# bminixhofer/zett

Hardware: AMD Instinct MI355X
Metric: predicted token-embeddings/sec (full target vocab) (higher is better)
Workload: dtype f16

## Files before the change

zett_amd/csrc/gemm.hip.h:

```cpp
#pragma once

#include <hip/hip_runtime.h>
#include <stdint.h>

#include <type_traits>

#ifndef ZETT_GROUP_M
#define ZETT_GROUP_M 4
#endif

namespace zett {

typedef __attribute__((ext_vector_type(16))) float f32x16;
typedef __attribute__((ext_vector_type(4))) float f32x4;
typedef __attribute__((ext_vector_type(8))) __bf16 bf16x8;
typedef __attribute__((ext_vector_type(4))) uint32_t u32x4;

typedef uint16_t bf16_t;
typedef _Float16 f16_t;
typedef __attribute__((ext_vector_type(8))) _Float16 f16x8;

__device__ __forceinline__ float bf16_to_f32(bf16_t v) { return __uint_as_float(((uint32_t)v) << 16); }
__device__ __forceinline__ bf16_t f32_to_bf16(float f) {
    return __builtin_bit_cast(bf16_t, (__bf16)f);
// ... 76 lines not shown
}

typedef __attribute__((ext_vector_type(2))) float f32x2;
#define ZETT_PIN_STAGE(arr, n) do { _Pragma("unroll") for (int e_ = 0; e_ < (n); ++e_) asm volatile("" : "+v"((arr)[e_])); } while (0)

template <int ACT, bool HAS_RES, bool HAS_SCALE, int NV>
__device__ __forceinline__ void epi_values(float (&vs)[NV], const float (&bias)[NV], const float (&res)[NV], const float (&sc)[NV], const float (&sh)[NV]) {
#pragma clang fp contract(off)
    static_assert(NV % 2 == 0, "pairs");
    constexpr int NP = NV / 2;
    f32x2 v[NP];
#pragma unroll
    for (int e = 0; e < NP; ++e) v[e] = f32x2{vs[2 * e], vs[2 * e + 1]} + f32x2{bias[2 * e], bias[2 * e + 1]};
    if (ACT == ACT_GELU_TANH) {
        f32x2 u2[NP], t[NP];
        ZETT_PIN_STAGE(v, NP);
#pragma unroll
        for (int e = 0; e < NP; ++e) u2[e] = (v[e] * v[e]) * v[e];
        ZETT_PIN_STAGE(u2, NP);
#pragma unroll
        for (int e = 0; e < NP; ++e) u2[e] = 1.5957691216057308f * __builtin_elementwise_fma(f32x2{0.044715f, 0.044715f}, u2[e], v[e]);
        ZETT_PIN_STAGE(u2, NP);
#pragma unroll
        for (int e = 0; e < NP; ++e) u2[e] = u2[e] * 1.4426950408889634f;
        ZETT_PIN_STAGE(u2, NP);
#pragma unroll
        for (int e = 0; e < NP; ++e) t[e] = f32x2{__builtin_amdgcn_exp2f(u2[e].x), __builtin_amdgcn_exp2f(u2[e].y)};
        ZETT_PIN_STAGE(t, NP);
#pragma unroll
        for (int e = 0; e < NP; ++e) t[e] = 1.0f + t[e];
        ZETT_PIN_STAGE(t, NP);
#pragma unroll
        for (int e = 0; e < NP; ++e) t[e] = f32x2{__builtin_amdgcn_rcpf(t[e].x), __builtin_amdgcn_rcpf(t[e].y)};
        ZETT_PIN_STAGE(t, NP);
#pragma unroll
        for (int e = 0; e < NP; ++e) t[e] = 1.0f - 2.0f * t[e];
        ZETT_PIN_STAGE(t, NP);
#pragma unroll
        for (int e = 0; e < NP; ++e) v[e] = (0.5f * v[e]) * (1.0f + t[e]);
        ZETT_PIN_STAGE(v, NP);
    } else if (ACT == ACT_GELU_ERF) {
        f32x2 z[NP], ax[NP], t[NP], p[NP], ex[NP];
        ZETT_PIN_STAGE(v, NP);
#pragma unroll
        for (int e = 0; e < NP; ++e) z[e] = v[e] * 0.70710678118654752440f;
        ZETT_PIN_STAGE(z, NP);
#pragma unroll
        for (int e = 0; e < NP; ++e) ax[e] = __builtin_elementwise_abs(z[e]);
#pragma unroll
        for (int e = 0; e < NP; ++e) t[e] = __builtin_elementwise_fma(f32x2{0.3275911f, 0.3275911f}, ax[e], f32x2{1.0f, 1.0f});
        ZETT_PIN_STAGE(t, NP);
#pragma unroll
        for (int e = 0; e < NP; ++e) t[e] = f32x2{__builtin_amdgcn_rcpf(t[e].x), __builtin_amdgcn_rcpf(t[e].y)};
        ZETT_PIN_STAGE(t, NP);
#pragma unroll
        for (int e = 0; e < NP; ++e) ex[e] = (ax[e] * ax[e]) * -1.4426950408889634f;
        ZETT_PIN_STAGE(ex, NP);
#pragma unroll
        for (int e = 0; e < NP; ++e) ex[e] = f32x2{__builtin_amdgcn_exp2f(ex[e].x), __builtin_amdgcn_exp2f(ex[e].y)};
        ZETT_PIN_STAGE(ex, NP);
#pragma unroll
        for (int e = 0; e < NP; ++e) p[e] = __builtin_elementwise_fma(f32x2{1.061405429f, 1.061405429f}, t[e], f32x2{-1.453152027f, -1.453152027f});
        ZETT_PIN_STAGE(p, NP);
#pragma unroll
        for (int e = 0; e < NP; ++e) p[e] = __builtin_elementwise_fma(p[e], t[e], f32x2{1.421413741f, 1.421413741f});
        ZETT_PIN_STAGE(p, NP);
#pragma unroll
        for (int e = 0; e < NP; ++e) p[e] = __builtin_elementwise_fma(p[e], t[e], f32x2{-0.284496736f, -0.284496736f});
        ZETT_PIN_STAGE(p, NP);
#pragma unroll
        for (int e = 0; e < NP; ++e) p[e] = __builtin_elementwise_fma(p[e], t[e], f32x2{0.254829592f, 0.254829592f});
        ZETT_PIN_STAGE(p, NP);
#pragma unroll
        for (int e = 0; e < NP; ++e) p[e] = -(p[e] * t[e]);
        ZETT_PIN_STAGE(p, NP);
#pragma unroll
        for (int e = 0; e < NP; ++e) p[e] = __builtin_elementwise_fma(p[e], ex[e], f32x2{1.0f, 1.0f});
        ZETT_PIN_STAGE(p, NP);
#pragma unroll
        for (int e = 0; e < NP; ++e) p[e] = 1.0f + __builtin_elementwise_copysign(p[e], z[e]);
        ZETT_PIN_STAGE(p, NP);
#pragma unroll
        for (int e = 0; e < NP; ++e) v[e] = (v[e] * 0.5f) * p[e];
        ZETT_PIN_STAGE(v, NP);
    }
    if (HAS_RES) {
#pragma unroll
        for (int e = 0; e < NP; ++e) v[e] = v[e] + f32x2{res[2 * e], res[2 * e + 1]};
    }
    if (HAS_SCALE) {
#pragma unroll
        for (int e = 0; e < NP; ++e) v[e] = __builtin_elementwise_fma(f32x2{sc[2 * e], sc[2 * e + 1]}, v[e], f32x2{sh[2 * e], sh[2 * e + 1]});
    }
#pragma unroll
    for (int e = 0; e < NP; ++e) { vs[2 * e] = v[e].x; vs[2 * e + 1] = v[e].y; }
}

template <typename T>
struct GemmEpilogue {
    const float* bias;
    int act;
    const float* residual;
    int ld_res;
    const float* res_stats;
    const float* res_gamma;
    const float* res_beta;
    const int32_t* res_index;
    float2* stats_part;
    int ld_part;
    const float* fold_stats;
    const float* fold_c;
    const float* scale;
    const float* shift;
    float* out_f32;
    int ld_f32;
    T* out_lo;
    int ld_lo;
    int split_col;
    float* out_f32_b;
    int32_t* range_flag;
    int range_final;
    const T* residual_lo;
    int ld_res_lo;
    void* dst;
    const int64_t* dst_rows;
    int64_t ld_dst;
    int dst_dtype;
};

template <typename T> struct LoRange { static constexpr bool checked = false; static constexpr float limit = 0.f; };
template <> struct LoRange<f16_t> { static constexpr bool checked = true; static constexpr float limit = 65504.0f; };
__device__ __forceinline__ bool out_of_range(float v, float limit) { return !(__builtin_fabsf(v) <= limit); }
constexpr float ZETT_F32_MAX = 3.402823466e38f;
constexpr int ZETT_RANGE_BIT_SOURCE = 1, ZETT_RANGE_BIT_ACTIVATION = 2, ZETT_RANGE_BIT_OUTPUT = 4, ZETT_RANGE_BIT_WEIGHT = 8, ZETT_RANGE_BIT_DEST = 16;
template <typename OT> __device__ __forceinline__ bool dest_overflow(float v) {
    if constexpr (std::is_same<OT, f16_t>::value) { const float a = __builtin_fabsf(v); return a >= 65520.0f && a <= 3.402823466e38f; }
    else return false;
}
__device__ __forceinline__ void range_report(int32_t* flag, bool bad, int bit) {
    if (bad && flag) atomicOr(flag, bit);
}

template <typename T>
struct GemmArgs {
    const T* A;
    int lda;
    const T* W;
    int ldw;
    int M, N, K;
    GemmEpilogue<T> epi;
    int tile_order = 0;
    int group = 0;
    int row0 = 0;
};

constexpr int GEMM_BM = 128;
constexpr int GEMM_BN = 128;
constexpr int GEMM_WAIT_VMCNT0 = 0x0F70;
constexpr int GEMM_ROW_BYTES = 128;
constexpr int GEMM_TILE_BYTES = GEMM_BM * GEMM_ROW_BYTES;

__device__ __forceinline__ int lds_chunk_off(int row, int chunk) {
    return row * GEMM_ROW_BYTES + ((chunk ^ ((row >> 1) & 7)) << 4);
}

template <typename T>
__device__ __forceinline__ void mfma_chunk(const u32x4& a, const u32x4& b, f32x16& acc);

template <>
__device__ __forceinline__ void mfma_chunk<bf16_t>(const u32x4& a, const u32x4& b, f32x16& acc) {
    acc = __builtin_amdgcn_mfma_f32_32x32x16_bf16(__builtin_bit_cast(bf16x8, a), __builtin_bit_cast(bf16x8, b),
                                                  acc, 0, 0, 0);
}
template <>
__device__ __forceinline__ void mfma_chunk<f16_t>(const u32x4& a, const u32x4& b, f32x16& acc) {
    acc = __builtin_amdgcn_mfma_f32_32x32x16_f16(__builtin_bit_cast(f16x8, a), __builtin_bit_cast(f16x8, b), acc, 0, 0, 0);
}
template <>
__device__ __forceinline__ void mfma_chunk<float>(const u32x4& a, const u32x4& b, f32x16& acc) {
#pragma unroll
    for (int j = 0; j < 4; ++j)
        acc = __builtin_amdgcn_mfma_f32_32x32x2f32(__uint_as_float(a[j]), __uint_as_float(b[j]), acc, 0, 0, 0);
}

template <typename T>
__global__ __launch_bounds__(256) void gemm_tn_kernel(GemmArgs<T> g) {
    extern __shared__ __attribute__((aligned(16))) unsigned char smem[];
    constexpr int EPC = 16 / (int)sizeof(T);
    constexpr int BK = GEMM_ROW_BYTES / (int)sizeof(T);

    const int tiles_m = (g.M + GEMM_BM - 1) / GEMM_BM;
    const int tiles_n = (g.N + GEMM_BN - 1) / GEMM_BN;
    const int nwg = tiles_m * tiles_n;
    int wg = blockIdx.x;
    {
        const int q = nwg >> 3, r = nwg & 7, xcd = wg & 7;
        wg = (xcd < r ? xcd * (q + 1) : r * (q + 1) + (xcd - r) * q) + (wg >> 3);
    }
    constexpr int GROUP_M = 8;
    const int group_size = GROUP_M * tiles_n;
    const int first_m = (wg / group_size) * GROUP_M;
    const int gm = (tiles_m - first_m) < GROUP_M ? (tiles_m - first_m) : GROUP_M;
    const int tm = first_m + (wg % group_size) % gm;
    const int tn = (wg % group_size) / gm;
    const int m0 = tm * GEMM_BM, n0 = tn * GEMM_BN;

    const int tid = threadIdx.x;
    const int lane = tid & 63, wave = tid >> 6;
    const int wm = wave >> 1, wn = wave & 1;
    const int l31 = lane & 31, hi = lane >> 5;

    const unsigned char* a_src[4];
    const unsigned char* w_src[4];
    int lds_dst[4];
#pragma unroll
    for (int i = 0; i < 4; ++i) {
        const int c = tid + 256 * i;
        const int row = c >> 3, ch = c & 7;
        int ar = m0 + row; ar = ar < g.M ? ar : g.M - 1;
        int wr = n0 + row; wr = wr < g.N ? wr : g.N - 1;
        a_src[i] = (const unsigned char*)(g.A + (size_t)ar * g.lda) + ch * 16;
        w_src[i] = (const unsigned char*)(g.W + (size_t)wr * g.ldw) + ch * 16;
        lds_dst[i] = lds_chunk_off(row, ch);
    }

    f32x16 acc[2][2];
#pragma unroll
    for (int i = 0; i < 2; ++i)
#pragma unroll
        for (int j = 0; j < 2; ++j)
#pragma unroll
            for (int r = 0; r < 16; ++r) acc[i][j][r] = 0.f;

    const int nk = g.K / BK;
    u32x4 ra[4], rw[4];
#pragma unroll
    for (int i = 0; i < 4; ++i) {
        ra[i] = *(const u32x4*)(a_src[i]);
        rw[i] = *(const u32x4*)(w_src[i]);
    }
#pragma unroll
    for (int i = 0; i < 4; ++i) {
        *(u32x4*)(smem + lds_dst[i]) = ra[i];
        *(u32x4*)(smem + GEMM_TILE_BYTES + lds_dst[i]) = rw[i];
    }
    __syncthreads();

    for (int kt = 0; kt < nk; ++kt) {
        const int cur = kt & 1;
        const unsigned char* As = smem + cur * 2 * GEMM_TILE_BYTES;
        const unsigned char* Ws = As + GEMM_TILE_BYTES;
        const bool more = kt + 1 < nk;
        if (more) {
            const size_t koff = (size_t)(kt + 1) * GEMM_ROW_BYTES;
#pragma unroll
            for (int i = 0; i < 4; ++i) {
                ra[i] = *(const u32x4*)(a_src[i] + koff);
                rw[i] = *(const u32x4*)(w_src[i] + koff);
            }
        }
#pragma unroll
        for (int kk = 0; kk < 4; ++kk) {
            const int ch = kk * 2 + hi;
            u32x4 fa[2], fw[2];
#pragma unroll
            for (int i = 0; i < 2; ++i) {
                fa[i] = *(const u32x4*)(As + lds_chunk_off(wm * 64 + i * 32 + l31, ch));
                fw[i] = *(const u32x4*)(Ws + lds_chunk_off(wn * 64 + i * 32 + l31, ch));
            }
#pragma unroll
            for (int i = 0; i < 2; ++i)
#pragma unroll
                for (int j = 0; j < 2; ++j) mfma_chunk<T>(fa[i], fw[j], acc[i][j]);
        }
        if (more) {
            unsigned char* Ad = smem + (cur ^ 1) * 2 * GEMM_TILE_BYTES;
#pragma unroll
            for (int i = 0; i < 4; ++i) {
                *(u32x4*)(Ad + lds_dst[i]) = ra[i];
                *(u32x4*)(Ad + GEMM_TILE_BYTES + lds_dst[i]) = rw[i];
            }
        }
        __syncthreads();
    }
    (void)EPC;

    const GemmEpilogue<T>& e = g.epi;
    bool bad_lo = false, bad_out = false;
#pragma unroll
    for (int j = 0; j < 2; ++j) {
        const int col = n0 + wn * 64 + j * 32 + l31;
        if (col >= g.N) continue;
        const float bias = e.bias ? e.bias[col] : 0.f;
        const float sc = e.scale ? e.scale[col] : 1.f;
        const float sh = e.shift ? e.shift[col] : 0.f;
#pragma unroll
        for (int i = 0; i < 2; ++i) {
#pragma unroll
            for (int r = 0; r < 16; ++r) {
                const int row = m0 + wm * 64 + i * 32 + (r & 3) + 8 * (r >> 2) + 4 * hi;
                if (row >= g.M) continue;
                const size_t rrow = e.res_index ? (size_t)e.res_index[row] : (size_t)row;
                float res = e.residual ? e.residual[rrow * e.ld_res + col] : 0.f;
                if (e.residual && e.res_stats) res = ln_affine(res, e.res_stats[2 * rrow], e.res_stats[2 * rrow + 1], e.res_gamma[col], e.res_beta[col]);
                const bool hr = e.residual != nullptr, hs = e.scale != nullptr;
                const float v = e.act == ACT_GELU_TANH ? epi_value<ACT_GELU_TANH>(acc[i][j][r], bias, hr, res, hs, sc, sh)
// ... 32 lines not shown
```

zett_amd/csrc/gemm4d.hip.h:

```cpp
#pragma once

#include <hip/hip_runtime.h>
#include <stdint.h>

#include <algorithm>
#include <type_traits>

#include "gemm_tile.hip.h"

namespace zett {

#ifndef G4D_ABLATE
#define G4D_ABLATE 5
#endif
constexpr int G4D_ABL = G4D_ABLATE;
#ifdef G4D_MFMA32
constexpr bool G4D_M32 = true;
static_assert(G4D_ABLATE < 5, "the 32x32x16 K loop exists for the ablation levels without an epilogue");
#else
constexpr bool G4D_M32 = false;
#endif
typedef float f32x16 __attribute__((ext_vector_type(16)));

constexpr int g4d_wait_vm(int n) { return ((n >> 4) << 14) | 0x0F70 | (n & 15); }

template <typename T> __device__ __forceinline__ void mfma16_agpr(f32x4& c, const u32x4& a, const u32x4& b);
template <> __device__ __forceinline__ void mfma16_agpr<bf16_t>(f32x4& c, const u32x4& a, const u32x4& b) {
    asm volatile("v_mfma_f32_16x16x32_bf16 %0, %1, %2, %0" : "+a"(c) : "v"(a), "v"(b));
}
template <> __device__ __forceinline__ void mfma16_agpr<f16_t>(f32x4& c, const u32x4& a, const u32x4& b) {
    asm volatile("v_mfma_f32_16x16x32_f16 %0, %1, %2, %0" : "+a"(c) : "v"(a), "v"(b));
}

template <typename T> __device__ __forceinline__ void mfma32_agpr(f32x16& c, const u32x4& a, const u32x4& b);
template <> __device__ __forceinline__ void mfma32_agpr<bf16_t>(f32x16& c, const u32x4& a, const u32x4& b) {
    asm volatile("v_mfma_f32_32x32x16_bf16 %0, %1, %2, %0" : "+a"(c) : "v"(a), "v"(b));
}
template <> __device__ __forceinline__ void mfma32_agpr<f16_t>(f32x16& c, const u32x4& a, const u32x4& b) {
    asm volatile("v_mfma_f32_32x32x16_f16 %0, %1, %2, %0" : "+a"(c) : "v"(a), "v"(b));
}

template <int K> __device__ __forceinline__ float g4d_xor_lane(float v) {
    return __builtin_bit_cast(float, __builtin_amdgcn_ds_swizzle(__builtin_bit_cast(int, v), (K << 10) | 0x1f));
}


enum { G4D_EPI_GENERIC = 0, G4D_EPI_LO = 1, G4D_EPI_F32 = 2, G4D_EPI_F32_SCALE = 3, G4D_EPI_BOTH = 4, G4D_EPI_F32_LN = 5, G4D_EPI_LO_FOLD = 6,
       G4D_EPI_LO_LN = 7, G4D_EPI_F32_SCALE_FOLD = 8, G4D_EPI_LN16 = 9 };
constexpr int G4D_EPI_STRIDE = 132;
constexpr int G4D_EPI_REGION = 64 * G4D_EPI_STRIDE * 4;
constexpr int G4D_LDS_BYTES = 4 * G4D_EPI_REGION;
static_assert(G4D_LDS_BYTES >= G256_LDS_BYTES && G4D_LDS_BYTES <= 160 * 1024, "LDS budget");

template <bool HALF> struct G4dGeom {
    static constexpr int BM = HALF ? 128 : G256_BM;
    static constexpr int WROWS = BM / 2;
    static constexpr int MI = WROWS / 16;
    static constexpr int AREQ = BM / 32;
    static constexpr int NREQ = AREQ + 8;
    static constexpr int NPASS = WROWS / 64;
    static constexpr int STAGES = HALF ? 3 : 2;
    static constexpr int A_BYTES = BM * GEMM_ROW_BYTES;
    static constexpr int STAGE_BYTES = A_BYTES + G256_OPERAND_BYTES;
    static constexpr int LDS_BYTES = STAGES * STAGE_BYTES;
};

template <typename T, int ACT = ACT_NONE, bool RES = false, int EPI = G4D_EPI_GENERIC, bool HALF = false, typename OT = void>
__global__ __launch_bounds__(256) __attribute__((amdgpu_waves_per_eu(1, 1))) void gemm4d_tn_kernel(GemmArgs<T> g) {
    extern __shared__ __attribute__((aligned(16))) unsigned char smem[];
    constexpr int BK = GEMM_ROW_BYTES / (int)sizeof(T);
    typedef G4dGeom<HALF> GEO;
    static_assert(!HALF || EPI != G4D_EPI_GENERIC, "the half tile carries the streamlined epilogues only");
    constexpr bool DST = !std::is_void<OT>::value;
    static_assert(!DST || EPI == G4D_EPI_F32_SCALE || EPI == G4D_EPI_F32_SCALE_FOLD, "destination stores: the output heads' epilogues only");

    const int tiles_m = (g.M - g.row0 + GEO::BM - 1) / GEO::BM;
    const int tiles_n = (g.N + G256_BN - 1) / G256_BN;
    const int nwg = tiles_m * tiles_n;
    int wg = blockIdx.x;
    {
        const int q = nwg >> 3, r = nwg & 7, xcd = wg & 7;
        wg = (xcd < r ? xcd * (q + 1) : r * (q + 1) + (xcd - r) * q) + (wg >> 3);
    }
    const int GROUP_N = g.group > 0 ? g.group : 4;
    int tm, tn;
    if (g.tile_order == 0) {
        const int group_size = GROUP_N * tiles_m;
        const int first_n = (wg / group_size) * GROUP_N;
        const int gn = (tiles_n - first_n) < GROUP_N ? (tiles_n - first_n) : GROUP_N;
        tn = first_n + (wg % group_size) % gn;
        tm = (wg % group_size) / gn;
    } else {
        const int GROUP_M = g.group > 0 ? g.group : ZETT_GROUP_M;
        const int group_size = GROUP_M * tiles_n;
        const int first_m = (wg / group_size) * GROUP_M;
        const int gm = (tiles_m - first_m) < GROUP_M ? (tiles_m - first_m) : GROUP_M;
        tm = first_m + (wg % group_size) % gm;
        tn = (wg % group_size) / gm;
    }
    const int m0 = g.row0 + tm * GEO::BM, n0 = tn * G256_BN;

    const int tid = threadIdx.x;
    const int lane = tid & 63;
    const int wave = __builtin_amdgcn_readfirstlane(tid >> 6);
    const int wm = wave >> 1, wn = wave & 1;

    const unsigned char* a_base = (const unsigned char*)(g.A + (size_t)m0 * g.lda);
    const unsigned char* w_base = (const unsigned char*)(g.W + (size_t)n0 * g.ldw);
    uint32_t a_voff[8], w_voff[8];
#pragma unroll
    for (int r = 0; r < 8; ++r) {
        const int row = wave * 64 + r * 8 + (lane >> 3);
        const int chunk = ((lane & 7) ^ ((row >> 1) & 7)) << 4;
        int wr = row; wr = n0 + wr < g.N ? wr : g.N - 1 - n0;
        w_voff[r] = (uint32_t)wr * (uint32_t)g.ldw * (uint32_t)sizeof(T) + chunk;
    }
#pragma unroll
    for (int r = 0; r < GEO::AREQ; ++r) {
        const int row = wave * (GEO::AREQ * 8) + r * 8 + (lane >> 3);
        const int chunk = ((lane & 7) ^ ((row >> 1) & 7)) << 4;
        int ar = row; ar = m0 + ar < g.M ? ar : g.M - 1 - m0;
        a_voff[r] = (uint32_t)ar * (uint32_t)g.lda * (uint32_t)sizeof(T) + chunk;
    }
    const __amdgpu_buffer_rsrc_t a_rsrc = __builtin_amdgcn_make_buffer_rsrc((void*)a_base, (short)0, 0x7fffffff, G4R_RSRC_WORD3);
    const __amdgpu_buffer_rsrc_t w_rsrc = __builtin_amdgcn_make_buffer_rsrc((void*)w_base, (short)0, 0x7fffffff, G4R_RSRC_WORD3);
    unsigned char* const my_rows = smem + wave * 64 * GEMM_ROW_BYTES;
    unsigned char* const my_a_rows = smem + wave * (GEO::AREQ * 8) * GEMM_ROW_BYTES;
    auto dma_a = [&](int stage, int kt, int r) {
        __builtin_amdgcn_raw_ptr_buffer_load_lds(a_rsrc, (lds_ptr_t)(my_a_rows + stage * GEO::STAGE_BYTES + r * 8 * GEMM_ROW_BYTES), 16,
                                                 a_voff[r], kt * GEMM_ROW_BYTES, 0, 0);
    };
    auto dma_w = [&](int stage, int kt, int r) {
        __builtin_amdgcn_raw_ptr_buffer_load_lds(w_rsrc, (lds_ptr_t)(my_rows + stage * GEO::STAGE_BYTES + GEO::A_BYTES + r * 8 * GEMM_ROW_BYTES), 16,
                                                 w_voff[r], kt * GEMM_ROW_BYTES, 0, 0);
    };

    constexpr bool M32 = G4D_M32 && !HALF;
    f32x4 acc[8][8];
    f32x16 acc32[4][4];
    if constexpr (M32) {
#pragma unroll
        for (int i = 0; i < 4; ++i)
#pragma unroll
            for (int j = 0; j < 4; ++j)
#pragma unroll
                for (int r = 0; r < 16; ++r) acc32[i][j][r] = 0.f;
    } else {
#pragma unroll
    for (int i = 0; i < GEO::MI; ++i)
#pragma unroll
        for (int j = 0; j < 8; ++j)
#pragma unroll
            for (int r = 0; r < 4; ++r) acc[i][j][r] = 0.f;
    }

    int a_off[2], w_off[2];
    {
        const int l15 = lane & 15, kq = lane >> 4;
        const int swz = (l15 >> 1) & 7;
#pragma unroll
        for (int kb = 0; kb < 2; ++kb) {
            const int c = ((kb * 4 + kq) ^ swz) << 4;
            a_off[kb] = (wm * GEO::WROWS + l15) * GEMM_ROW_BYTES + c;
            w_off[kb] = GEO::A_BYTES + (wn * 128 + l15) * GEMM_ROW_BYTES + c;
        }
    }
    int a_off32[4], w_off32[4];
    if constexpr (M32) {
        const int l31 = lane & 31, kh = lane >> 5;
        const int swz = (l31 >> 1) & 7;
#pragma unroll
        for (int k16 = 0; k16 < 4; ++k16) {
            const int c = ((k16 * 2 + kh) ^ swz) << 4;
            a_off32[k16] = (wm * GEO::WROWS + l31) * GEMM_ROW_BYTES + c;
            w_off32[k16] = GEO::A_BYTES + (wn * 128 + l31) * GEMM_ROW_BYTES + c;
        }
    }
    u32x4 fa[2][8], fw[2][8];
    auto read_a = [&](int stage, int kb, int i) {
        if constexpr (M32) fa[kb][i] = *(const u32x4*)(smem + stage * GEO::STAGE_BYTES + a_off32[kb * 2 + (i >> 2)] + (i & 3) * 32 * GEMM_ROW_BYTES);
        else fa[kb][i] = *(const u32x4*)(smem + stage * GEO::STAGE_BYTES + a_off[kb] + i * 16 * GEMM_ROW_BYTES);
    };
    auto read_w = [&](int stage, int kb, int j) {
        if constexpr (M32) fw[kb][j] = *(const u32x4*)(smem + stage * GEO::STAGE_BYTES + w_off32[kb * 2 + (j >> 2)] + (j & 3) * 32 * GEMM_ROW_BYTES);
        else fw[kb][j] = *(const u32x4*)(smem + stage * GEO::STAGE_BYTES + w_off[kb] + j * 16 * GEMM_ROW_BYTES);
    };

    const int nk = g.K / BK;
    constexpr bool LN16K = EPI == G4D_EPI_LN16;
    uint4 res16[LN16K ? 16 : 1];
    const bool res16_early = LN16K && g.epi.res_index == nullptr;
    auto res16_request = [&](int p, int t) __attribute__((always_inline)) {
        if constexpr (LN16K) {
            int grow = m0 + wm * GEO::WROWS + p * 64 + t * 4 + (lane >> 4);
            grow = grow < g.M ? grow : g.M - 1;
            int gc = n0 + wn * 128 + (lane & 15) * 8;
            gc = gc < g.N ? gc : 0;
            res16[t] = *(const uint4*)(g.epi.residual_lo + (size_t)grow * g.epi.ld_res_lo + gc);
        }
    };
#pragma unroll
    for (int st = 0; st < GEO::STAGES; ++st) {
        if (st < nk) {
#pragma unroll
            for (int r = 0; r < 8; ++r) dma_w(st, st, r);
#pragma unroll
            for (int r = 0; r < GEO::AREQ; ++r) dma_a(st, st, r);
        }
    }
    {
        const int ahead = (nk < GEO::STAGES ? nk : GEO::STAGES) - 1;
        if (ahead >= 2) __builtin_amdgcn_s_waitcnt(g4d_wait_vm(2 * GEO::NREQ));
        else if (ahead == 1) __builtin_amdgcn_s_waitcnt(g4d_wait_vm(GEO::NREQ));
        else __builtin_amdgcn_s_waitcnt(g4d_wait_vm(0));
    }
    __builtin_amdgcn_s_barrier();
    __builtin_amdgcn_sched_barrier(0);
#pragma unroll
    for (int j = 0; j < 8; ++j) read_w(0, 0, j);
#pragma unroll
    for (int i = 0; i < GEO::MI; ++i) read_a(0, 0, i);
    if constexpr (G4D_ABL < 2) {
#pragma unroll
        for (int j = 0; j < 8; ++j) read_w(0, 1, j);
#pragma unroll
        for (int i = 0; i < GEO::MI; ++i) read_a(0, 1, i);
        __builtin_amdgcn_s_waitcnt(G4R_WAIT_LGKM0);
    }

    auto step = [&](int kt, int cur, auto more_c, auto more2_c, auto moreA_c, auto wave_c) {
        constexpr bool more = decltype(more_c)::value, more2 = decltype(more2_c)::value, moreA = decltype(moreA_c)::value;
        constexpr int WV = decltype(wave_c)::value;
        const int nxt = cur + 1 == GEO::STAGES ? 0 : cur + 1;
        constexpr int P_BAR1 = HALF ? 26 : 36, P_BAR2 = HALF ? 52 : 102;
        constexpr int INFLIGHT = HALF ? ((more2 ? 1 : 0) + (moreA ? 1 : 0)) * GEO::NREQ : (moreA ? GEO::NREQ : 0);
#pragma unroll
        for (int kb = 0; kb < 2; ++kb)
#pragma unroll
        for (int i = 0; i < GEO::MI; ++i)
#pragma unroll
        for (int j = 0; j < 8; ++j) {
            const int p = kb * (GEO::MI * 8) + i * 8 + j;
            if (G4D_ABL >= 4 && p == P_BAR1 && (moreA || (!more && EPI != G4D_EPI_GENERIC))) {
                __builtin_amdgcn_s_waitcnt(G4R_WAIT_LGKM0);
                __builtin_amdgcn_s_barrier();
                __builtin_amdgcn_sched_barrier(0);
            }
            if (G4D_ABL >= 4 && p == P_BAR2 && more) {
                __builtin_amdgcn_s_waitcnt(g4d_wait_vm(INFLIGHT));
                __builtin_amdgcn_s_barrier();
                __builtin_amdgcn_sched_barrier(0);
            }
            if constexpr (M32) {
                if ((p & 1) == 0) {
                    const int q = (p >> 1) & 31, h = q >> 4, i32 = (q >> 2) & 3, j32 = q & 3;
                    mfma32_agpr<T>(acc32[i32][j32], fa[kb][h * 4 + i32], fw[kb][h * 4 + j32]);
                }
            } else
            mfma16_agpr<T>(acc[i][j], fa[kb][i], fw[kb][j]);
            constexpr bool RD = G4D_ABL >= 2, DMA = G4D_ABL >= 3;
            if (RD && p < 16 && (p & 1) == 0) read_w(cur, 1, p >> 1);
            if constexpr (!HALF) {
                if (RD && p >= 16 && p <= 30 && (p & 1) == 0) read_a(cur, 1, (p - 16) >> 1);
                if (DMA && moreA && p >= 38 && p < 70 && WV == ((p - 38) & 3)) dma_w(cur, kt + 2, (p - 38) >> 2);
                if (DMA && moreA && p >= 70 && p < 102 && WV == ((p - 70) & 3)) dma_a(cur, kt + 2, (p - 70) >> 2);
                if (RD && more && p >= 103 && p <= 110) read_w(nxt, 0, p - 103);
                if (RD && more && p >= 111 && p <= 125 && (p & 1) == 1) read_a(nxt, 0, (p - 111) >> 1);
                if constexpr (LN16K) { if (!more && p >= 40 && p < 104 && (p & 3) == 0 && res16_early) res16_request(0, (p - 40) >> 2); }
            } else {
                if (p >= 16 && p <= 22 && (p & 1) == 0) read_a(cur, 1, (p - 16) >> 1);
                if (moreA && p >= 27 && p < 43 && (WV & 1) == ((p - 27) & 1)) dma_w(cur, kt + 3, (p - 27) >> 1);
                if (moreA && p >= 43 && p < 51 && (WV & 1) == ((p - 43) & 1)) dma_a(cur, kt + 3, (p - 43) >> 1);
                if (more && p >= 53 && p <= 60) read_w(nxt, 0, p - 53);
                if (more && p >= 60 && p <= 63) read_a(nxt, 0, p - 60);
// ... 5 lines not shown
    typedef std::integral_constant<bool, true> yes_t;
    typedef std::integral_constant<bool, false> no_t;
    auto k_loop = [&](auto wave_c) {
        int kt = 0, cur = 0;
        auto next = [&]() { ++kt; cur = cur + 1 == GEO::STAGES ? 0 : cur + 1; };
        for (; kt + GEO::STAGES < nk; next()) step(kt, cur, yes_t{}, yes_t{}, yes_t{}, wave_c);
        if constexpr (HALF) {
            if (kt + 2 < nk) { step(kt, cur, yes_t{}, yes_t{}, no_t{}, wave_c); next(); }
        }
        if (kt + 1 < nk) { step(kt, cur, yes_t{}, no_t{}, no_t{}, wave_c); next(); }
        step(kt, cur, no_t{}, no_t{}, no_t{}, wave_c);
    };
    if (wave == 0) k_loop(std::integral_constant<int, 0>{});
    else if (wave == 1) k_loop(std::integral_constant<int, 1>{});
    else if (wave == 2) k_loop(std::integral_constant<int, 2>{});
    else k_loop(std::integral_constant<int, 3>{});

    asm volatile("s_nop 15\n\ts_nop 15");
    if constexpr (G4D_ABL < 5) {
        float keep = 0.f;
        if constexpr (M32) {
#pragma unroll
            for (int i = 0; i < 4; ++i)
#pragma unroll
                for (int j = 0; j < 4; ++j)
#pragma unroll
                    for (int r = 0; r < 16; ++r) keep += acc32[i][j][r];
        } else {
#pragma unroll
        for (int i = 0; i < GEO::MI; ++i)
#pragma unroll
            for (int j = 0; j < 8; ++j) keep += acc[i][j][0] + acc[i][j][1] + acc[i][j][2] + acc[i][j][3];
        }
        if (keep == 123.456f) g.epi.out_lo[threadIdx.x] = (T)0;
        return;
    }
    int tid_e = tid;
    asm volatile("" : "+v"(tid_e));
    const int lane_e = tid_e & 63;
    const int l15 = lane_e & 15, kq = lane_e >> 4;
    if constexpr (EPI == G4D_EPI_GENERIC) {
        __syncthreads();
        float* region = (float*)(smem + wave * 32768);
        typedef EpiDrain<T, ACT, RES, 64, 128, !RES, false> Drain;
        const int gcol = n0 + wn * 128 + (lane_e % Drain::LPR) * 8;
        const bool col_ok = gcol < g.N;
        float4 bias8[2], sc8[2], sh8[2];
        Drain::load_cols(g.epi, gcol, col_ok, bias8, sc8, sh8);
        float4 lng[2], lnb[2];
        Drain::load_ln_cols(g.epi, gcol, col_ok, lng, lnb);
#pragma unroll
        for (int p = 0; p < 2; ++p) {
            float4 oa[Drain::NIT], ob[Drain::NIT];
            const int row0 = m0 + wm * 128 + p * 64;
            Drain::load_res(g, row0, gcol, col_ok, lane_e, oa, ob);
            float2 lnst;
            Drain::load_res_stats(g, row0, lane_e, lnst);
#pragma unroll
            for (int i4 = 0; i4 < 4; ++i4)
#pragma unroll
                for (int j = 0; j < 8; ++j)
#pragma unroll
                    for (int r = 0; r < 4; ++r)
                        region[(i4 * 16 + kq * 4 + r) * 128 + j * 16 + l15] = acc[4 * p + i4][j][r];
            if (RES || p == 0) __builtin_amdgcn_s_waitcnt(GEMM_WAIT_VMCNT0);
            Drain::ln_res(g, lane_e, lng, lnb, lnst, oa, ob);
            Drain::drain(g, region, row0, gcol, col_ok, lane_e, bias8, sc8, sh8, oa, ob);
        }
    } else {
        constexpr bool LO = EPI == G4D_EPI_LO || EPI == G4D_EPI_LO_FOLD, SCALE = EPI == G4D_EPI_F32_SCALE || EPI == G4D_EPI_F32_SCALE_FOLD;
        constexpr bool LN16 = EPI == G4D_EPI_LN16;
        constexpr bool LNP = EPI == G4D_EPI_F32_LN || EPI == G4D_EPI_LO_LN || LN16, FOLD = EPI == G4D_EPI_LO_FOLD || EPI == G4D_EPI_F32_SCALE_FOLD;
        constexpr bool WF32 = EPI != G4D_EPI_LO_LN && !LN16;
        static_assert(!LNP || RES, "a LayerNorm producer is a residual epilogue");
        static_assert((EPI != G4D_EPI_F32_LN && !LN16) || ACT == ACT_NONE, "the encoder's producer has no activation");
        static_assert(!LN16 || sizeof(T) == 2, "16-bit residual stream");
        constexpr int CPL = (LO || LN16) ? 8 : 4;
        constexpr int LPR = 128 / CPL;
        constexpr int RPI = 64 / LPR;
        constexpr int NIT = 64 / RPI;
        static_assert(!(LO && RES), "the 16-bit-only epilogue has no residual");
        float* region = (float*)(smem + wave * G4D_EPI_REGION);
        const GemmEpilogue<T>& e = g.epi;
        constexpr bool W16 = LO || EPI == G4D_EPI_BOTH || LNP;
        constexpr bool CHK16 = W16 && LoRange<T>::checked;
        const bool chk_final = !W16 && e.range_final != 0;
        bool bad = false;
        const int idx = lane_e % LPR, rsub = lane_e / LPR;
        const int gcol = n0 + wn * 128 + idx * CPL;
        const bool col_ok = gcol < g.N;
        const int grow0 = m0 + wm * GEO::WROWS + rsub;
        float bias[CPL], sc[CPL], sh[CPL];
#pragma unroll
        for (int c = 0; c < CPL; ++c) { bias[c] = 0.f; sc[c] = 1.f; sh[c] = 0.f; }
        if (col_ok) {
#pragma unroll
            for (int c4 = 0; c4 < CPL; c4 += 4) {
                if (e.bias) { const float4 b = *(const float4*)(e.bias + gcol + c4); bias[c4] = b.x; bias[c4 + 1] = b.y; bias[c4 + 2] = b.z; bias[c4 + 3] = b.w; }
                if (SCALE) {
                    const float4 a = *(const float4*)(e.scale + gcol + c4), b = *(const float4*)(e.shift + gcol + c4);
                    sc[c4] = a.x; sc[c4 + 1] = a.y; sc[c4 + 2] = a.z; sc[c4 + 3] = a.w;
                    sh[c4] = b.x; sh[c4 + 1] = b.y; sh[c4 + 2] = b.z; sh[c4 + 3] = b.w;
                }
            }
        }
        const bool res_ln = RES && ACT == ACT_NONE && e.res_stats != nullptr;
        float lg[CPL], lb[CPL];
#pragma unroll
        for (int c = 0; c < CPL; ++c) { lg[c] = 1.f; lb[c] = 0.f; }
        float2 pst[2] = {make_float2(0.f, 1.f), make_float2(0.f, 1.f)};
        if constexpr (RES && ACT == ACT_NONE) {
            if (res_ln) {
                if (col_ok) {
#pragma unroll
                    for (int c4 = 0; c4 < CPL; c4 += 4) {
                        const float4 a = *(const float4*)(e.res_gamma + gcol + c4), b = *(const float4*)(e.res_beta + gcol + c4);
                        lg[c4] = a.x; lg[c4 + 1] = a.y; lg[c4 + 2] = a.z; lg[c4 + 3] = a.w; lb[c4] = b.x; lb[c4 + 1] = b.y; lb[c4 + 2] = b.z; lb[c4 + 3] = b.w;
                    }
                }
#pragma unroll
                for (int p = 0; p < GEO::NPASS; ++p) {
                    int srow = m0 + wm * GEO::WROWS + p * 64 + lane_e; srow = srow < g.M ? srow : g.M - 1;
                    if (e.res_index) srow = e.res_index[srow];
                    pst[p] = *(const float2*)(e.res_stats + 2 * (size_t)srow);
                }
            }
        }
        int rix[2] = {0, 0};
        const bool res_ix = RES && e.res_index != nullptr;
        if constexpr (RES) {
            if (res_ix) {
#pragma unroll
                for (int p = 0; p < GEO::NPASS; ++p) {
                    int srow = m0 + wm * GEO::WROWS + p * 64 + lane_e; srow = srow < g.M ? srow : g.M - 1;
                    rix[p] = e.res_index[srow];
                }
            }
        }
        float fc[FOLD ? CPL : 1];
        float2 fst[2] = {make_float2(0.f, 1.f), make_float2(0.f, 1.f)};
        if constexpr (FOLD) {
#pragma unroll
            for (int c = 0; c < CPL; ++c) fc[c] = 0.f;
            if (col_ok) {
#pragma unroll
                for (int c4 = 0; c4 < CPL; c4 += 4) {
                    const float4 a = *(const float4*)(e.fold_c + gcol + c4);
                    fc[c4] = a.x; fc[c4 + 1] = a.y; fc[c4 + 2] = a.z; fc[c4 + 3] = a.w;
                }
            }
#pragma unroll
            for (int p = 0; p < GEO::NPASS; ++p) {
                int srow = m0 + wm * GEO::WROWS + p * 64 + lane_e; srow = srow < g.M ? srow : g.M - 1;
                fst[p] = *(const float2*)(e.fold_stats + 2 * (size_t)srow);
            }
        }
        int64_t drow[2] = {0, 0};
        if constexpr (DST) {
#pragma unroll
            for (int p = 0; p < GEO::NPASS; ++p) {
                int srow = m0 + wm * GEO::WROWS + p * 64 + lane_e; srow = srow < g.M ? srow : g.M - 1;
                drow[p] = e.dst_rows ? e.dst_rows[srow] : (int64_t)srow;
            }
        }
        bool bad_dst = false;
        constexpr int RB = LNP ? 1 : 2;
        float4 res[LN16 ? 1 : RB][(RES && !LN16) ? NIT : 1];
        auto load_res16 = [&](int p, int ta, int tb) {
            if constexpr (LN16) {
#pragma unroll
                for (int t = ta; t < tb; ++t) {
                    if (res_ix) {
                        const int grow = grow0 + p * 64 + t * RPI;
                        const size_t rrow = (size_t)__shfl(rix[p], t * RPI + rsub, 64);
                        res16[t] = (grow < g.M && col_ok) ? *(const uint4*)(e.residual_lo + rrow * e.ld_res_lo + gcol) : make_uint4(0u, 0u, 0u, 0u);
                    } else {
                        res16_request(p, t);
                    }
                }
            }
        };
        auto load_res = [&](int p) {
            if constexpr (LN16) {
                load_res16(p, 0, NIT);
            } else if constexpr (RES) {
#pragma unroll
                for (int t = 0; t < NIT; ++t) {
                    const int grow = grow0 + p * 64 + t * RPI;
                    size_t rrow = (size_t)grow;
                    if (res_ix) {
                        const int i0 = __builtin_amdgcn_readlane(rix[p], t * RPI), i1 = __builtin_amdgcn_readlane(rix[p], t * RPI + 1);
                        rrow = (size_t)(rsub ? i1 : i0);
                    }
                    res[p % RB][t] = (grow < g.M && col_ok) ? *(const float4*)(e.residual + rrow * e.ld_res + gcol) : make_float4(0.f, 0.f, 0.f, 0.f);
                }
            }
        };
        auto stage = [&](int p) {
#pragma unroll
            for (int i4 = 0; i4 < 4; ++i4)
#pragma unroll
                for (int j = 0; j < 8; ++j)
#pragma unroll
                    for (int r = 0; r < 4; ++r)
                        region[(i4 * 16 + kq * 4 + r) * G4D_EPI_STRIDE + j * 16 + l15] = acc[4 * p + i4][j][r];
            if constexpr (FOLD)
                *(float2*)(region + lane_e * G4D_EPI_STRIDE + 128) = fst[p];
            if constexpr (LN16)
                *(float2*)(region + lane_e * G4D_EPI_STRIDE + 128) = pst[p];
        };
        auto drain = [&](int p, auto full_c) {
            constexpr bool FULL = decltype(full_c)::value;
            constexpr int GROUP = (LO || RES) ? 4 : 8;
            constexpr int NV = GROUP * CPL;
            float acc_s = 0.f, acc_q = 0.f;
#pragma unroll
            for (int t0 = 0; t0 < NIT; t0 += GROUP) {
                float v[NV], bb[NV], rr[NV], ss[NV], hh[NV];
#pragma unroll
                for (int u = 0; u < GROUP; ++u) {
                    const float* src = region + ((t0 + u) * RPI + rsub) * G4D_EPI_STRIDE + idx * CPL;
#pragma unroll
                    for (int c4 = 0; c4 < CPL; c4 += 4) {
                        const float4 x = *(const float4*)(src + c4);
                        v[u * CPL + c4] = x.x; v[u * CPL + c4 + 1] = x.y; v[u * CPL + c4 + 2] = x.z; v[u * CPL + c4 + 3] = x.w;
                    }
#pragma unroll
                    for (int c = 0; c < CPL; ++c) { bb[u * CPL + c] = bias[c]; ss[u * CPL + c] = sc[c]; hh[u * CPL + c] = sh[c]; rr[u * CPL + c] = 0.f; }
                    if constexpr (LN16) {
                        const uint4 x = res16[t0 + u];
                        unpack2_lo<T>(x.x, rr[u * 8], rr[u * 8 + 1]); unpack2_lo<T>(x.y, rr[u * 8 + 2], rr[u * 8 + 3]);
                        unpack2_lo<T>(x.z, rr[u * 8 + 4], rr[u * 8 + 5]); unpack2_lo<T>(x.w, rr[u * 8 + 6], rr[u * 8 + 7]);
                        if (res_ln) {
                            const float2 st = *(const float2*)(region + ((t0 + u) * RPI + rsub) * G4D_EPI_STRIDE + 128);
#pragma unroll
                            for (int c = 0; c < 8; ++c) rr[u * 8 + c] = ln_affine(rr[u * 8 + c], st.x, st.y, lg[c], lb[c]);
                        }
                    } else if constexpr (RES) {
                        const float4 x = res[p % RB][t0 + u];
                        rr[u * CPL] = x.x; rr[u * CPL + 1] = x.y; rr[u * CPL + 2] = x.z; rr[u * CPL + 3] = x.w;
                        if (ACT == ACT_NONE && res_ln) {
                            const int r0 = (t0 + u) * RPI;
                            const float mean0 = __builtin_bit_cast(float, __builtin_amdgcn_readlane(__builtin_bit_cast(int, pst[p].x), r0));
                            const float mean1 = __builtin_bit_cast(float, __builtin_amdgcn_readlane(__builtin_bit_cast(int, pst[p].x), r0 + 1));
                            const float rstd0 = __builtin_bit_cast(float, __builtin_amdgcn_readlane(__builtin_bit_cast(int, pst[p].y), r0));
                            const float rstd1 = __builtin_bit_cast(float, __builtin_amdgcn_readlane(__builtin_bit_cast(int, pst[p].y), r0 + 1));
                            const float mean = rsub ? mean1 : mean0, rstd = rsub ? rstd1 : rstd0;
#pragma unroll
                            for (int c = 0; c < 4; ++c) rr[u * CPL + c] = ln_affine(rr[u * CPL + c], mean, rstd, lg[c], lb[c]);
                        }
                    }
                }
                if constexpr (FOLD) {
#pragma unroll
                    for (int u = 0; u < GROUP; ++u) {
                        const float2 st = *(const float2*)(region + ((t0 + u) * RPI + rsub) * G4D_EPI_STRIDE + 128);
                        const float t = -st.x * st.y;
                        const f32x2 t2 = {t, t}, r2 = {st.y, st.y};
#pragma unroll
                        for (int c = 0; c < CPL; c += 2) {
                            const f32x2 x = __builtin_elementwise_fma(t2, f32x2{fc[c], fc[c + 1]}, f32x2{bias[c], bias[c + 1]});
                            const f32x2 y = __builtin_elementwise_fma(f32x2{v[u * CPL + c], v[u * CPL + c + 1]}, r2, x);
                            v[u * CPL + c] = y.x; v[u * CPL + c + 1] = y.y;
                            bb[u * CPL + c] = 0.f; bb[u * CPL + c + 1] = 0.f;
                        }
                    }
                }
                epi_values<ACT, RES, SCALE, NV>(v, bb, rr, ss, hh);
                if constexpr (CHK16) {
#pragma unroll
                    for (int x = 0; x < NV; ++x) bad |= out_of_range(v[x], LoRange<T>::limit);
                } else if (chk_final) {
#pragma unroll
                    for (int x = 0; x < NV; ++x) bad |= out_of_range(v[x], ZETT_F32_MAX);
                }
                if constexpr (LN16) {
                    static_assert(!LN16 || (GROUP == 4 && CPL == 8 && RPI == 4), "reduce-scatter layout");
                    float S[4], Q[4];
#pragma unroll
                    for (int u = 0; u < 4; ++u) {
                        const float* x = v + 8 * u;
                        S[u] = ((x[0] + x[1]) + (x[2] + x[3])) + ((x[4] + x[5]) + (x[6] + x[7]));
                        Q[u] = __builtin_fmaf(x[0], x[0], __builtin_fmaf(x[1], x[1], __builtin_fmaf(x[2], x[2], __builtin_fmaf(x[3], x[3],
                               __builtin_fmaf(x[4], x[4], __builtin_fmaf(x[5], x[5], __builtin_fmaf(x[6], x[6], x[7] * x[7])))))));
                    }
                    const bool b3 = (idx & 8) != 0, b2 = (idx & 4) != 0;
                    float ks0 = b3 ? S[2] : S[0], ks1 = b3 ? S[3] : S[1], kq0 = b3 ? Q[2] : Q[0], kq1 = b3 ? Q[3] : Q[1];
                    ks0 += g4d_xor_lane<8>(b3 ? S[0] : S[2]); ks1 += g4d_xor_lane<8>(b3 ? S[1] : S[3]);
                    kq0 += g4d_xor_lane<8>(b3 ? Q[0] : Q[2]); kq1 += g4d_xor_lane<8>(b3 ? Q[1] : Q[3]);
                    float ks = b2 ? ks1 : ks0, kq = b2 ? kq1 : kq0;
                    ks += g4d_xor_lane<4>(b2 ? ks0 : ks1); kq += g4d_xor_lane<4>(b2 ? kq0 : kq1);
                    ks += g4d_xor_lane<2>(ks); kq += g4d_xor_lane<2>(kq);
                    ks += g4d_xor_lane<1>(ks); kq += g4d_xor_lane<1>(kq);
                    const bool mine = (idx & 3) == (t0 >> 2);
                    acc_s = mine ? ks : acc_s; acc_q = mine ? kq : acc_q;
                } else if constexpr (LNP) {
                    static_assert(GROUP == 4 && CPL == 4 && RPI == 2, "reduce-scatter layout");
                    float S[4], Q[4];
#pragma unroll
                    for (int u = 0; u < 4; ++u) {
                        const float a = v[4 * u], b = v[4 * u + 1], c = v[4 * u + 2], d = v[4 * u + 3];
                        S[u] = (a + b) + (c + d);
                        Q[u] = __builtin_fmaf(a, a, __builtin_fmaf(b, b, __builtin_fmaf(c, c, d * d)));
                    }
                    const bool b4 = (idx & 16) != 0, b3 = (idx & 8) != 0;
                    float ks0 = b4 ? S[2] : S[0], ks1 = b4 ? S[3] : S[1], kq0 = b4 ? Q[2] : Q[0], kq1 = b4 ? Q[3] : Q[1];
// ... 80 lines not shown
        return -1;
    }
    if (e.stats_part) {
        const bool common = e.out_lo && e.residual && !e.scale && !e.shift && !e.out_f32_b && e.split_col >= g.N && g.N % 128 == 0 &&
                            e.ld_lo % 4 == 0 && e.ld_res % 4 == 0;
        if (common && e.out_f32 && e.act == ACT_NONE && e.ld_f32 % 4 == 0) return G4D_EPI_F32_LN;
        if (common && !e.out_f32 && e.act == ACT_GELU_TANH && !e.res_stats && !e.res_index) return G4D_EPI_LO_LN;
        return -1;
    }
    if (e.fold_stats) {
        if (e.fold_c && e.out_lo && !e.out_f32 && !e.residual && !e.scale && !e.shift && !e.out_f32_b && e.split_col >= g.N &&
            g.N % 8 == 0 && e.ld_lo % 8 == 0) return G4D_EPI_LO_FOLD;
        if (e.fold_c && e.out_f32 && !e.out_lo && !e.residual && e.scale && e.shift && e.act == ACT_NONE && !e.out_f32_b && e.split_col >= g.N &&
            g.N % 4 == 0 && e.ld_f32 % 4 == 0) return G4D_EPI_F32_SCALE_FOLD;
        return -1;
    }
    if (e.out_f32_b || e.split_col < g.N) return G4D_EPI_GENERIC;
    if (e.res_stats && (e.act != ACT_NONE || !e.residual)) return G4D_EPI_GENERIC;
    if (e.out_lo && !e.out_f32 && !e.residual && !e.scale && !e.shift && g.N % 8 == 0 && e.ld_lo % 8 == 0) return G4D_EPI_LO;
    if (e.out_f32 && e.out_lo && !e.residual && !e.scale && !e.shift && e.act == ACT_NONE && g.N % 4 == 0 && e.ld_f32 % 4 == 0 && e.ld_lo % 4 == 0)
        return G4D_EPI_BOTH;
    if (e.out_f32 && !e.out_lo && g.N % 4 == 0 && e.ld_f32 % 4 == 0 && (!e.residual || e.ld_res % 4 == 0)) {
        if (e.scale && e.shift && !e.residual && e.act == ACT_NONE) return G4D_EPI_F32_SCALE;
        if (!e.scale && !e.shift && (e.act == ACT_NONE || (e.act == ACT_GELU_TANH && e.residual))) return G4D_EPI_F32;
    }
    return G4D_EPI_GENERIC;
}

template <typename T, int ACT, bool RES, int EPI, bool HALF = false>
inline hipError_t launch_gemm4d_inst(const GemmArgs<T>& g, hipStream_t stream) {
    constexpr int lds = EPI == G4D_EPI_GENERIC ? G256_LDS_BYTES : (G4dGeom<HALF>::LDS_BYTES > G4D_LDS_BYTES ? G4dGeom<HALF>::LDS_BYTES : G4D_LDS_BYTES);
    static_assert(lds <= 160 * 1024, "LDS budget");
    static DeviceFlags attr;
    bool* done = attr.current();
    if (!done || !*done) {
        hipError_t e = hipFuncSetAttribute((const void*)gemm4d_tn_kernel<T, ACT, RES, EPI, HALF>, hipFuncAttributeMaxDynamicSharedMemorySize, lds);
        if (e != hipSuccess) return e;
        if (done) *done = true;
    }
    constexpr int BM = HALF ? 128 : G256_BM;
    const int tiles_m = (g.M - g.row0 + BM - 1) / BM;
    const int tiles_n = (g.N + G256_BN - 1) / G256_BN;
    if (tiles_m <= 0 || tiles_n <= 0) return hipSuccess;
    hipLaunchKernelGGL((gemm4d_tn_kernel<T, ACT, RES, EPI, HALF>), dim3(tiles_m * tiles_n), dim3(256), lds, stream, g);
    return hipGetLastError();
}

template <typename T, int ACT, bool HALF>
inline hipError_t launch_gemm4d_act(const GemmArgs<T>& g, hipStream_t stream, int mode) {
    const bool res = g.epi.residual != nullptr;
    switch (mode) {
        case G4D_EPI_LO: return launch_gemm4d_inst<T, ACT, false, G4D_EPI_LO, HALF>(g, stream);
        case G4D_EPI_LO_FOLD: return launch_gemm4d_inst<T, ACT, false, G4D_EPI_LO_FOLD, HALF>(g, stream);
        case G4D_EPI_F32:
            if constexpr (ACT == ACT_NONE) return res ? launch_gemm4d_inst<T, ACT, true, G4D_EPI_F32, HALF>(g, stream) : launch_gemm4d_inst<T, ACT, false, G4D_EPI_F32, HALF>(g, stream);
            else if constexpr (ACT == ACT_GELU_TANH) { if (res) return launch_gemm4d_inst<T, ACT, true, G4D_EPI_F32, HALF>(g, stream); }
            [[fallthrough]];
        default:
            if constexpr (HALF) return hipErrorInvalidValue;
            else return res ? launch_gemm4d_inst<T, ACT, true, G4D_EPI_GENERIC>(g, stream) : launch_gemm4d_inst<T, ACT, false, G4D_EPI_GENERIC>(g, stream);
    }
}

template <typename T, bool HALF>
inline hipError_t launch_gemm4d_mode(const GemmArgs<T>& g, hipStream_t stream, int mode) {
    if (mode == G4D_EPI_F32_LN) return launch_gemm4d_inst<T, ACT_NONE, true, G4D_EPI_F32_LN, HALF>(g, stream);
    if (mode == G4D_EPI_LN16) return launch_gemm4d_inst<T, ACT_NONE, true, G4D_EPI_LN16, HALF>(g, stream);
    if (mode == G4D_EPI_LO_LN) return launch_gemm4d_inst<T, ACT_GELU_TANH, true, G4D_EPI_LO_LN, HALF>(g, stream);
    if (mode == G4D_EPI_F32_SCALE_FOLD) return launch_gemm4d_inst<T, ACT_NONE, false, G4D_EPI_F32_SCALE_FOLD, HALF>(g, stream);
    if (mode == G4D_EPI_F32_SCALE) return launch_gemm4d_inst<T, ACT_NONE, false, G4D_EPI_F32_SCALE, HALF>(g, stream);
    if (mode == G4D_EPI_BOTH) return launch_gemm4d_inst<T, ACT_NONE, false, G4D_EPI_BOTH, HALF>(g, stream);
    switch (g.epi.act) {
        case ACT_GELU_TANH: return launch_gemm4d_act<T, ACT_GELU_TANH, HALF>(g, stream, mode);
        case ACT_GELU_ERF: return launch_gemm4d_act<T, ACT_GELU_ERF, HALF>(g, stream, mode);
        default: return launch_gemm4d_act<T, ACT_NONE, HALF>(g, stream, mode);
    }
}

template <typename T>
inline bool gemm4d_half_ok(const GemmArgs<T>& g, int mode) {
    if (mode <= G4D_EPI_GENERIC) return false;
    if (mode == G4D_EPI_F32) return g.epi.act == ACT_NONE || (g.epi.act == ACT_GELU_TANH && g.epi.residual);
    return true;
}

inline int gemm4d_row_split(int M, int N, int cus = 256, double half_cost = 0.62) {
    const long tn = (N + G256_BN - 1) / G256_BN, tm = (M + G256_BM - 1) / G256_BM;
    const long T = tm * tn;
    if (T % cus == 0) return M;
    const long rounds = (T + cus - 1) / cus;
    const long tm_full = std::min<long>(tm, ((rounds - 1) * cus) / tn);
    const long row0 = tm_full * G256_BM;
    if (row0 >= M) return M;
    const long th = ((M - row0 + 127) / 128) * tn;
    const double cost = (double)((tm_full * tn + cus - 1) / cus) + half_cost * (double)((th + cus - 1) / cus);
    return cost < (double)rounds - 0.05 ? (int)row0 : M;
}

template <typename T, int EPI, typename OT, bool HALF>
inline hipError_t launch_gemm4d_dst_inst(const GemmArgs<T>& g, hipStream_t stream) {
    constexpr int lds = G4dGeom<HALF>::LDS_BYTES > G4D_LDS_BYTES ? G4dGeom<HALF>::LDS_BYTES : G4D_LDS_BYTES;
    static DeviceFlags attr;
    bool* done = attr.current();
    if (!done || !*done) {
        hipError_t e = hipFuncSetAttribute((const void*)gemm4d_tn_kernel<T, ACT_NONE, false, EPI, HALF, OT>, hipFuncAttributeMaxDynamicSharedMemorySize, lds);
        if (e != hipSuccess) return e;
        if (done) *done = true;
    }
    constexpr int BM = HALF ? 128 : G256_BM;
    const int tiles_m = (g.M - g.row0 + BM - 1) / BM;
    const int tiles_n = (g.N + G256_BN - 1) / G256_BN;
    if (tiles_m <= 0 || tiles_n <= 0) return hipSuccess;
    hipLaunchKernelGGL((gemm4d_tn_kernel<T, ACT_NONE, false, EPI, HALF, OT>), dim3(tiles_m * tiles_n), dim3(256), lds, stream, g);
    return hipGetLastError();
}

template <typename T, bool HALF>
inline hipError_t launch_gemm4d_dst_mode(const GemmArgs<T>& g, hipStream_t stream, int mode) {
    const int dt = g.epi.dst_dtype;
    if (mode == G4D_EPI_F32_SCALE_FOLD) {
        if (dt == 1) return launch_gemm4d_dst_inst<T, G4D_EPI_F32_SCALE_FOLD, f16_t, HALF>(g, stream);
        if (dt == 2) return launch_gemm4d_dst_inst<T, G4D_EPI_F32_SCALE_FOLD, bf16_t, HALF>(g, stream);
        return launch_gemm4d_dst_inst<T, G4D_EPI_F32_SCALE_FOLD, float, HALF>(g, stream);
    }
    if (dt == 1) return launch_gemm4d_dst_inst<T, G4D_EPI_F32_SCALE, f16_t, HALF>(g, stream);
    if (dt == 2) return launch_gemm4d_dst_inst<T, G4D_EPI_F32_SCALE, bf16_t, HALF>(g, stream);
    return launch_gemm4d_dst_inst<T, G4D_EPI_F32_SCALE, float, HALF>(g, stream);
}

template <typename T>
inline int gemm4d_dst_mode(const GemmArgs<T>& g) {
    const GemmEpilogue<T>& e = g.epi;
    if (!e.dst || e.dst_dtype < 0 || e.dst_dtype > 2 || e.ld_dst % 4 != 0) return -1;
    const size_t align = e.dst_dtype == 0 ? 16 : 8;
    if ((uintptr_t)e.dst % align) return -1;
    GemmArgs<T> f = g;
    f.epi.out_f32 = (float*)e.dst;
    f.epi.ld_f32 = 4;
    const int mode = gemm4d_epi_mode(f);
    return (mode == G4D_EPI_F32_SCALE || mode == G4D_EPI_F32_SCALE_FOLD) ? mode : -1;
}

hipError_t launch_gemm_4d_half(const GemmArgs<f16_t>& g, hipStream_t stream, int mode);
hipError_t launch_gemm_4d_half(const GemmArgs<bf16_t>& g, hipStream_t stream, int mode);

hipError_t launch_gemm_4d_half_dst(const GemmArgs<f16_t>& g, hipStream_t stream, int mode);
hipError_t launch_gemm_4d_half_dst(const GemmArgs<bf16_t>& g, hipStream_t stream, int mode);

template <typename T>
inline hipError_t launch_gemm4d(const GemmArgs<T>& g, hipStream_t stream, bool force_generic = false) {
    const bool dst = g.epi.dst != nullptr;
    const int mode = dst ? gemm4d_dst_mode(g) : (force_generic && !g.epi.stats_part && !g.epi.fold_stats) ? G4D_EPI_GENERIC : gemm4d_epi_mode(g);
    if (mode < 0) return hipErrorInvalidValue;
    int split = g.row0 == -1 ? gemm4d_row_split(g.M, g.N) : (g.row0 == -2 ? 0 : (g.row0 > 0 ? std::min(g.row0, g.M) : g.M));
    if (split < g.M && (!gemm4d_half_ok(g, mode) || split % G256_BM != 0)) split = g.M;
    GemmArgs<T> full = g;
    full.row0 = 0;
    if (split < g.M) {
        full.M = split;
        if (split > 0)
            if (hipError_t e = dst ? launch_gemm4d_dst_mode<T, false>(full, stream, mode) : launch_gemm4d_mode<T, false>(full, stream, mode); e != hipSuccess) return e;
        GemmArgs<T> rest = g;
        rest.row0 = split;
        return dst ? launch_gemm_4d_half_dst(rest, stream, mode) : launch_gemm_4d_half(rest, stream, mode);
    }
    return dst ? launch_gemm4d_dst_mode<T, false>(full, stream, mode) : launch_gemm4d_mode<T, false>(full, stream, mode);
}

}
```

zett_amd/csrc/gemm_launch.hip:

```cpp
#include "gemm_launch.hip.h"

namespace zett {

hipError_t launch_gemm_variant(int variant, const GemmArgs<f16_t>& g, hipStream_t stream) {
    if (variant == 7 || variant == 8) return launch_gemm_4d(g, stream, variant == 8);
    return launch_gemm_x(variant, g, stream);
}
hipError_t launch_gemm_variant(int variant, const GemmArgs<bf16_t>& g, hipStream_t stream) {
    if (variant == 7 || variant == 8) return launch_gemm_4d(g, stream, variant == 8);
    return launch_gemm_x(variant, g, stream);
}
hipError_t launch_gemm_variant(int variant, const GemmArgs<float>& g, hipStream_t stream) {
    if (variant == 7 || variant == 8) return hipErrorInvalidValue;
    return launch_gemm_x(variant, g, stream);
}

}
```

zett_amd/csrc/rowops.hip.h:

```cpp
#pragma once

#include <hip/hip_runtime.h>
#include <stdint.h>

#include <type_traits>

#include "gemm.hip.h"

namespace zett {


struct PlanArrays {
    int32_t* row_count;
    int32_t* row_offset;
    uint8_t* row_uniform;
    int32_t* id_flag;
    int32_t* id_slot;
    int32_t* id_list;
    int32_t* tok_slot;
    int32_t* tok_pos;
    int32_t* tok_row;
    int32_t* tok_pkey;
    int32_t* pair_flag;
    int32_t* pair_slot;
    int32_t* tok_pair;
    int32_t* pair_tslot;
    int32_t* pair_pos;
    uint8_t* tok_key;
    int32_t* err;
    int32_t* counters;
    int32_t n_pair_keys;
};

__global__ void plan_rows_kernel(const int32_t* __restrict__ sfm, int64_t n_rows, int seq, int pad, int lam,
                                 int n_ids, PlanArrays p) {
    const int64_t n = (int64_t)blockIdx.x * blockDim.x + threadIdx.x;
    if (n >= n_rows) return;
    const int32_t* row = sfm + n * seq;
    int visible = 0;
    for (int j = 0; j < seq; ++j) {
        const int id = row[j];
        if (id < 0 || id >= n_ids) {
            atomicMax(p.err, (int)(n < 0x7ffffffe ? n + 1 : 0x7fffffff));
            p.row_count[n] = 0;
            p.row_uniform[n] = 2;
            return;
        }
        visible += (id != pad);
    }
    const bool uniform = (visible + lam) == 0;
    int count;
    if (uniform) {
        count = seq;
        for (int j = 0; j < seq; ++j) p.id_flag[row[j]] = 1;
    } else {
        count = visible + lam + (row[0] == pad ? 1 : 0);
        for (int j = 0; j < seq; ++j)
            if (j == 0 || row[j] != pad) p.id_flag[row[j]] = 1;
    }
    p.row_count[n] = count;
    p.row_uniform[n] = uniform ? 1 : 0;
}

__global__ __launch_bounds__(1024) void exclusive_scan_kernel(const int32_t* __restrict__ in,
                                                              int32_t* __restrict__ out, int64_t n) {
    __shared__ int32_t part[1024];
    const int t = threadIdx.x;
    const int64_t per = (n + 1023) / 1024;
    const int64_t b = (int64_t)t * per, e = (b + per < n) ? b + per : n;
    int32_t s = 0;
    for (int64_t i = b; i < e; ++i) s += in[i];
    part[t] = s;
    __syncthreads();
    for (int off = 1; off < 1024; off <<= 1) {
        int32_t v = (t >= off) ? part[t - off] : 0;
        __syncthreads();
        part[t] += v;
        __syncthreads();
    }
    int32_t run = (t == 0) ? 0 : part[t - 1];
    for (int64_t i = b; i < e; ++i) { const int32_t v = in[i]; out[i] = run; run += v; }
    if (t == 1023) out[n] = part[1023];
}

constexpr int SCAN_CHUNK = 4096;

__device__ __forceinline__ int32_t block_exclusive_scan_256(int32_t v, int32_t* sh , int32_t* total) {
    const int t = threadIdx.x;
    sh[t] = v;
    __syncthreads();
    for (int off = 1; off < 256; off <<= 1) {
        const int32_t add = (t >= off) ? sh[t - off] : 0;
        __syncthreads();
        sh[t] += add;
        __syncthreads();
    }
    if (total) *total = sh[255];
    return sh[t] - v;
}

__global__ __launch_bounds__(256) void scan_chunk_sums_kernel(const int32_t* __restrict__ in, int64_t n, int32_t* __restrict__ sums) {
    __shared__ int32_t sh[256];
    const int64_t base = (int64_t)blockIdx.x * SCAN_CHUNK + threadIdx.x * 16;
    int32_t s = 0;
#pragma unroll
    for (int k = 0; k < 16; ++k) { const int64_t i = base + k; if (i < n) s += in[i]; }
    int32_t total;
    block_exclusive_scan_256(s, sh, &total);
    if (threadIdx.x == 0) sums[blockIdx.x] = total;
}

__global__ __launch_bounds__(256) void scan_apply_kernel(const int32_t* __restrict__ in, int64_t n, const int32_t* __restrict__ offs,
                                                         int32_t* __restrict__ out) {
    __shared__ int32_t sh[256];
    const int64_t base = (int64_t)blockIdx.x * SCAN_CHUNK + threadIdx.x * 16;
    int32_t v[16];
    int32_t s = 0;
#pragma unroll
    for (int k = 0; k < 16; ++k) { const int64_t i = base + k; v[k] = i < n ? in[i] : 0; s += v[k]; }
    int32_t run = offs[blockIdx.x] + block_exclusive_scan_256(s, sh, nullptr);
#pragma unroll
    for (int k = 0; k < 16; ++k) { const int64_t i = base + k; if (i < n) out[i] = run; run += v[k]; }
    if (blockIdx.x == gridDim.x - 1 && threadIdx.x == 0) out[n] = offs[gridDim.x];
}

inline void launch_exclusive_scan(const int32_t* in, int32_t* out, int64_t n, int32_t* scratch, hipStream_t st) {
    if (n <= SCAN_CHUNK * 4) {
        hipLaunchKernelGGL(exclusive_scan_kernel, dim3(1), dim3(1024), 0, st, in, out, n);
        return;
    }
    const int chunks = (int)((n + SCAN_CHUNK - 1) / SCAN_CHUNK);
    int32_t* sums = scratch;
    int32_t* offs = scratch + chunks;
    hipLaunchKernelGGL(scan_chunk_sums_kernel, dim3(chunks), dim3(256), 0, st, in, n, sums);
    hipLaunchKernelGGL(exclusive_scan_kernel, dim3(1), dim3(1024), 0, st, (const int32_t*)sums, offs, (int64_t)chunks);
    hipLaunchKernelGGL(scan_apply_kernel, dim3(chunks), dim3(256), 0, st, in, n, (const int32_t*)offs, out);
}

__global__ void plan_tokens_kernel(const int32_t* __restrict__ sfm, int64_t n_rows, int seq, int pad, int lam,
                                   int n_ids, PlanArrays p) {
    const int64_t n = (int64_t)blockIdx.x * blockDim.x + threadIdx.x;
    if (n >= n_rows) return;
    const int32_t* row = sfm + n * seq;
    int t = p.row_offset[n];
    if (p.row_uniform[n] == 2) return;
    const bool uniform = p.row_uniform[n] == 1;
    const int lp = seq + lam;
    for (int j = 0; j < seq; ++j) {
        const int id = row[j];
        const bool vis = id != pad;
        if (uniform || vis || j == 0) {
            p.tok_slot[t] = p.id_slot[id];
            p.tok_pos[t] = j;
            p.tok_row[t] = (int32_t)n;
            p.tok_key[t] = vis ? 1 : 0;
            if (p.pair_flag) { const int key = id * lp + j; p.tok_pkey[t] = key; p.pair_flag[key] = 1; }
            ++t;
        }
    }
    if (lam) {
        p.tok_slot[t] = -1;
        p.tok_pos[t] = seq;
        p.tok_row[t] = (int32_t)n;
        p.tok_key[t] = 1;
        if (p.pair_flag) { const int key = n_ids * lp + seq; p.tok_pkey[t] = key; p.pair_flag[key] = 1; }
    }
}

__global__ void plan_pairs_kernel(int64_t n_rows, PlanArrays p) {
    const int64_t t = (int64_t)blockIdx.x * blockDim.x + threadIdx.x;
    if (t >= p.row_offset[n_rows]) return;
    const int ps = p.pair_slot[p.tok_pkey[t]];
    p.tok_pair[t] = ps;
    p.pair_tslot[ps] = p.tok_slot[t];
    p.pair_pos[ps] = p.tok_pos[t];
}

__device__ __forceinline__ int chunk_row(int t_rel, int row_rel, bool first, int rows);
__global__ void pair_rows_kernel(int m, int tok0, int64_t row0, int rows, PlanArrays p, int32_t* __restrict__ brow_pair) {
    const int t = blockIdx.x * blockDim.x + threadIdx.x;
    if (t >= m) return;
    const int n = p.tok_row[tok0 + t];
    brow_pair[chunk_row(t, (int)(n - row0), p.row_offset[n] == tok0 + t, rows)] = p.tok_pair[tok0 + t];
}

__global__ void plan_idlist_kernel(int n_ids, PlanArrays p) {
    const int id = blockIdx.x * blockDim.x + threadIdx.x;
    if (id < n_ids && p.id_flag[id]) p.id_list[p.id_slot[id]] = id;
    if (id == 0) {
        p.counters[0] = p.id_slot[n_ids];
        p.counters[1] = p.err[0];
        p.counters[2] = p.n_pair_keys ? p.pair_slot[p.n_pair_keys] : 0;
    }
}

__device__ __forceinline__ float wave_sum(float v) {
#pragma unroll
    for (int off = 32; off > 0; off >>= 1) v += __shfl_xor(v, off, 64);
    return v;
}

__device__ __forceinline__ float block_sum_256(float v, float* red ) {
    v = wave_sum(v);
    __syncthreads();
    if ((threadIdx.x & 63) == 0) red[threadIdx.x >> 6] = v;
    __syncthreads();
    return red[0] + red[1] + red[2] + red[3];
}

template <typename T> __device__ __forceinline__ void store_lo4(T* dst, float4 v);
template <> __device__ __forceinline__ void store_lo4<float>(float* dst, float4 v) { *(float4*)dst = v; }
template <> __device__ __forceinline__ void store_lo4<bf16_t>(bf16_t* dst, float4 v) {
    *(uint2*)dst = make_uint2(pack2_lo<bf16_t>(v.x, v.y), pack2_lo<bf16_t>(v.z, v.w));
}
template <> __device__ __forceinline__ void store_lo4<f16_t>(f16_t* dst, float4 v) {
    *(uint2*)dst = make_uint2(pack2_lo<f16_t>(v.x, v.y), pack2_lo<f16_t>(v.z, v.w));
}

template <int SRC_DTYPE> __device__ __forceinline__ float4 load_src4(const void* base, size_t elem);
template <> __device__ __forceinline__ float4 load_src4<0>(const void* base, size_t e) {
    return *(const float4*)((const float*)base + e);
}
template <> __device__ __forceinline__ float4 load_src4<1>(const void* base, size_t e) {
    const uint2 u = *(const uint2*)((const uint16_t*)base + e);
    typedef __attribute__((ext_vector_type(4))) _Float16 f16x4;
    const f16x4 hv = __builtin_bit_cast(f16x4, u);
    return make_float4((float)hv[0], (float)hv[1], (float)hv[2], (float)hv[3]);
}
template <> __device__ __forceinline__ float4 load_src4<2>(const void* base, size_t e) {
    const uint2 u = *(const uint2*)((const uint16_t*)base + e);
    return make_float4(__uint_as_float(u.x << 16), __uint_as_float(u.x & 0xffff0000u),
                       __uint_as_float(u.y << 16), __uint_as_float(u.y & 0xffff0000u));
}

template <typename T, int SRC_DTYPE>
__global__ __launch_bounds__(256) void gather_src_kernel(const int32_t* __restrict__ id_list, int slot0, int n_slots,
                                                         const void* __restrict__ src, int e_in, int v0,
                                                         const float* __restrict__ fallback,
                                                         const float* __restrict__ sc_w, const float* __restrict__ sc_b,
                                                         T* __restrict__ out, int32_t* __restrict__ range_flag) {
    const int s = blockIdx.x;
    if (s >= n_slots) return;
    const int id = id_list[slot0 + s];
    T* dst = out + (size_t)s * e_in;
    bool bad = false;
    auto chk = [&](float4 v) {
        if (LoRange<T>::checked)
            bad |= out_of_range(v.x, LoRange<T>::limit) | out_of_range(v.y, LoRange<T>::limit) | out_of_range(v.z, LoRange<T>::limit) |
                   out_of_range(v.w, LoRange<T>::limit);
    };
    if (id >= v0) {
        const float* f = fallback + (size_t)(id - v0) * e_in;
        for (int c = threadIdx.x * 4; c < e_in; c += 1024) { const float4 v = *(const float4*)(f + c); chk(v); store_lo4<T>(dst + c, v); }
    } else {
        const size_t base = (size_t)id * e_in;
        for (int c = threadIdx.x * 4; c < e_in; c += 1024) {
            float4 v = load_src4<SRC_DTYPE>(src, base + c);
            if (sc_w) {
                const float4 w = *(const float4*)(sc_w + c), b = *(const float4*)(sc_b + c);
                v.x = w.x * v.x + b.x; v.y = w.y * v.y + b.y; v.z = w.z * v.z + b.z; v.w = w.w * v.w + b.w;
            }
            chk(v);
            store_lo4<T>(dst + c, v);
        }
    }
    range_report(range_flag, bad, ZETT_RANGE_BIT_SOURCE);
}

struct LnEmbed {
    const float* table;
    const int32_t* tok_slot;
    const int32_t* tok_pos;
    const float* type0;
    const float* pos_emb;
    const float* lang;
    int lang_pos;
    const int32_t* tok_row;
    const int32_t* row_offset;
    int64_t row0;
    int rows;
    const void* table_lo;
    const float* table_stats;
    const float* table_gamma;
    const float* table_beta;
};

__device__ __forceinline__ int chunk_row(int t_rel, int row_rel, bool first, int rows) {
    return first ? row_rel : rows + t_rel - row_rel - 1;
}

struct LnReadout {
    const float* bias_w;
    const float* bias_b;
    float* out_bias;
    const void* in_lo;
    const int64_t* bias_rows;
    int32_t* range_flag;
};

template <typename BT> __device__ __forceinline__ void ln_readout_store(const LnReadout& ro, int r, float v) {
    if constexpr (std::is_void<BT>::value) {
        ro.out_bias[r] = v;
    } else {
        const int64_t d = ro.bias_rows ? ro.bias_rows[r] : (int64_t)r;
        if (d < 0) return;
        ((BT*)ro.out_bias)[d] = to_lo<BT>(v);
        range_report(ro.range_flag, dest_overflow<BT>(v), ZETT_RANGE_BIT_DEST);
    }
}

constexpr int LN_MAX_VEC = 8;

template <typename T, bool EMBED, int TPR = 256, bool READOUT = false, typename BT = void>
__global__ __launch_bounds__(256) void layernorm_rows_kernel(const float* __restrict__ in, int ld_in, int rows, int H,
                                                             const float* __restrict__ gamma,
                                                             const float* __restrict__ beta, float eps,
                                                             float* __restrict__ out_f32, T* __restrict__ out_lo,
                                                             float* __restrict__ stats_out, float* __restrict__ sum_out,
                                                             LnEmbed emb, int tok0, LnReadout readout) {
    __shared__ float red[4];
    const int r = blockIdx.x * (256 / TPR) + (int)threadIdx.x / TPR;
    if (r >= rows) return;
    const int nvec = H >> 2;
    const int tid = threadIdx.x % TPR;
    auto row_sum = [&](float x_) { return TPR == 256 ? block_sum_256(x_, red) : wave_sum(x_); };
    const float* x = nullptr;
    const float* posr = nullptr;
    bool is_lang = false;
    int ro = r;
    const T* tbl_lo = nullptr;
    float2 tbl_st = make_float2(0.f, 1.f);
    if constexpr (EMBED) {
        const int slot = emb.tok_slot[tok0 + r];
        is_lang = slot < 0;
        if (emb.table_lo && !is_lang) {
            tbl_lo = (const T*)emb.table_lo + (size_t)slot * H;
            tbl_st = *(const float2*)(emb.table_stats + 2 * (size_t)slot);
            x = emb.lang;
        } else
        x = is_lang ? emb.lang : emb.table + (size_t)slot * H;
        posr = emb.pos_emb + (size_t)emb.tok_pos[tok0 + r] * H;
        if (emb.tok_row) {
            const int n = emb.tok_row[tok0 + r];
            ro = chunk_row(r, (int)(n - emb.row0), emb.row_offset[n] == tok0 + r, emb.rows);
        }
// ... 146 lines not shown
    float2 tbl_st = make_float2(0.f, 1.f);
    if constexpr (EMBED) {
        const int slot = emb.tok_slot[tok0 + r];
        is_lang = slot < 0;
        if (emb.table_lo && !is_lang) {
            tbl_lo = (const T*)emb.table_lo + (size_t)slot * H;
            tbl_st = *(const float2*)(emb.table_stats + 2 * (size_t)slot);
            x = emb.lang;
        } else
        x = is_lang ? emb.lang : emb.table + (size_t)slot * H;
        posr = emb.pos_emb + (size_t)emb.tok_pos[tok0 + r] * H;
        if (emb.tok_row) {
            const int n = emb.tok_row[tok0 + r];
            ro = chunk_row(r, (int)(n - emb.row0), emb.row_offset[n] == tok0 + r, emb.rows);
        }
    } else {
        x = in + (size_t)r * ld_in;
    }
    auto load = [&](int c, float (&a)[8]) {
        bool have = false;
        if constexpr (READOUT) {
            if (readout.in_lo) { load8<T>((const T*)readout.in_lo + (size_t)r * ld_in + c, a); have = true; }
        }
        if constexpr (EMBED) {
            if (tbl_lo) {
                load8<T>(tbl_lo + c, a);
                float g[8], b[8];
                load8<float>(emb.table_gamma + c, g);
                load8<float>(emb.table_beta + c, b);
#pragma unroll
                for (int k = 0; k < 8; ++k) a[k] = ln_affine(a[k], tbl_st.x, tbl_st.y, g[k], b[k]);
                have = true;
            }
        }
        if (!have) load8<float>(x + c, a);
        if constexpr (EMBED) {
            float t0[8], p[8];
            load8<float>(emb.type0 + c, t0);
            load8<float>(posr + c, p);
            if (is_lang) {
                float pl[8];
                load8<float>(emb.pos_emb + (size_t)emb.lang_pos * H + c, pl);
#pragma unroll
                for (int k = 0; k < 8; ++k) a[k] -= (t0[k] + pl[k]);
            }
#pragma unroll
            for (int k = 0; k < 8; ++k) a[k] = (a[k] + t0[k]) + p[k];
        }
    };
    float v[NVMAX][8];
    float s = 0.f;
#pragma unroll
    for (int j = 0; j < NVMAX; ++j) {
        if (j < nv) {
            load((tid + TPR * j) * 8, v[j]);
            s += ((v[j][0] + v[j][1]) + (v[j][2] + v[j][3])) + ((v[j][4] + v[j][5]) + (v[j][6] + v[j][7]));
        }
    }
    const float mean = group_sum<TPR>(s) / (float)H;
    float q = 0.f;
#pragma unroll
    for (int j = 0; j < NVMAX; ++j) {
        if (j < nv) {
            float d[8];
#pragma unroll
            for (int k = 0; k < 8; ++k) { d[k] = v[j][k] - mean; d[k] *= d[k]; }
            q += ((d[0] + d[1]) + (d[2] + d[3])) + ((d[4] + d[5]) + (d[6] + d[7]));
        }
    }
    const float var = group_sum<TPR>(q) / (float)H;
    const float rstd = 1.0f / sqrtf(var + eps);
    if (stats_out && tid == 0) *(float2*)(stats_out + 2 * (size_t)ro) = make_float2(mean, rstd);
    float dot = 0.f;
#pragma unroll
    for (int j = 0; j < NVMAX; ++j) {
        if (j < nv) {
            const int c = (tid + TPR * j) * 8;
            float g[8], b[8], o[8];
            load8<float>(gamma + c, g);
            load8<float>(beta + c, b);
#pragma unroll
            for (int k = 0; k < 8; ++k) o[k] = ln_affine(v[j][k], mean, rstd, g[k], b[k]);
            if (EMBED && sum_out) store8<float>(sum_out + (size_t)ro * H + c, v[j]);
            if (out_f32) store8<float>(out_f32 + (size_t)ro * H + c, o);
            if (out_lo) store8<T>(out_lo + (size_t)ro * H + c, o);
            if (READOUT && readout.bias_w) {
                float w[8];
                load8<float>(readout.bias_w + c, w);
                dot += ((o[0] * w[0] + o[1] * w[1]) + (o[2] * w[2] + o[3] * w[3])) + ((o[4] * w[4] + o[5] * w[5]) + (o[6] * w[6] + o[7] * w[7]));
            }
        }
    }
    if constexpr (READOUT) {
        if (readout.out_bias) {
            const float tot = group_sum<TPR>(dot);
            if (tid == 0) ln_readout_store<BT>(readout, r, readout.bias_w ? tot + readout.bias_b[0] : 0.f);
        }
    }
}

constexpr int ATT_FAST_KEYS = 8;

template <typename T> __device__ __forceinline__ float dot8_lo(const uint4& a, const uint4& b);
template <> __device__ __forceinline__ float dot8_lo<f16_t>(const uint4& a, const uint4& b) {
    typedef __attribute__((ext_vector_type(2))) _Float16 h2;
    float s = __builtin_amdgcn_fdot2(__builtin_bit_cast(h2, a.x), __builtin_bit_cast(h2, b.x), 0.f, false);
    s = __builtin_amdgcn_fdot2(__builtin_bit_cast(h2, a.y), __builtin_bit_cast(h2, b.y), s, false);
    s = __builtin_amdgcn_fdot2(__builtin_bit_cast(h2, a.z), __builtin_bit_cast(h2, b.z), s, false);
    return __builtin_amdgcn_fdot2(__builtin_bit_cast(h2, a.w), __builtin_bit_cast(h2, b.w), s, false);
}
template <> __device__ __forceinline__ float dot8_lo<bf16_t>(const uint4& a, const uint4& b) {
    float x[8], y[8];
    unpack2_lo<bf16_t>(a.x, x[0], x[1]); unpack2_lo<bf16_t>(a.y, x[2], x[3]); unpack2_lo<bf16_t>(a.z, x[4], x[5]); unpack2_lo<bf16_t>(a.w, x[6], x[7]);
    unpack2_lo<bf16_t>(b.x, y[0], y[1]); unpack2_lo<bf16_t>(b.y, y[2], y[3]); unpack2_lo<bf16_t>(b.z, y[4], y[5]); unpack2_lo<bf16_t>(b.w, y[6], y[7]);
    float s = 0.f;
#pragma unroll
    for (int c = 0; c < 8; ++c) s = fmaf(x[c], y[c], s);
    return s;
}
template <> __device__ __forceinline__ float dot8_lo<float>(const uint4&, const uint4&) { return 0.f; }

__device__ __forceinline__ float head_sum(float s, int lph) {
    auto dpp = [](float v, auto ctrl) {
        return __builtin_bit_cast(float, __builtin_amdgcn_update_dpp(0, __builtin_bit_cast(int, v), decltype(ctrl)::value, 0xf, 0xf, true));
    };
    if (lph >= 2) s += dpp(s, std::integral_constant<int, 0xB1>{});
    if (lph >= 4) s += dpp(s, std::integral_constant<int, 0x4E>{});
    if (lph >= 8) s += dpp(s, std::integral_constant<int, 0x141>{});
    if (lph >= 16) s += dpp(s, std::integral_constant<int, 0x140>{});
    if (lph >= 32) s += __builtin_bit_cast(float, __builtin_amdgcn_ds_swizzle(__builtin_bit_cast(int, s), (16 << 10) | 0x1f));
    if (lph >= 64) s += __shfl_xor(s, 32, 64);
    return s;
}

struct AttentionWaves { int64_t total, full; int full_groups, lanes_per_row; };
__host__ __device__ inline AttentionWaves attention_waves(int rows, int H, bool pack) {
    const int rem = H & 511, gfull = H >> 9;
    AttentionWaves a;
    if (pack && (rem == 256 || rem == 128 || rem == 64)) {
        a.full_groups = gfull; a.lanes_per_row = rem >> 3;
        a.full = (int64_t)rows * gfull;
        const int per = 64 / a.lanes_per_row;
        a.total = a.full + (rows + per - 1) / per;
    } else {
        a.full_groups = (H + 511) >> 9; a.lanes_per_row = 64;
        a.full = (int64_t)rows * a.full_groups;
        a.total = a.full;
    }
    return a;
}

template <typename T>
__global__ __launch_bounds__(256) void attention_rows_kernel(const T* __restrict__ qbase, size_t ldq,
                                                             const T* __restrict__ kbase, const T* __restrict__ vbase,
                                                             size_t ldkv, int H, int head_dim,
                                                             const int32_t* __restrict__ row_offset,
                                                             const uint8_t* __restrict__ row_uniform,
                                                             const uint8_t* __restrict__ tok_key, int64_t row0,
                                                             int rows, int tok0, float scaling, int flags ,
                                                             const int32_t* __restrict__ tok_pair, T* __restrict__ ctx) {
    const int cls_only = flags & 1;
    const int lane = threadIdx.x & 63;
    const int64_t w = (int64_t)blockIdx.x * 4 + (threadIdx.x >> 6);
    const AttentionWaves aw = attention_waves(rows, H, (flags & 4) != 0);
    if (w >= aw.total) return;
    int rl, grp, li = lane, base = 0, lpr = 64;
    bool valid = true;
    if (w < aw.full) { rl = (int)(w / aw.full_groups); grp = (int)(w % aw.full_groups); }
    else {
        lpr = aw.lanes_per_row;
        const int sub = lane / lpr;
        li = lane - sub * lpr;
        base = sub * lpr;
        rl = (int)(w - aw.full) * (64 / lpr) + sub;
        grp = aw.full_groups;
        valid = rl < rows;
        if (!valid) rl = rows - 1;
    }
    const int col = grp * 512 + li * 8;
    const bool active = valid && col < H;
    const int lph = head_dim >> 3;
    const int64_t n = row0 + rl;
    const int t0 = row_offset[n] - tok0, t1 = row_offset[n + 1] - tok0;
    const bool uniform = row_uniform[n];
    const int nq = cls_only ? 1 : (t1 - t0);
    const int ccol = active ? col : 0;
    auto brow = [&](int t) -> size_t { return (size_t)chunk_row(t, rl, t == t0, rows); };
    int pslot = 0;
    if (tok_pair) { const int t = t0 + li; pslot = t < t1 ? tok_pair[tok0 + t] : 0; }
    auto qrow = [&](int t) -> size_t {
        if (!tok_pair) return brow(t);
        return t - t0 < lpr ? (size_t)__shfl(pslot, base + (t - t0), 64) : (size_t)tok_pair[tok0 + t];
    };
    const int nk = t1 - t0;
    if constexpr (sizeof(T) == 2) {
        if (nk <= ATT_FAST_KEYS && (flags & 2)) {
            const bool mine = li < nk && (uniform || tok_key[tok0 + t0 + li] != 0);
            const unsigned on = (unsigned)(__ballot(mine) >> base) & (lpr >= 32 ? 0xffffffffu : ((1u << lpr) - 1u));
            uint4 kk[ATT_FAST_KEYS], vv[ATT_FAST_KEYS], qq[ATT_FAST_KEYS];
#pragma unroll
            for (int j = 0; j < ATT_FAST_KEYS; ++j) {
                if (j < nk) {
                    const size_t kr = qrow(t0 + j);
                    kk[j] = *(const uint4*)(kbase + kr * ldkv + ccol);
                    vv[j] = *(const uint4*)(vbase + kr * ldkv + ccol);
                    if (!cls_only) qq[j] = *(const uint4*)(qbase + kr * ldq + ccol);
                }
            }
            if (cls_only) qq[0] = *(const uint4*)(qbase + (size_t)rl * ldq + ccol);
            const float sc2 = scaling * 1.4426950408889634f;
#pragma unroll
            for (int qi = 0; qi < ATT_FAST_KEYS; ++qi) {
                if (qi < nq) {
                    float sj[ATT_FAST_KEYS];
                    float mx = -INFINITY;
#pragma unroll
                    for (int j = 0; j < ATT_FAST_KEYS; ++j) {
                        sj[j] = -INFINITY;
                        if (j < nk && ((on >> j) & 1u)) {
                            const float d = head_sum(dot8_lo<T>(qq[qi], kk[j]), lph);
                            sj[j] = uniform ? 0.f : d * sc2;
                            mx = fmaxf(mx, sj[j]);
                        }
                    }
                    float l = 0.f, acc[8];
#pragma unroll
                    for (int c = 0; c < 8; ++c) acc[c] = 0.f;
#pragma unroll
                    for (int j = 0; j < ATT_FAST_KEYS; ++j) {
                        if (j < nk && ((on >> j) & 1u)) {
                            const float pj = __builtin_amdgcn_exp2f(sj[j] - mx);
                            l += pj;
                            float v[8];
                            unpack2_lo<T>(vv[j].x, v[0], v[1]); unpack2_lo<T>(vv[j].y, v[2], v[3]);
                            unpack2_lo<T>(vv[j].z, v[4], v[5]); unpack2_lo<T>(vv[j].w, v[6], v[7]);
#pragma unroll
                            for (int c = 0; c < 8; ++c) acc[c] = fmaf(pj, v[c], acc[c]);
                        }
                    }
                    const float inv = 1.0f / l;
#pragma unroll
                    for (int c = 0; c < 8; ++c) acc[c] *= inv;
                    if (active) {
                        const size_t orow = cls_only ? (size_t)rl : brow(t0 + qi);
                        store8<T>(ctx + orow * H + col, acc);
                    }
                }
            }
            return;
        }
    }
    for (int qi = 0; qi < nq; ++qi) {
        float q[8];
        load8<T>(qbase + (cls_only ? (size_t)rl : qrow(t0 + qi)) * ldq + ccol, q);
        float mx = -INFINITY, l = 0.f, acc[8];
#pragma unroll
        for (int c = 0; c < 8; ++c) acc[c] = 0.f;
        for (int kj = t0; kj < t1; ++kj) {
            if (!uniform && !tok_key[tok0 + kj]) continue;
            float k[8], v[8];
            const size_t kr = qrow(kj);
            load8<T>(kbase + kr * ldkv + ccol, k);
            load8<T>(vbase + kr * ldkv + ccol, v);
            float s = 0.f;
#pragma unroll
            for (int c = 0; c < 8; ++c) s = fmaf(q[c], k[c], s);
            for (int off = 1; off < lph; off <<= 1) s += __shfl_xor(s, off, 64);
            s = uniform ? 0.f : s * scaling;
            const float nm = fmaxf(mx, s);
            const float corr = expf(mx - nm);
            const float p = expf(s - nm);
            l = fmaf(l, corr, p);
#pragma unroll
            for (int c = 0; c < 8; ++c) acc[c] = fmaf(acc[c], corr, p * v[c]);
            mx = nm;
        }
        const float inv = 1.0f / l;
#pragma unroll
        for (int c = 0; c < 8; ++c) acc[c] *= inv;
        if (active) {
            const size_t orow = cls_only ? (size_t)rl : brow(t0 + qi);
            store8<T>(ctx + orow * H + col, acc);
        }
    }
}

__global__ __launch_bounds__(64) void ln_stats_kernel(const float2* __restrict__ part, int parts, int ld_part, int rows, int H, float eps,
                                                      float* __restrict__ stats) {
    const int r = blockIdx.x * blockDim.x + threadIdx.x;
    if (r >= rows) return;
    float s = 0.f, q = 0.f;
    const float2* col = part + r;
    int p = 0;
    for (; p + 8 <= parts; p += 8) {
        float2 v[8];
#pragma unroll
        for (int j = 0; j < 8; ++j) v[j] = col[(size_t)(p + j) * ld_part];
#pragma unroll
        for (int j = 0; j < 8; ++j) { s += v[j].x; q += v[j].y; }
    }
    {
        float2 v[8];
#pragma unroll
        for (int j = 0; j < 8; ++j) v[j] = p + j < parts ? col[(size_t)(p + j) * ld_part] : make_float2(0.f, 0.f);
#pragma unroll
        for (int j = 0; j < 8; ++j)
            if (p + j < parts) { s += v[j].x; q += v[j].y; }
    }
    const float mean = s / (float)H;
    const float var = fmaxf(q / (float)H - mean * mean, 0.f);
    *(float2*)(stats + 2 * (size_t)r) = make_float2(mean, 1.0f / sqrtf(var + eps));
}

template <typename T>
__global__ __launch_bounds__(256) void fold_weight_kernel(const float* __restrict__ w, int K, const float* __restrict__ gamma,
                                                          const float* __restrict__ beta, const float* __restrict__ bias,
                                                          T* __restrict__ w_fold, float* __restrict__ c_out, float* __restrict__ b_out,
                                                          int32_t* __restrict__ range_flag) {
    __shared__ float red[4];
    const int n = blockIdx.x;
    const float* row = w + (size_t)n * K;
    float cs = 0.f, bs = 0.f;
    for (int k = threadIdx.x; k < K; k += 256) {
        const float x = row[k];
        if (LoRange<T>::checked) range_report(range_flag, out_of_range(x * gamma[k], LoRange<T>::limit), ZETT_RANGE_BIT_WEIGHT);
        const T lo = to_lo<T>(x * gamma[k]);
        w_fold[(size_t)n * K + k] = lo;
        cs += lo_to_f32<T>(lo);
        bs = fmaf(x, beta[k], bs);
    }
    const float ct = block_sum_256(cs, red);
    const float bt = block_sum_256(bs, red);
    if (threadIdx.x == 0) { c_out[n] = ct; b_out[n] = bias[n] + bt; }
}

template <typename T>
__global__ void convert_f32_to_lo_kernel(const float* __restrict__ in, T* __restrict__ out, size_t n, int32_t* __restrict__ range_flag) {
    size_t i = ((size_t)blockIdx.x * blockDim.x + threadIdx.x) * 4;
    const size_t stride = (size_t)gridDim.x * blockDim.x * 4;
    bool bad = false;
    for (; i + 3 < n; i += stride) {
        const float4 v = *(const float4*)(in + i);
        if (LoRange<T>::checked)
            bad |= out_of_range(v.x, LoRange<T>::limit) | out_of_range(v.y, LoRange<T>::limit) | out_of_range(v.z, LoRange<T>::limit) |
                   out_of_range(v.w, LoRange<T>::limit);
        store_lo4<T>(out + i, v);
    }
    if (blockIdx.x == 0 && threadIdx.x == 0) {
        for (size_t j = n & ~(size_t)3; j < n; ++j) { out[j] = to_lo<T>(in[j]); if (LoRange<T>::checked) bad |= out_of_range(in[j], LoRange<T>::limit); }
    }
    range_report(range_flag, bad, ZETT_RANGE_BIT_WEIGHT);
}
template <int SRC_DTYPE>
__global__ void convert_to_f32_kernel(const void* __restrict__ in, float* __restrict__ out, size_t n) {
    size_t i = (size_t)blockIdx.x * blockDim.x + threadIdx.x;
    const size_t stride = (size_t)gridDim.x * blockDim.x;
    for (; i < n; i += stride) {
        if constexpr (SRC_DTYPE == 1) out[i] = (float)((const _Float16*)in)[i];
        else out[i] = __uint_as_float(((uint32_t)((const uint16_t*)in)[i]) << 16);
    }
}

template <typename OT> __device__ __forceinline__ void store4_dst(OT* d, float4 v) {
    if constexpr (std::is_same<OT, float>::value) *(float4*)d = v;
    else *(uint2*)d = make_uint2(pack2_lo<OT>(v.x, v.y), pack2_lo<OT>(v.z, v.w));
}

template <typename OT, bool VEC>
__global__ __launch_bounds__(256) void dest_store_rows_kernel(const float* __restrict__ src, int64_t ld_src, OT* __restrict__ dst, int64_t ld_dst,
                                                              const int64_t* __restrict__ rows, int64_t n_rows, int cols, int32_t* range_flag) {
    bool bad = false;
    for (int64_t i = blockIdx.x; i < n_rows; i += gridDim.x) {
        const int64_t d = rows ? rows[i] : i;
        if (d < 0) continue;
        const float* s = src + i * ld_src;
        OT* o = dst + d * ld_dst;
        if constexpr (VEC) {
            for (int c = (int)threadIdx.x * 4; c < cols; c += 256 * 4) {
                const float4 v = *(const float4*)(s + c);
                store4_dst<OT>(o + c, v);
                bad |= dest_overflow<OT>(v.x) | dest_overflow<OT>(v.y) | dest_overflow<OT>(v.z) | dest_overflow<OT>(v.w);
            }
        } else {
            for (int c = (int)threadIdx.x; c < cols; c += 256) {
                const float v = s[c];
                o[c] = to_lo<OT>(v);
                bad |= dest_overflow<OT>(v);
            }
        }
    }
    range_report(range_flag, bad, ZETT_RANGE_BIT_DEST);
}

__global__ void dest_rows_check_kernel(const int64_t* __restrict__ rows, int64_t n, int64_t n_dest, int32_t* err) {
    const int64_t i = (int64_t)blockIdx.x * blockDim.x + threadIdx.x;
    if (i < n && rows[i] >= n_dest) atomicMax(err, (int)(i < 0x7ffffffe ? i + 1 : 0x7fffffff));
}

}
```

zett_amd/csrc/zett_hip.hip:

```cpp
#include <hip/hip_runtime.h>

#include <algorithm>
#include <array>
#include <cstdlib>
#include <cmath>
#include <cstdarg>
#include <cstdio>
#include <cstring>
#include <map>
#include <string>
#include <type_traits>
#include <vector>

#include "../../include/zett_hip.h"
#include "common.hip.h"
#include "gemm.hip.h"
#include "gemm_launch.hip.h"
#include "rowops.hip.h"
#include "retok.hip.h"
#include "lexical.hip.h"
#include "partition.hip.h"

using namespace zett;

namespace {

struct Tensor {
    float* f32 = nullptr;
    void* lo = nullptr;
    std::vector<int64_t> shape;
    size_t numel = 0;
};

inline size_t round_up(size_t v, size_t m) { return (v + m - 1) / m * m; }

}

struct zett_hypernet {
    zett_config cfg{};
    int device = 0;
    int precision = ZETT_PREC_BF16;
    bool finalized = false;
    std::map<std::string, Tensor> w;
    std::vector<void*> qkv_w;
    std::vector<float*> qkv_b;
    struct Folded { void* w = nullptr; float* c = nullptr; float* b = nullptr; };
    std::vector<Folded> fold_qkv, fold_up;
    Folded fold_head_in, fold_head_out;
    float* head_one = nullptr;
    float* head_zero = nullptr;
    int ln_fold = 1;
    float* head_scale = nullptr;
    float* head_shift = nullptr;
    std::vector<void*> owned;
    int64_t max_chunk_tokens = 0;
    int time_gemm = 0;
    int cls_only_last = 1;
    int pair_dedupe = 1;
    int residual_lo = 1;
    int concurrent_lanes = 0;
    hipStream_t lane_stream = nullptr;
    hipEvent_t lane_ev[4] = {nullptr, nullptr, nullptr, nullptr};
    int attention_fast = 1;
    int attention_pack = 1;
    int gemm_tail_split = 1;
    int gemm_tile_order = 0;
    int ln_rows8 = 1;
    int table_lo = 1;
    int gemm_group = 0;
    int gemm4d_min_k = 512;
    int gemm_variant = 0;
    struct PlanSlot {
        DevBuf i32, u8;
        int32_t* host = nullptr;
        size_t host_ints = 0;
        hipEvent_t done = nullptr;
        hipEvent_t released = nullptr;
        const int32_t* sfm = nullptr;
        int64_t n_rows = 0;
        int seq = 0;
        bool pair_plan = false;
        const int32_t* ext_id_slot = nullptr;
        bool pending = false;
    } plan[2];
    PlanSlot table_plan;
    struct ExtTable { const void* table = nullptr; const float* stats = nullptr; const int32_t* id_slot = nullptr; } ext;
    int plan_cur = 0;
    hipStream_t plan_stream = nullptr;
    hipEvent_t plan_fork = nullptr;
    DevBuf table, x0, yf, yt, big, pre, ctx, cf, ct, lnstats, lnparts;
    hipEvent_t out_ready[2] = {nullptr, nullptr};
    bool out_recorded = false;
    int range_accumulate = 0;
    int32_t* range_word = nullptr;
    int32_t* range_host = nullptr;
    DevBuf dest_word, dest_stage[2], dest_sink;
    int32_t* dest_host = nullptr;
    hipEvent_t dest_checked = nullptr;
    std::vector<hipEvent_t> ev;
    size_t ev_used = 0;
    std::vector<double> ev_flops;
    std::vector<std::array<int, 4>> ev_shape;
    std::vector<zett_gemm_record> gemm_log;
    zett_stats stats{};
};

namespace {

size_t elt_size(int precision) { return precision == ZETT_PREC_F32 ? 4 : 2; }

bool is_gemm_weight(const std::string& n) {
    static const char* suffixes[] = {"input_projection.0.weight", "dense1.weight", "dense2.weight",
                                     "query.weight", "key.weight", "value.weight", "dense.weight",
                                     "output_projection.1.weight", "output_projection_out.1.weight"};
    for (const char* s : suffixes) {
        const size_t ls = strlen(s);
        if (n.size() >= ls && n.compare(n.size() - ls, ls, s) == 0) return true;
    }
    return false;
}

void expected_shapes(const zett_config& c, std::map<std::string, std::vector<int64_t>>& s) {
    const int64_t H = c.hidden, I = c.intermediate;
    auto proj = [&](const std::string& p) {
        s[p + "dense1.weight"] = {I, H}; s[p + "dense1.bias"] = {I};
        s[p + "dense2.weight"] = {H, I}; s[p + "dense2.bias"] = {H};
        s[p + "ln.weight"] = {H}; s[p + "ln.bias"] = {H};
    };
    if (c.embed_lang) s["lang_embeddings.weight"] = {c.n_langs, H};
    s["model.embeddings.token_type_embeddings.weight"] = {1, H};
    s["model.embeddings.LayerNorm.weight"] = {H};
    s["model.embeddings.LayerNorm.bias"] = {H};
    s["model.embeddings.position_embeddings.weight"] = {c.max_positions, H};
    for (int l = 0; l < c.layers; ++l) {
        const std::string p = "model.encoder.layer." + std::to_string(l) + ".";
        for (const char* q : {"query", "key", "value"}) {
            s[p + "attention.self." + q + ".weight"] = {H, H};
            s[p + "attention.self." + q + ".bias"] = {H};
        }
        s[p + "attention.output.dense.weight"] = {H, H}; s[p + "attention.output.dense.bias"] = {H};
        s[p + "attention.output.LayerNorm.weight"] = {H}; s[p + "attention.output.LayerNorm.bias"] = {H};
        s[p + "intermediate.dense.weight"] = {I, H}; s[p + "intermediate.dense.bias"] = {I};
        s[p + "output.dense.weight"] = {H, I}; s[p + "output.dense.bias"] = {H};
        s[p + "output.LayerNorm.weight"] = {H}; s[p + "output.LayerNorm.bias"] = {H};
    }
    s["fallback_embeddings.weight"] = {c.n_extra, c.n_in_embd};
    s["input_projection.0.weight"] = {H, c.n_in_embd}; s["input_projection.0.bias"] = {H};
    proj("input_projection.1.");
    proj("output_projection.0.");
    const int64_t w0 = c.single_head ? c.n_in_embd : c.n_embd;
    s["output_projection.1.weight"] = {w0, H}; s["output_projection.1.bias"] = {w0};
    if (c.separate_out && !c.single_head) {
        proj("output_projection_out.0.");
        s["output_projection_out.1.weight"] = {c.n_embd, H}; s["output_projection_out.1.bias"] = {c.n_embd};
    }
    if (c.rescale) {
        s["in_scaler.w"] = {1, c.n_in_embd}; s["in_scaler.b"] = {1, c.n_in_embd};
        s["scaler.w"] = {1, c.n_embd}; s["scaler.b"] = {1, c.n_embd};
        if (c.separate_out) { s["out_scaler.w"] = {1, c.n_embd}; s["out_scaler.b"] = {1, c.n_embd}; }
    }
    if (c.predict_bias) { s["bias_projection.weight"] = {1, H}; s["bias_projection.bias"] = {1}; }
}

int validate_config(const zett_config& c, int precision) {
    if (c.n_embd <= 0 || c.hidden <= 0 || c.intermediate <= 0 || c.heads <= 0 || c.layers <= 0)
        return fail(ZETT_E_INVALID, "non-positive dimension in zett_config");
    if (c.n_in_embd != (c.separate_out ? 2 * c.n_embd : c.n_embd))
        return fail(ZETT_E_INVALID, "n_in_embd must be 2*n_embd iff separate_out");
    if (c.hidden % c.heads) return fail(ZETT_E_INVALID, "hidden %d not divisible by heads %d", c.hidden, c.heads);
    const int d = c.hidden / c.heads;
    if (d < 8 || d > 512 || (d & (d - 1))) return fail(ZETT_E_INVALID, "head_dim %d unsupported (need a power of two in [8,512])", d);
    const int kq = precision == ZETT_PREC_F32 ? 32 : 64;
    for (int k : {c.n_in_embd, c.hidden, c.intermediate})
        if (k % kq) return fail(ZETT_E_INVALID, "contraction width %d is not a multiple of %d", k, kq);
    if (c.n_embd % 4) return fail(ZETT_E_INVALID, "n_embd must be a multiple of 4");
    if (c.n_extra < 1) return fail(ZETT_E_INVALID, "n_extra must be >= 1 (reference allocates max(hn_n_extra_tokens,1))");
    if (c.pad_token_id < 0) return fail(ZETT_E_INVALID, "pad_token_id is required");
    if (c.embed_lang && c.n_langs <= 0) return fail(ZETT_E_INVALID, "hn_embed_lang_id needs n_langs");
    return 0;
}

struct WorkspaceSizes {
    int64_t chunk_tokens;
    size_t table, x0, f32_rows, lo_rows, big, stats;
    size_t total() const { return table + x0 + 3 * f32_rows + 3 * lo_rows + big + stats; }
};

static int64_t pair_keys(const zett_config& c, int seq) {
    return ((int64_t)c.original_vocab_size + c.n_extra + 1) * (int64_t)(seq + (c.embed_lang ? 1 : 0));
}

static size_t plan_i32_bytes(const zett_config& c, int64_t N, int seq) {
    const int64_t V = (int64_t)c.original_vocab_size + c.n_extra;
    const int64_t max_tok = N * (int64_t)(seq + (c.embed_lang ? 1 : 0));
    const int64_t K = pair_keys(c, seq);
    const size_t scan_scratch = 2 * ((size_t)std::max<int64_t>(std::max<int64_t>(N, V), K) / SCAN_CHUNK + 2) + 1;
    return ((size_t)N + (N + 1) + 3 + V + (V + 1) + V + 7 * (size_t)max_tok + 2 * (size_t)K + 2 + scan_scratch) * 4;
}

static int64_t chunk_token_cap(const zett_config& c, size_t es) {
    const size_t wide = (size_t)std::max(c.intermediate, 3 * c.hidden);
    const size_t per_token = (size_t)c.n_in_embd * es + 3 * (size_t)c.hidden * 4 + 3 * (size_t)c.hidden * es + wide * es + 24;
    return std::max<int64_t>(131072, (int64_t)(((size_t)12 << 30) / per_token));
}

static WorkspaceSizes workspace_sizes(const zett_config& c, size_t es, int seq, int64_t Ttot, int64_t D, int64_t cap) {
    const int lam = c.embed_lang ? 1 : 0;
    WorkspaceSizes w{};
    if (cap <= 0) cap = chunk_token_cap(c, es);
    w.chunk_tokens = std::max<int64_t>(std::min<int64_t>(cap, std::max<int64_t>(Ttot, D)), seq + lam);
    const size_t MC = (size_t)w.chunk_tokens, MCS = MC + 768;
    const size_t wide = (size_t)std::max(c.intermediate, 3 * c.hidden);
    w.table = (size_t)D * c.hidden * 4;
    w.x0 = MCS * c.n_in_embd * es;
    w.f32_rows = MCS * c.hidden * 4;
    w.lo_rows = MCS * c.hidden * es;
    w.big = MCS * wide * es;
    w.stats = 2 * MCS * 2 * sizeof(float);
    return w;
}

struct PlanLayout {
    PlanArrays p{};
    int32_t* scan_tmp = nullptr;
    bool pair_plan = false;
    int64_t PK = 0;
    size_t n_clear = 0;
};
static PlanLayout plan_layout(const zett_hypernet* h, const zett_hypernet::PlanSlot& s, int64_t N, int seq) {
    const zett_config& c = h->cfg;
    const int lam = c.embed_lang ? 1 : 0;
    const int V = c.original_vocab_size + c.n_extra;
    const int64_t max_tok = N * (int64_t)(seq + lam);
    PlanLayout L;
    PlanArrays& p = L.p;
    L.PK = pair_keys(c, seq);
    L.pair_plan = h->pair_dedupe && c.layers >= 2 && L.PK <= std::max<int64_t>(4 * max_tok, (int64_t)1 << 23) && L.PK < (int64_t)0x7fffffff;
    int32_t* base = s.i32.as<int32_t>();
    p.id_flag = base; base += V;
    if (L.pair_plan) { p.pair_flag = base; base += L.PK; }
    p.err = base; base += 1;
    L.n_clear = (size_t)(base - s.i32.as<int32_t>());
    p.row_count = base; base += N;
    p.row_offset = base; base += N + 1;
    p.counters = base; base += 3;
    p.id_slot = base; base += V + 1;
    p.id_list = base; base += V;
    p.tok_slot = base; base += max_tok;
    p.tok_pos = base; base += max_tok;
    p.tok_row = base; base += max_tok;
    p.n_pair_keys = L.pair_plan ? (int32_t)L.PK : 0;
    if (L.pair_plan) {
        p.tok_pkey = base; base += max_tok;
        p.tok_pair = base; base += max_tok;
        p.pair_tslot = base; base += max_tok;
        p.pair_pos = base; base += max_tok;
        p.pair_slot = base; base += L.PK + 1;
    }
    L.scan_tmp = base;
    p.row_uniform = s.u8.as<uint8_t>();
    p.tok_key = p.row_uniform + N;
    return L;
}

static int enqueue_plan(zett_hypernet* h, zett_hypernet::PlanSlot& s, const int32_t* sfm, int64_t N, int seq, hipStream_t st) {
    const zett_config& c = h->cfg;
    const int lam = c.embed_lang ? 1 : 0;
    const int V = c.original_vocab_size + c.n_extra;
    const int64_t max_tok = N * (int64_t)(seq + lam);
    if (int rc = s.i32.reserve(plan_i32_bytes(c, N, seq))) return rc;
    if (int rc = s.u8.reserve((size_t)N + (size_t)max_tok)) return rc;
    const size_t need_ints = (size_t)N + 1 + 3;
    if (s.host_ints < need_ints) {
        if (s.host) (void)hipHostFree(s.host);
        s.host = nullptr;
        HIP_TRY(hipHostMalloc((void**)&s.host, need_ints * 4, hipHostMallocDefault));
        s.host_ints = need_ints;
    }
    if (!s.done) HIP_TRY(hipEventCreateWithFlags(&s.done, hipEventDisableTiming));
    if (!s.released) HIP_TRY(hipEventCreateWithFlags(&s.released, hipEventDisableTiming));
    const PlanLayout L = plan_layout(h, s, N, seq);
    const PlanArrays& p = L.p;
    HIP_TRY(hipMemsetAsync(s.i32.p, 0, L.n_clear * 4, st));
    const int rb = (int)((N + 255) / 256);
    hipLaunchKernelGGL(plan_rows_kernel, dim3(rb), dim3(256), 0, st, sfm, N, seq, c.pad_token_id, lam, V, p);
    launch_exclusive_scan(p.row_count, p.row_offset, N, L.scan_tmp, st);
    launch_exclusive_scan(p.id_flag, p.id_slot, (int64_t)V, L.scan_tmp, st);
    {
        PlanArrays pt = p;
        if (h->ext.id_slot) pt.id_slot = const_cast<int32_t*>(h->ext.id_slot);
        hipLaunchKernelGGL(plan_tokens_kernel, dim3(rb), dim3(256), 0, st, sfm, N, seq, c.pad_token_id, lam, V, pt);
    }
    if (L.pair_plan) {
        launch_exclusive_scan(p.pair_flag, p.pair_slot, L.PK, L.scan_tmp, st);
        hipLaunchKernelGGL(plan_pairs_kernel, dim3((unsigned)((max_tok + 255) / 256)), dim3(256), 0, st, N, p);
    }
    hipLaunchKernelGGL(plan_idlist_kernel, dim3((V + 255) / 256), dim3(256), 0, st, V, p);
    HIP_TRY(hipGetLastError());
    HIP_TRY(hipMemcpyAsync(s.host, p.row_offset, ((size_t)N + 1 + 3) * 4, hipMemcpyDeviceToHost, st));
    HIP_TRY(hipEventRecord(s.done, st));
    s.sfm = sfm; s.n_rows = N; s.seq = seq; s.pair_plan = L.pair_plan; s.ext_id_slot = h->ext.id_slot;
    return 0;
}

template <typename T>
int do_forward(zett_hypernet* h, const int32_t* sfm, int64_t N, int seq, const void* src, int src_dtype, const zett_dest* dest,
               int64_t v_src, int lang_index, float* out_in, float* out_out, float* out_bias, hipStream_t st);
template <typename T>
int do_table_rows(zett_hypernet* h, const int32_t* id_list, int first, int count, const void* src, int src_dtype, void* table_out, float* stats_out, hipStream_t st);

}

extern "C" {

const char* zett_last_error(void) { return g_err.c_str(); }
int zett_abi_version(void) { return ZETT_ABI_VERSION; }

int zett_create(const zett_config* cfg, int device, int precision, zett_hypernet** out) {
    if (!cfg || !out) return fail(ZETT_E_INVALID, "null argument");
    if (precision != ZETT_PREC_BF16 && precision != ZETT_PREC_F32 && precision != ZETT_PREC_F16) return fail(ZETT_E_INVALID, "unknown precision %d", precision);
    if (int rc = validate_config(*cfg, precision)) return rc;
    int ndev = 0;
    HIP_TRY(hipGetDeviceCount(&ndev));
    if (device < 0 || device >= ndev) return fail(ZETT_E_INVALID, "device %d out of range (%d visible)", device, ndev);
    ZETT_ON_DEVICE(device);
    auto* h = new zett_hypernet();
    h->cfg = *cfg;
    h->device = device;
    h->precision = precision;
    if (hipMalloc((void**)&h->range_word, 64) != hipSuccess || hipHostMalloc((void**)&h->range_host, 64, hipHostMallocDefault) != hipSuccess ||
        hipMemset(h->range_word, 0, 64) != hipSuccess) {
        if (h->range_word) (void)hipFree(h->range_word);
        if (h->range_host) (void)hipHostFree(h->range_host);
        delete h;
        return fail(ZETT_E_HIP, "allocation of the range word failed");
    }
    *out = h;
    return 0;
}

int zett_destroy(zett_hypernet* h) {
    if (!h) return 0;
    ::zett::DeviceScope _scope(h->device);
    for (auto& kv : h->w) {
        if (kv.second.f32) (void)hipFree(kv.second.f32);
        if (kv.second.lo && kv.second.lo != (void*)kv.second.f32) (void)hipFree(kv.second.lo);
    }
    for (void* p : h->owned) (void)hipFree(p);
    for (DevBuf* b : {&h->table, &h->x0, &h->yf, &h->yt, &h->big, &h->pre, &h->ctx, &h->cf, &h->ct, &h->lnstats, &h->lnparts, &h->dest_word, &h->dest_stage[0], &h->dest_stage[1], &h->dest_sink})
        b->release();
    for (zett_hypernet::PlanSlot* psp : {&h->plan[0], &h->plan[1], &h->table_plan}) {
        zett_hypernet::PlanSlot& ps = *psp;
        ps.i32.release(); ps.u8.release();
        if (ps.host) (void)hipHostFree(ps.host);
        if (ps.done) (void)hipEventDestroy(ps.done);
        if (ps.released) (void)hipEventDestroy(ps.released);
    }
    if (h->plan_stream) (void)hipStreamDestroy(h->plan_stream);
    if (h->plan_fork) (void)hipEventDestroy(h->plan_fork);
    if (h->range_word) (void)hipFree(h->range_word);
    if (h->range_host) (void)hipHostFree(h->range_host);
    if (h->dest_host) (void)hipHostFree(h->dest_host);
    if (h->dest_checked) (void)hipEventDestroy(h->dest_checked);
    for (hipEvent_t e : h->out_ready) if (e) (void)hipEventDestroy(e);
    for (hipEvent_t e : h->lane_ev) if (e) (void)hipEventDestroy(e);
    if (h->lane_stream) (void)hipStreamDestroy(h->lane_stream);
    for (hipEvent_t e : h->ev) (void)hipEventDestroy(e);
    delete h;
    return 0;
}

int zett_load_weight(zett_hypernet* h, const char* name, const void* data, int dtype, const int64_t* shape, int ndim) {
    if (!h || !name || !data || !shape || ndim < 1) return fail(ZETT_E_INVALID, "null argument");
    if (h->finalized) return fail(ZETT_E_STATE, "weights are frozen after zett_finalize");
    std::map<std::string, std::vector<int64_t>> exp;
    expected_shapes(h->cfg, exp);
    const std::string n(name);
    auto it = exp.find(n);
    if (it == exp.end()) return 0;
    std::vector<int64_t> got(shape, shape + ndim);
    if (got != it->second) {
        std::string a, b;
        for (auto v : got) a += std::to_string(v) + ",";
        for (auto v : it->second) b += std::to_string(v) + ",";
        return fail(ZETT_E_INVALID, "%s: shape [%s] does not match the config's [%s]", name, a.c_str(), b.c_str());
    }
    ZETT_ON_DEVICE(h->device);
    size_t numel = 1;
    for (auto v : got) numel *= (size_t)v;
    Tensor& t = h->w[n];
    if (t.f32) { (void)hipFree(t.f32); t.f32 = nullptr; }
    t.shape = got;
    t.numel = numel;
    HIP_TRY(hipMalloc((void**)&t.f32, numel * 4));
    if (dtype == ZETT_F32) {
        HIP_TRY(hipMemcpy(t.f32, data, numel * 4, hipMemcpyDefault));
    } else if (dtype == ZETT_F16 || dtype == ZETT_BF16) {
        void* stage = nullptr;
        HIP_TRY(hipMalloc(&stage, numel * 2));
        hipError_t e = hipMemcpy(stage, data, numel * 2, hipMemcpyDefault);
        if (e == hipSuccess) {
            const int blocks = (int)std::min<size_t>((numel + 255) / 256, 65535);
            if (dtype == ZETT_F16) hipLaunchKernelGGL(convert_to_f32_kernel<1>, dim3(blocks), dim3(256), 0, 0, stage, t.f32, numel);
            else hipLaunchKernelGGL(convert_to_f32_kernel<2>, dim3(blocks), dim3(256), 0, 0, stage, t.f32, numel);
            e = hipDeviceSynchronize();
        }
        (void)hipFree(stage);
        if (e != hipSuccess) return fail(ZETT_E_HIP, "upload of %s failed: %s", name, hipGetErrorString(e));
    } else {
        return fail(ZETT_E_INVALID, "unknown dtype %d", dtype);
    }
    return 0;
}

int zett_finalize(zett_hypernet* h) {
    if (!h) return fail(ZETT_E_INVALID, "null handle");
    if (h->finalized) return 0;
    ZETT_ON_DEVICE(h->device);
    std::map<std::string, std::vector<int64_t>> exp;
    expected_shapes(h->cfg, exp);
    for (auto& kv : exp)
        if (!h->w.count(kv.first)) return fail(ZETT_E_STATE, "missing weight: %s", kv.first.c_str());
    const zett_config& c = h->cfg;
    const size_t es = elt_size(h->precision);
    for (auto& kv : h->w) {
        Tensor& t = kv.second;
        if (!is_gemm_weight(kv.first)) continue;
        if (h->precision == ZETT_PREC_F32) { t.lo = t.f32; continue; }
        HIP_TRY(hipMalloc(&t.lo, t.numel * 2));
        const int blocks = (int)std::min<size_t>((t.numel / 4 + 255) / 256 + 1, 65535);
        if (h->precision == ZETT_PREC_F16)
            hipLaunchKernelGGL(convert_f32_to_lo_kernel<f16_t>, dim3(blocks), dim3(256), 0, 0, t.f32, (f16_t*)t.lo, t.numel, h->range_word);
        else
            hipLaunchKernelGGL(convert_f32_to_lo_kernel<bf16_t>, dim3(blocks), dim3(256), 0, 0, t.f32, (bf16_t*)t.lo, t.numel, h->range_word);
    }
    HIP_TRY(hipDeviceSynchronize());
    const size_t H = c.hidden;
    for (int l = 0; l < c.layers; ++l) {
        const std::string p = "model.encoder.layer." + std::to_string(l) + ".attention.self.";
        void* wq = nullptr; float* bq = nullptr;
        HIP_TRY(hipMalloc(&wq, 3 * H * H * es));
        HIP_TRY(hipMalloc((void**)&bq, 3 * H * 4));
        h->owned.push_back(wq); h->owned.push_back(bq);
        int k = 0;
        for (const char* q : {"query", "key", "value"}) {
            Tensor& tw = h->w[p + q + ".weight"];
            Tensor& tb = h->w[p + q + ".bias"];
            HIP_TRY(hipMemcpy((char*)wq + (size_t)k * H * H * es, tw.lo, H * H * es, hipMemcpyDeviceToDevice));
            HIP_TRY(hipMemcpy(bq + (size_t)k * H, tb.f32, H * 4, hipMemcpyDeviceToDevice));
            ++k;
        }
        h->qkv_w.push_back(wq);
        h->qkv_b.push_back(bq);
    }
    if (h->precision != ZETT_PREC_F32 && c.hidden % 128 == 0) {
        auto fold = [&](const float* w32, size_t N, size_t K, const float* gamma, const float* beta, const float* bias,
                        zett_hypernet::Folded& f) -> int {
            HIP_TRY(hipMalloc(&f.w, N * K * es));
            HIP_TRY(hipMalloc((void**)&f.c, N * 4));
            HIP_TRY(hipMalloc((void**)&f.b, N * 4));
            h->owned.push_back(f.w); h->owned.push_back(f.c); h->owned.push_back(f.b);
            if (h->precision == ZETT_PREC_F16)
                hipLaunchKernelGGL(fold_weight_kernel<f16_t>, dim3((unsigned)N), dim3(256), 0, 0, w32, (int)K, gamma, beta, bias, (f16_t*)f.w, f.c, f.b, h->range_word);
            else
                hipLaunchKernelGGL(fold_weight_kernel<bf16_t>, dim3((unsigned)N), dim3(256), 0, 0, w32, (int)K, gamma, beta, bias, (bf16_t*)f.w, f.c, f.b, h->range_word);
            return 0;
        };
        h->fold_qkv.resize(c.layers); h->fold_up.resize(c.layers);
        float* tmp = nullptr;
        HIP_TRY(hipMalloc((void**)&tmp, 3 * H * H * 4));
        for (int l = 0; l < c.layers; ++l) {
            const std::string lp = "model.encoder.layer." + std::to_string(l) + ".";
            if (int rc = fold(h->w[lp + "intermediate.dense.weight"].f32, c.intermediate, H, h->w[lp + "attention.output.LayerNorm.weight"].f32,
                              h->w[lp + "attention.output.LayerNorm.bias"].f32, h->w[lp + "intermediate.dense.bias"].f32, h->fold_up[l])) return rc;
            if (l == 0) continue;
            const std::string pp = "model.encoder.layer." + std::to_string(l - 1) + ".output.LayerNorm.";
            int k = 0;
            for (const char* q : {"query", "key", "value"}) {
                HIP_TRY(hipMemcpy(tmp + (size_t)k * H * H, h->w[lp + "attention.self." + q + ".weight"].f32, H * H * 4, hipMemcpyDeviceToDevice));
                ++k;
            }
            if (int rc = fold(tmp, 3 * H, H, h->w[pp + "weight"].f32, h->w[pp + "bias"].f32, h->qkv_b[l], h->fold_qkv[l])) return rc;
        }
        if (!(c.single_head && c.separate_out)) {
            const size_t w0 = c.single_head ? c.n_in_embd : c.n_embd;
            if (int rc = fold(h->w["output_projection.1.weight"].f32, w0, H, h->w["output_projection.0.ln.weight"].f32,
                              h->w["output_projection.0.ln.bias"].f32, h->w["output_projection.1.bias"].f32, h->fold_head_in)) return rc;
            if (c.separate_out && !c.single_head)
                if (int rc = fold(h->w["output_projection_out.1.weight"].f32, c.n_embd, H, h->w["output_projection_out.0.ln.weight"].f32,
                                  h->w["output_projection_out.0.ln.bias"].f32, h->w["output_projection_out.1.bias"].f32, h->fold_head_out)) return rc;
            std::vector<float> ones(w0, 1.0f), zeros(w0, 0.0f);
            HIP_TRY(hipMalloc((void**)&h->head_one, w0 * 4));
            HIP_TRY(hipMalloc((void**)&h->head_zero, w0 * 4));
            h->owned.push_back(h->head_one); h->owned.push_back(h->head_zero);
            HIP_TRY(hipMemcpy(h->head_one, ones.data(), w0 * 4, hipMemcpyHostToDevice));
            HIP_TRY(hipMemcpy(h->head_zero, zeros.data(), w0 * 4, hipMemcpyHostToDevice));
        }
        HIP_TRY(hipDeviceSynchronize());
        (void)hipFree(tmp);
    }
    HIP_TRY(hipMemcpy(h->range_host, h->range_word, 4, hipMemcpyDeviceToHost));
    if (h->range_host[0] & ZETT_RANGE_WEIGHT)
        return fail(ZETT_E_RANGE, "a GEMM weight (or a LayerNorm-folded weight W*gamma) exceeds the half range (|w| > 65504 or not finite): "
                                  "this checkpoint needs ZETT_PREC_BF16 or ZETT_PREC_F32");
    if (c.rescale) {
        const size_t w0 = c.single_head ? c.n_in_embd : c.n_embd;
        HIP_TRY(hipMalloc((void**)&h->head_scale, w0 * 4));
        HIP_TRY(hipMalloc((void**)&h->head_shift, w0 * 4));
        h->owned.push_back(h->head_scale); h->owned.push_back(h->head_shift);
        HIP_TRY(hipMemcpy(h->head_scale, h->w["scaler.w"].f32, c.n_embd * 4, hipMemcpyDeviceToDevice));
        HIP_TRY(hipMemcpy(h->head_shift, h->w["scaler.b"].f32, c.n_embd * 4, hipMemcpyDeviceToDevice));
        if (c.single_head && c.separate_out) {
            HIP_TRY(hipMemcpy(h->head_scale + c.n_embd, h->w["out_scaler.w"].f32, c.n_embd * 4, hipMemcpyDeviceToDevice));
            HIP_TRY(hipMemcpy(h->head_shift + c.n_embd, h->w["out_scaler.b"].f32, c.n_embd * 4, hipMemcpyDeviceToDevice));
        }
    }
    if (h->precision != ZETT_PREC_F32) {
        for (auto& kv : h->w) {
            Tensor& t = kv.second;
            if (is_gemm_weight(kv.first) && t.f32) { (void)hipFree(t.f32); t.f32 = nullptr; }
        }
    }
    h->finalized = true;
    return 0;
}

int zett_set_option(zett_hypernet* h, const char* key, int64_t value) {
    if (!h || !key) return fail(ZETT_E_INVALID, "null argument");
    const std::string k(key);
    if (k == "max_chunk_tokens") {
        if (value < 1024) return fail(ZETT_E_INVALID, "max_chunk_tokens must be >= 1024");
        h->max_chunk_tokens = value;
    } else if (k == "time_gemm") {
        h->time_gemm = value != 0;
    } else if (k == "cls_only_last_layer") {
        h->cls_only_last = value != 0;
    } else if (k == "pair_dedupe") {
        h->pair_dedupe = value != 0;
    } else if (k == "residual_lo") {
        if (value < 0 || value > 2) return fail(ZETT_E_INVALID, "residual_lo must be 0 (fp32 residual stream), 1 (16-bit stream in f16 mode) or 2 (in bf16 mode too)");
        h->residual_lo = (int)value;
    } else if (k == "concurrent_lanes") {
        if (value < 0 || value > 2) return fail(ZETT_E_INVALID, "concurrent_lanes must be 0 (never), 1 (auto) or 2 (whenever a call is one chunk of >= 512 rows)");
        h->concurrent_lanes = (int)value;
    } else if (k == "attention_fast") {
        h->attention_fast = value != 0;
    } else if (k == "ln_fold") {
        if (value < 0 || value > 2) return fail(ZETT_E_INVALID, "ln_fold must be 0 (off), 1 (encoder and output heads) or 2 (encoder only: A/B)");
        h->ln_fold = (int)value;
    } else if (k == "gemm_tail_split") {
        if (value < 0 || value > 3) return fail(ZETT_E_INVALID, "gemm_tail_split must be 0 (never), 1 (auto), 2 (cut every gemm4d launch in the middle) or 3 (128x256 tiles only)");
        h->gemm_tail_split = (int)value;
    } else if (k == "attention_pack") {
        h->attention_pack = value != 0;
    } else if (k == "ln_rows8") {
        h->ln_rows8 = value != 0;
    } else if (k == "table_lo") {
        h->table_lo = value != 0;
    } else if (k == "gemm_group") {
        if (value < 0 || value > 64) return fail(ZETT_E_INVALID, "gemm_group must be 0 (default: 4) .. 64");
        h->gemm_group = (int)value;
    } else if (k == "gemm_tile_order") {
        if (value < 0 || value > 1) return fail(ZETT_E_INVALID, "gemm_tile_order must be 0 or 1");
        h->gemm_tile_order = (int)value;
    } else if (k == "gemm4d_min_k") {
        if (value < 64) return fail(ZETT_E_INVALID, "gemm4d_min_k must be >= 64");
        h->gemm4d_min_k = (int)value;
    } else if (k == "range_accumulate") {
        h->range_accumulate = value != 0;
    } else if (k == "gemm_variant") {
        if (value != 0 && value != 1 && value != 2 && value != 3 && value != 7 && value != 8)
            return fail(ZETT_E_INVALID, "gemm_variant must be 0 (auto), 1 (128x128), 2 (256x256 register-staged), 3 (384x256), 7 (256x256 four-wave direct-to-LDS) or 8 (7 with the generic epilogue drain)");
        h->gemm_variant = (int)value;
    } else {
        return fail(ZETT_E_INVALID, "unknown option %s", key);
    }
    return 0;
}

int zett_workspace_bytes(const zett_hypernet* h, int64_t n_rows, int32_t seq, int64_t* out_bytes) {
    if (!h || !out_bytes) return fail(ZETT_E_INVALID, "null argument");
    if (n_rows < 0 || seq < 1) return fail(ZETT_E_INVALID, "bad surface-form shape [%lld, %d]", (long long)n_rows, seq);
    const zett_config& c = h->cfg;
    const int64_t V = (int64_t)c.original_vocab_size + c.n_extra;
    const int64_t max_tok = n_rows * (int64_t)(seq + (c.embed_lang ? 1 : 0));
    const WorkspaceSizes w = workspace_sizes(c, elt_size(h->precision), seq, max_tok, std::min<int64_t>(V, max_tok), h->max_chunk_tokens);
    const size_t parts = c.hidden % 128 == 0 ? (size_t)(c.hidden / 128) * ((size_t)w.chunk_tokens + 768) * 8 : 0;
    *out_bytes = (int64_t)(w.total() + parts + plan_i32_bytes(c, n_rows, seq) + (size_t)n_rows + (size_t)max_tok);
    return 0;
}

int zett_get_stats(const zett_hypernet* h, zett_stats* out) {
    if (!h || !out) return fail(ZETT_E_INVALID, "null argument");
    *out = h->stats;
    return 0;
}

int zett_stream_wait_output(zett_hypernet* h, int which, void* stream) {
    if (!h) return fail(ZETT_E_INVALID, "null handle");
    if (which != ZETT_OUT_IN && which != ZETT_OUT_BIAS) return fail(ZETT_E_INVALID, "which must be ZETT_OUT_IN or ZETT_OUT_BIAS");
    if (!h->out_recorded) return fail(ZETT_E_STATE, "no forward has run on this handle");
    ZETT_ON_DEVICE(h->device);
    HIP_TRY(hipStreamWaitEvent((hipStream_t)stream, h->out_ready[which], 0));
    return 0;
}

int zett_get_gemm_log(const zett_hypernet* h, zett_gemm_record* out, int64_t capacity, int64_t* count) {
    if (!h || !count || capacity < 0 || (capacity > 0 && !out)) return fail(ZETT_E_INVALID, "null argument");
    *count = (int64_t)h->gemm_log.size();
    for (int64_t i = 0; i < capacity && i < *count; ++i) out[i] = h->gemm_log[(size_t)i];
    return 0;
}

int zett_check_range(zett_hypernet* h, void* stream, int32_t* flags) {
    if (!h) return fail(ZETT_E_INVALID, "null handle");
    ZETT_ON_DEVICE(h->device);
    hipStream_t st = (hipStream_t)stream;
    HIP_TRY(hipMemcpyAsync(h->range_host, h->range_word, 4, hipMemcpyDeviceToHost, st));
    HIP_TRY(hipStreamSynchronize(st));
    const int32_t w = h->range_host[0];
    if (h->range_accumulate && w) HIP_TRY(hipMemsetAsync(h->range_word, 0, 4, st));
    if (flags) *flags = w;
    if (!w) return 0;
    return fail(ZETT_E_RANGE, "the last forward left the range of its arithmetic:%s%s%s%s (precision %s)",
                (w & ZETT_RANGE_SOURCE) ? " in_scaler(source_embeddings) beyond the half range;" : "",
                (w & ZETT_RANGE_ACTIVATION) ? " a 16-bit activation (Q/K/V, FFN intermediate or the operand copy of the residual sum) beyond the half range;" : "",
                (w & ZETT_RANGE_OUTPUT) ? " non-finite predicted embeddings;" : "",
                (w & ZETT_RANGE_DEST) ? " a finite value beyond the range of an f16 destination (stored as inf);" : "",
                h->precision == ZETT_PREC_F16 ? "f16: re-run with ZETT_PREC_BF16" : h->precision == ZETT_PREC_BF16 ? "bf16" : "f32");
}

int zett_partition_workspace_bytes(int64_t n_rows, int32_t n_ids, int64_t* out_bytes) {
    if (!out_bytes || n_rows < 0 || n_ids < 1) return fail(ZETT_E_INVALID, "bad argument");
    *out_bytes = (int64_t)partition_workspace_bytes(n_rows, n_ids);
    return 0;
}

int zett_partition_rows(const int32_t* surface_forms, int64_t n_rows, int32_t seq, int32_t pad_id, int32_t n_ids, int32_t world,
                        const int32_t* caps, int32_t* perm_out, void* workspace, int64_t workspace_bytes, int32_t device, void* stream) {
    if (n_rows < 0 || seq < 1 || n_ids < 1) return fail(ZETT_E_INVALID, "bad surface-form shape [%lld, %d] / id range %d", (long long)n_rows, seq, n_ids);
    if (world < 1 || world > PART_MAX_RANKS) return fail(ZETT_E_INVALID, "zett_partition_rows handles 1..%d ranks (one node), got %d", PART_MAX_RANKS, world);
    if (n_rows == 0) return 0;
    if (!surface_forms || !caps || !perm_out || !workspace) return fail(ZETT_E_INVALID, "null argument");
    if (n_rows >= (int64_t)0x7fffffff) return fail(ZETT_E_INVALID, "too many rows for one call");
    int64_t total = 0;
    for (int r = 0; r < world; ++r) { if (caps[r] < 0) return fail(ZETT_E_INVALID, "negative capacity"); total += caps[r]; }
    if (total != n_rows) return fail(ZETT_E_INVALID, "the ranks' capacities sum to %lld, the matrix has %lld rows", (long long)total, (long long)n_rows);
    if ((size_t)workspace_bytes < partition_workspace_bytes(n_rows, n_ids)) return fail(ZETT_E_INVALID, "workspace too small (zett_partition_workspace_bytes)");
    ZETT_ON_DEVICE(device);
    hipStream_t st = (hipStream_t)stream;
    const size_t have_bytes = ((size_t)(n_ids + 3) / 4) * 4 + 64;
    uint32_t* have = (uint32_t*)workspace;
    PartCaps caps_arg = {};
    for (int r = 0; r < world; ++r) caps_arg.v[r] = caps[r];
    HIP_TRY(hipMemsetAsync(have, 0, have_bytes, st));
    const size_t lds_have = ((size_t)(n_ids + 3) / 4) * 4;
    if (lds_have <= 150 * 1024) {
        static bool attr_set[64] = {};
        if (device >= 64 || !attr_set[device]) {
            HIP_TRY(hipFuncSetAttribute((const void*)partition_rows_kernel<true>, hipFuncAttributeMaxDynamicSharedMemorySize, 150 * 1024));
            if (device < 64) attr_set[device] = true;
        }
        hipLaunchKernelGGL(partition_rows_kernel<true>, dim3(1), dim3(PART_THREADS), lds_have, st, surface_forms, n_rows, (int)seq, (int)pad_id, (int)n_ids,
                           (int)world, caps_arg, have, perm_out);
    } else {
        hipLaunchKernelGGL(partition_rows_kernel<false>, dim3(1), dim3(PART_THREADS), 0, st, surface_forms, n_rows, (int)seq, (int)pad_id, (int)n_ids,
                           (int)world, caps_arg, have, perm_out);
    }
    HIP_TRY(hipGetLastError());
    return 0;
}

int zett_scatter_rows(const void* src, void* dst, const int64_t* order, int64_t n_rows, int64_t row_bytes, int32_t device, void* stream) {
    if (n_rows < 0 || row_bytes < 1) return fail(ZETT_E_INVALID, "bad shape");
    if (n_rows == 0) return 0;
    if (!src || !dst || !order) return fail(ZETT_E_INVALID, "null argument");
    if (row_bytes != 4 && row_bytes % 16 != 0) return fail(ZETT_E_INVALID, "row_bytes must be 4 or a multiple of 16, got %lld", (long long)row_bytes);
    if (((uintptr_t)src | (uintptr_t)dst) % (row_bytes == 4 ? 4 : 16)) return fail(ZETT_E_INVALID, "misaligned buffer");
    ZETT_ON_DEVICE(device);
    hipStream_t st = (hipStream_t)stream;
    if (row_bytes == 4)
        hipLaunchKernelGGL(scatter_words_kernel, dim3((unsigned)((n_rows + 255) / 256)), dim3(256), 0, st, (const uint32_t*)src, (uint32_t*)dst, order, n_rows);
    else
        hipLaunchKernelGGL(scatter_rows_kernel, dim3((unsigned)std::min<int64_t>(n_rows, 65535 * 16)), dim3(256), 0, st, (const unsigned char*)src, (unsigned char*)dst,
                           order, n_rows, row_bytes);
    HIP_TRY(hipGetLastError());
    return 0;
}

int zett_forward_prepare(zett_hypernet* h, const int32_t* surface_forms, int64_t n_rows, int32_t seq, void* input_stream) {
    if (!h) return fail(ZETT_E_INVALID, "null handle");
// ... 55 lines not shown
        for (hipEvent_t& e : h->out_ready) {
            if (!e) HIP_TRY(hipEventCreateWithFlags(&e, hipEventDisableTiming));
            HIP_TRY(hipEventRecord(e, (hipStream_t)stream));
        }
        h->out_recorded = true;
        return 0;
    }
    if (!surface_forms || !source_embeddings || (!dest && (!out_in || !out_bias))) return fail(ZETT_E_INVALID, "null tensor argument");
    const bool has_out = c.separate_out;
    if (!dest && has_out && !out_out) return fail(ZETT_E_INVALID, "out_out is required when separate_out_embeddings is set");
    if (src_dtype < ZETT_F32 || src_dtype > ZETT_BF16) return fail(ZETT_E_INVALID, "unknown source dtype %d", src_dtype);
    if (v_src < c.original_vocab_size) return fail(ZETT_E_INDEX, "source_embeddings has %lld rows, config.original_vocab_size is %d", (long long)v_src, c.original_vocab_size);
    if (c.embed_lang && (lang_index < 0 || lang_index >= c.n_langs)) return fail(ZETT_E_INDEX, "lang_index %d outside [0,%d)", lang_index, c.n_langs);
    if (n_rows * (int64_t)(seq + 1) >= (int64_t)0x7fffffff) return fail(ZETT_E_INVALID, "too many positions for one call");
    ZETT_ON_DEVICE(h->device);
    hipStream_t st = (hipStream_t)stream;
    if (h->precision == ZETT_PREC_F16)
        return do_forward<f16_t>(h, surface_forms, n_rows, seq, source_embeddings, src_dtype, dest, v_src, lang_index, out_in, out_out, out_bias, st);
    if (h->precision == ZETT_PREC_BF16)
        return do_forward<bf16_t>(h, surface_forms, n_rows, seq, source_embeddings, src_dtype, dest, v_src, lang_index, out_in, out_out, out_bias, st);
    return do_forward<float>(h, surface_forms, n_rows, seq, source_embeddings, src_dtype, dest, v_src, lang_index, out_in, out_out, out_bias, st);
}

}

extern "C" {

int zett_forward(zett_hypernet* h, const int32_t* surface_forms, int64_t n_rows, int32_t seq,
                 const void* source_embeddings, int src_dtype, int64_t v_src, int32_t lang_index,
                 float* out_in, float* out_out, float* out_bias, void* stream) {
    return forward_entry(h, surface_forms, n_rows, seq, source_embeddings, src_dtype, v_src, lang_index, nullptr, out_in, out_out, out_bias, stream);
}

int zett_forward_into(zett_hypernet* h, const int32_t* surface_forms, int64_t n_rows, int32_t seq, const void* source_embeddings, int src_dtype,
                      int64_t v_src, int32_t lang_index, const zett_dest* dest, void* stream) {
    if (!h) return fail(ZETT_E_INVALID, "null handle");
    if (int rc = check_dest(h, dest, n_rows)) return rc;
    return forward_entry(h, surface_forms, n_rows, seq, source_embeddings, src_dtype, v_src, lang_index, dest, nullptr, nullptr, nullptr, stream);
}

int zett_table_plan(zett_hypernet* h, const int32_t* surface_forms, int64_t n_rows, int32_t seq, int32_t* id_slot_out, int32_t* id_list_out,
                    int64_t* n_ids_out, void* stream) {
    if (!h) return fail(ZETT_E_INVALID, "null handle");
    if (!h->finalized) return fail(ZETT_E_STATE, "zett_finalize has not been called");
    if (!surface_forms || !id_slot_out || !id_list_out || !n_ids_out) return fail(ZETT_E_INVALID, "null argument");
    if (n_rows < 1 || seq < 1) return fail(ZETT_E_INVALID, "bad surface-form shape [%lld, %d]", (long long)n_rows, seq);
    if (n_rows * (int64_t)(seq + 1) >= (int64_t)0x7fffffff) return fail(ZETT_E_INVALID, "too many positions for one call");
    const zett_config& c = h->cfg;
    const int V = c.original_vocab_size + c.n_extra;
    ZETT_ON_DEVICE(h->device);
    hipStream_t st = (hipStream_t)stream;
    zett_hypernet::PlanSlot& ps = h->table_plan;
    const zett_hypernet::ExtTable saved = h->ext;
    h->ext = zett_hypernet::ExtTable{};
    const int rc = enqueue_plan(h, ps, surface_forms, n_rows, seq, st);
    h->ext = saved;
    if (rc) return rc;
    HIP_TRY(hipEventSynchronize(ps.done));
    const int32_t* hoff = ps.host;
    if (hoff[n_rows + 2] != 0)
        return fail(ZETT_E_INDEX, "surface-form row %d holds an id outside [0, %d) (original_vocab_size %d + %d fallback rows)",
                    hoff[n_rows + 2] - 1, V, c.original_vocab_size, c.n_extra);
    const int D = hoff[n_rows + 1];
    const PlanLayout L = plan_layout(h, ps, n_rows, seq);
    HIP_TRY(hipMemcpyAsync(id_slot_out, L.p.id_slot, ((size_t)V + 1) * 4, hipMemcpyDeviceToDevice, st));
    if (D > 0) HIP_TRY(hipMemcpyAsync(id_list_out, L.p.id_list, (size_t)D * 4, hipMemcpyDeviceToDevice, st));
    *n_ids_out = D;
    return 0;
}

int zett_table_rows(zett_hypernet* h, const int32_t* id_list, int64_t first, int64_t count, const void* source_embeddings, int src_dtype,
                    int64_t v_src, void* table_out, float* stats_out, void* stream) {
    if (!h) return fail(ZETT_E_INVALID, "null handle");
    if (!h->finalized) return fail(ZETT_E_STATE, "zett_finalize has not been called");
    if (first < 0 || count < 0 || first + count >= (int64_t)0x7fffffff) return fail(ZETT_E_INVALID, "bad table range [%lld, +%lld)", (long long)first, (long long)count);
    if (count == 0) return 0;
    if (!id_list || !source_embeddings || !table_out || !stats_out) return fail(ZETT_E_INVALID, "null tensor argument");
    if (src_dtype < ZETT_F32 || src_dtype > ZETT_BF16) return fail(ZETT_E_INVALID, "unknown source dtype %d", src_dtype);
    if (v_src < h->cfg.original_vocab_size) return fail(ZETT_E_INDEX, "source_embeddings has %lld rows, config.original_vocab_size is %d", (long long)v_src, h->cfg.original_vocab_size);
    ZETT_ON_DEVICE(h->device);
    hipStream_t st = (hipStream_t)stream;
    if (h->precision == ZETT_PREC_F16) return do_table_rows<f16_t>(h, id_list, (int)first, (int)count, source_embeddings, src_dtype, table_out, stats_out, st);
    if (h->precision == ZETT_PREC_BF16) return do_table_rows<bf16_t>(h, id_list, (int)first, (int)count, source_embeddings, src_dtype, table_out, stats_out, st);
    return fail(ZETT_E_INVALID, "zett_table_rows: the folded 16-bit table exists in the 16-bit modes only");
}

}

namespace {
int forward_table_entry(zett_hypernet* h, const int32_t* surface_forms, int64_t n_rows, int32_t seq, const void* table, const float* table_stats,
                        const int32_t* id_slot, int32_t lang_index, const zett_dest* dest, float* out_in, float* out_out, float* out_bias, void* stream) {
    if (!h) return fail(ZETT_E_INVALID, "null handle");
    if (!h->finalized) return fail(ZETT_E_STATE, "zett_finalize has not been called");
    const zett_config& c = h->cfg;
    if (n_rows < 1 || seq < 1) return fail(ZETT_E_INVALID, "bad surface-form shape [%lld, %d]", (long long)n_rows, seq);
    if (seq + (c.embed_lang ? 1 : 0) > c.max_positions) return fail(ZETT_E_INDEX, "sequence %d exceeds position_embeddings (%d rows)", seq, c.max_positions);
    if (!surface_forms || !table || !table_stats || !id_slot || (!dest && (!out_in || !out_bias))) return fail(ZETT_E_INVALID, "null tensor argument");
    if (!dest && c.separate_out && !out_out) return fail(ZETT_E_INVALID, "out_out is required when separate_out_embeddings is set");
    if (c.embed_lang && (lang_index < 0 || lang_index >= c.n_langs)) return fail(ZETT_E_INDEX, "lang_index %d outside [0,%d)", lang_index, c.n_langs);
    if (n_rows * (int64_t)(seq + 1) >= (int64_t)0x7fffffff) return fail(ZETT_E_INVALID, "too many positions for one call");
    if (h->precision == ZETT_PREC_F32) return fail(ZETT_E_INVALID, "zett_forward_table: the folded 16-bit table exists in the 16-bit modes only");
    ZETT_ON_DEVICE(h->device);
    hipStream_t st = (hipStream_t)stream;
    h->ext.table = table; h->ext.stats = table_stats; h->ext.id_slot = id_slot;
    int rc;
    if (h->precision == ZETT_PREC_F16)
        rc = do_forward<f16_t>(h, surface_forms, n_rows, seq, nullptr, ZETT_F32, dest, 0, lang_index, out_in, out_out, out_bias, st);
    else
        rc = do_forward<bf16_t>(h, surface_forms, n_rows, seq, nullptr, ZETT_F32, dest, 0, lang_index, out_in, out_out, out_bias, st);
    h->ext = zett_hypernet::ExtTable{};
    return rc;
}

}

extern "C" {

int zett_forward_table(zett_hypernet* h, const int32_t* surface_forms, int64_t n_rows, int32_t seq, const void* table, const float* table_stats,
                       const int32_t* id_slot, int32_t lang_index, float* out_in, float* out_out, float* out_bias, void* stream) {
    return forward_table_entry(h, surface_forms, n_rows, seq, table, table_stats, id_slot, lang_index, nullptr, out_in, out_out, out_bias, stream);
}

int zett_forward_table_into(zett_hypernet* h, const int32_t* surface_forms, int64_t n_rows, int32_t seq, const void* table, const float* table_stats,
                            const int32_t* id_slot, int32_t lang_index, const zett_dest* dest, void* stream) {
    if (!h) return fail(ZETT_E_INVALID, "null handle");
    if (int rc = check_dest(h, dest, n_rows)) return rc;
    return forward_table_entry(h, surface_forms, n_rows, seq, table, table_stats, id_slot, lang_index, dest, nullptr, nullptr, nullptr, stream);
}

}

namespace {

template <typename T>
struct Runner {
    zett_hypernet* h;
    hipStream_t st;
    int rc = 0;

    const Tensor& W(const std::string& n) { return h->w.at(n); }
    const T* Wlo(const std::string& n) { return (const T*)h->w.at(n).lo; }
    const float* Wf(const std::string& n) { return h->w.at(n).f32; }

    GemmEpilogue<T> epi() {
        GemmEpilogue<T> e{};
        e.split_col = 0x7fffffff;
        e.range_flag = h->range_word;
        return e;
    }

    long a_rows_readable = 0;
    bool staged_dst = false;
    int stage_lane = 0;

    int variant_for(int M, int N, int K, const GemmEpilogue<T>& e) const {
    constexpr bool is_f32 = std::is_same<T, float>::value;
    int variant = h->gemm_variant;
    if (variant == 0) {
        variant = (M > 128 && N > 128) ? 2 : 1;
        if (variant != 1 && N % 256 == 0 && !e.scale && !e.residual) {
            const long t256 = (long)((M + 255) / 256) * (N / 256), t384 = (long)((M + 383) / 384) * (N / 256);
            const double c256 = (double)((t256 + 255) / 256), c384 = 1.7 * (double)((t384 + 255) / 256);
            if (c384 < c256) variant = 3;
        }
    }
    if (variant == 3 && (N % 256 != 0 || (long)((M + 383) / 384) * 384 > a_rows_readable || e.scale || e.shift || e.residual || e.range_final)) variant = 2;
    if (h->gemm_variant == 0 && variant == 2 && !is_f32 && K >= h->gemm4d_min_k) variant = 7;
    if ((variant == 7 || variant == 8) && is_f32) variant = 2;
    const bool wide_ok = N % 8 == 0 && (!e.out_lo || e.ld_lo % 8 == 0) && e.ld_f32 % 4 == 0 && (!e.residual || e.ld_res % 4 == 0) &&
                         (e.split_col >= N || e.split_col % 8 == 0);
    if (variant != 1 && !wide_ok) variant = 1;
    if (e.residual && (e.scale || e.shift)) variant = 1;
    if (e.stats_part || e.fold_stats) variant = 7;
        return variant;
    }


    void gemm(const T* A, int lda, const T* Wp, int ldw, int M, int N, int K, const GemmEpilogue<T>& e) {
        if (rc || M <= 0) return;
        GemmArgs<T> g{A, lda, Wp, ldw, M, N, K, e};
        g.tile_order = h->gemm_tile_order;
        g.group = h->gemm_group;
        g.row0 = h->gemm_tail_split == 1 ? -1 : h->gemm_tail_split == 2 ? ((M / 2 + 255) / 256) * 256 : h->gemm_tail_split == 3 ? -2 : 0;
        const double fl = 2.0 * (double)M * (double)N * (double)K;
        hipEvent_t e0 = nullptr, e1 = nullptr;
        if (h->time_gemm) {
            while (h->ev.size() < h->ev_used + 2) {
                hipEvent_t ev;
                if (hipEventCreate(&ev) != hipSuccess) { rc = fail(ZETT_E_HIP, "hipEventCreate failed"); return; }
                h->ev.push_back(ev);
            }
            e0 = h->ev[h->ev_used++];
            e1 = h->ev[h->ev_used++];
            h->ev_flops.push_back(fl);
            h->ev_shape.push_back({M, N, K, 0});
            (void)hipEventRecord(e0, st);
        }
        const int variant = variant_for(M, N, K, e);
        if (h->time_gemm && !h->ev_shape.empty()) h->ev_shape.back()[3] = variant;
        {
            zett_gemm_record r{};
            r.m = M; r.n = N; r.k = K; r.variant = variant;
            r.epilogue = (e.out_lo ? 1 : 0) | ((e.out_f32 || e.out_f32_b) ? 2 : 0) | (e.residual ? 4 : 0) | ((e.scale || e.shift) ? 8 : 0) |
                         (e.stats_part ? 16 : 0) | (e.fold_stats ? 32 : 0) | (e.residual_lo ? 64 : 0) | (e.act << 8) |
                         (e.dst ? 1024 : 0) | (staged_dst ? 2048 : 0);
            r.flops = fl;
            const double mn = (double)M * (double)N;
            const double dst_es = e.dst_dtype == ZETT_F32 ? 4.0 : 2.0;
            r.bytes = ((double)M + (double)N) * (double)K * sizeof(T) + (e.out_lo ? mn * sizeof(T) : 0.0) + ((e.out_f32 || e.out_f32_b) ? mn * 4.0 : 0.0) +
                      (e.dst ? mn * dst_es : 0.0) +
                      (e.residual ? mn * 4.0 : 0.0) + (e.residual_lo ? mn * sizeof(T) : 0.0) + (e.stats_part ? (double)M * (N / 128) * 8.0 : 0.0) + ((e.fold_stats || e.res_stats) ? (double)M * 8.0 : 0.0);
            h->gemm_log.push_back(r);
        }
        const hipError_t err = launch_gemm_variant(variant, g, st);
        if (h->time_gemm) (void)hipEventRecord(e1, st);
        if (err != hipSuccess) { rc = fail(ZETT_E_HIP, "gemm launch failed: %s", hipGetErrorString(err)); return; }
        h->stats.executed_flops += fl;
        h->stats.gemm_launches += 1;
    }

    struct DestOut { void* p; const int64_t* rows; int64_t ld; int dtype; };

    void head_gemm(const T* A, const T* Wp, int M, int N, int K, const GemmEpilogue<T>& e, const DestOut* d, const DestOut* d_b, int split) {
        if (rc || M <= 0) return;
        if (!d) { gemm(A, K, Wp, K, M, N, K, e); return; }
        GemmEpilogue<T> ed = e;
        ed.out_f32 = nullptr; ed.out_f32_b = nullptr; ed.ld_f32 = N;
        ed.dst = d->p; ed.dst_rows = d->rows; ed.ld_dst = d->ld; ed.dst_dtype = d->dtype;
        const GemmArgs<T> probe{A, K, Wp, K, M, N, K, ed};
        if (!d_b && variant_for(M, N, K, ed) == 7 && gemm_4d_dst_mode(probe) >= 0) { gemm(A, K, Wp, K, M, N, K, ed); return; }
        DevBuf& stage_buf = h->dest_stage[stage_lane];
        if (int r = stage_buf.reserve((size_t)M * (size_t)N * sizeof(float))) { rc = r; return; }
        float* S = stage_buf.as<float>();
        GemmEpilogue<T> es = e;
        es.out_f32 = S; es.ld_f32 = N;
        if (d_b) es.out_f32_b = S + split;
        staged_dst = true;
        gemm(A, K, Wp, K, M, N, K, es);
        staged_dst = false;
        dest_store(S, N, *d, M, d_b ? split : N);
        if (d_b) dest_store(S + split, N, *d_b, M, N - split);
    }

    void dest_store(const float* S, int64_t ld_s, const DestOut& d, int rows, int cols) {
        if (rc || rows <= 0) return;
        const bool vec = cols % 4 == 0 && ld_s % 4 == 0 && d.ld % 4 == 0 && (uintptr_t)S % 16 == 0 && (uintptr_t)d.p % (d.dtype == ZETT_F32 ? 16 : 8) == 0;
        const dim3 grid((unsigned)std::min<int64_t>(rows, 65535 * 16));
#define ZETT_DEST_STORE(OT) do { if (vec) hipLaunchKernelGGL((dest_store_rows_kernel<OT, true>), grid, dim3(256), 0, st, S, ld_s, (OT*)d.p, d.ld, d.rows, (int64_t)rows, cols, h->range_word); \
                                 else hipLaunchKernelGGL((dest_store_rows_kernel<OT, false>), grid, dim3(256), 0, st, S, ld_s, (OT*)d.p, d.ld, d.rows, (int64_t)rows, cols, h->range_word); } while (0)
        if (d.dtype == ZETT_F16) ZETT_DEST_STORE(f16_t);
        else if (d.dtype == ZETT_BF16) ZETT_DEST_STORE(bf16_t);
        else ZETT_DEST_STORE(float);
#undef ZETT_DEST_STORE
        check("dest_store");
    }

    template <typename BT>
    void readout_dst(const float* in, int rows, const float* gamma, const float* beta, float eps, float* of, T* ol, const LnReadout& readout) {
        const int H = h->cfg.hidden;
        if constexpr (sizeof(T) == 2) {
            const int tpr8 = h->ln_rows8 ? ln_rows8_tpr(H) : 0;
            if (tpr8) {
                const dim3 grid8((rows + 256 / tpr8 - 1) / (256 / tpr8));
                if (tpr8 == 32) hipLaunchKernelGGL((layernorm_rows8_kernel<T, false, 32, true, BT>), grid8, dim3(256), 0, st, in, H, rows, H, gamma, beta, eps, of, ol, (float*)nullptr, (float*)nullptr, LnEmbed{}, 0, readout);
                else hipLaunchKernelGGL((layernorm_rows8_kernel<T, false, 64, true, BT>), grid8, dim3(256), 0, st, in, H, rows, H, gamma, beta, eps, of, ol, (float*)nullptr, (float*)nullptr, LnEmbed{}, 0, readout);
                check("readout");
                return;
            }
        }
        if (H <= 2048) hipLaunchKernelGGL((layernorm_rows_kernel<T, false, 64, true, BT>), dim3((rows + 3) / 4), dim3(256), 0, st, in, H, rows, H, gamma, beta, eps, of, ol, (float*)nullptr, (float*)nullptr, LnEmbed{}, 0, readout);
        else hipLaunchKernelGGL((layernorm_rows_kernel<T, false, 256, true, BT>), dim3(rows), dim3(256), 0, st, in, H, rows, H, gamma, beta, eps, of, ol, (float*)nullptr, (float*)nullptr, LnEmbed{}, 0, readout);
        check("readout");
    }

    void check(const char* what) {
        if (rc) return;
        hipError_t e = hipGetLastError();
        if (e != hipSuccess) rc = fail(ZETT_E_HIP, "%s launch failed: %s", what, hipGetErrorString(e));
    }

    void layernorm(const float* in, int rows, const float* gamma, const float* beta, float eps, float* of, T* ol, float* stats = nullptr,
                   LnReadout readout = LnReadout{}, const T* in_lo = nullptr, int bias_dtype = -1) {
        if (rc || rows <= 0) return;
        readout.in_lo = in_lo;
        if (bias_dtype >= 0 && readout.out_bias) {
            if (bias_dtype == ZETT_F16) readout_dst<f16_t>(in, rows, gamma, beta, eps, of, ol, readout);
            else if (bias_dtype == ZETT_BF16) readout_dst<bf16_t>(in, rows, gamma, beta, eps, of, ol, readout);
            else readout_dst<float>(in, rows, gamma, beta, eps, of, ol, readout);
            return;
        }
        const int H = h->cfg.hidden;
        if constexpr (sizeof(T) == 2) {
            const int tpr8 = h->ln_rows8 ? ln_rows8_tpr(H) : 0;
            if (tpr8) {
                const dim3 grid8((rows + 256 / tpr8 - 1) / (256 / tpr8));
#define ZETT_LN8_LAUNCH(TPR, RO) hipLaunchKernelGGL((layernorm_rows8_kernel<T, false, TPR, RO>), grid8, dim3(256), 0, st, in, H, rows, H, gamma, beta, eps, of, ol, stats, (float*)nullptr, LnEmbed{}, 0, readout)
                if (readout.out_bias) { if (tpr8 == 32) ZETT_LN8_LAUNCH(32, true); else ZETT_LN8_LAUNCH(64, true); }
                else { if (tpr8 == 32) ZETT_LN8_LAUNCH(32, false); else ZETT_LN8_LAUNCH(64, false); }
#undef ZETT_LN8_LAUNCH
                check("layernorm");
                return;
            }
        }
        const dim3 grid = H <= 2048 ? dim3((rows + 3) / 4) : dim3(rows);
#define ZETT_LN_LAUNCH(TPR, RO) hipLaunchKernelGGL((layernorm_rows_kernel<T, false, TPR, RO>), grid, dim3(256), 0, st, in, H, rows, H, gamma, beta, eps, of, ol, stats, (float*)nullptr, LnEmbed{}, 0, readout)
        if (readout.out_bias) { if (H <= 2048) ZETT_LN_LAUNCH(64, true); else ZETT_LN_LAUNCH(256, true); }
        else { if (H <= 2048) ZETT_LN_LAUNCH(64, false); else ZETT_LN_LAUNCH(256, false); }
#undef ZETT_LN_LAUNCH
        check("layernorm");
    }

    void ln_stats(const float2* parts, int ld_part, int rows, float eps, float* stats) {
        if (rc || rows <= 0) return;
        hipLaunchKernelGGL(ln_stats_kernel, dim3((rows + 63) / 64), dim3(64), 0, st, parts, h->cfg.hidden / 128, ld_part, rows,
                           h->cfg.hidden, eps, stats);
        check("ln_stats");
    }

    void projector(const std::string& p, const T* x_lo, const float* x_f32, int rows, T* big, float* pre, float* of, T* ol,
                   float2* fold_parts = nullptr, int ld_part = 0, float* fold_stats = nullptr) {
        const zett_config& c = h->cfg;
        GemmEpilogue<T> e1 = epi();
        e1.bias = Wf(p + "dense1.bias"); e1.act = ACT_GELU_TANH; e1.out_lo = big; e1.ld_lo = c.intermediate;
        gemm(x_lo, c.hidden, Wlo(p + "dense1.weight"), c.hidden, rows, c.intermediate, c.hidden, e1);
        GemmEpilogue<T> e2 = epi();
        e2.bias = Wf(p + "dense2.bias"); e2.act = ACT_GELU_TANH; e2.residual = x_f32; e2.ld_res = c.hidden;
        e2.ld_f32 = c.hidden;
        if (fold_parts) { e2.out_lo = ol; e2.ld_lo = c.hidden; e2.stats_part = fold_parts; e2.ld_part = ld_part; }
        else e2.out_f32 = pre;
        gemm(big, c.intermediate, Wlo(p + "dense2.weight"), c.intermediate, rows, c.hidden, c.intermediate, e2);
        if (fold_parts) ln_stats(fold_parts, ld_part, rows, c.ln_eps_projector, fold_stats);
        else layernorm(pre, rows, Wf(p + "ln.weight"), Wf(p + "ln.bias"), c.ln_eps_projector, of, ol);
    }
};

template <typename T, int SD>
void launch_gather(hipStream_t st, const int32_t* id_list, int s0, int m, const void* src, const zett_config& c,
                   const float* fallback, const float* sw, const float* sb, T* out, int32_t* range_flag) {
    hipLaunchKernelGGL((gather_src_kernel<T, SD>), dim3(m), dim3(256), 0, st, id_list, s0, m, src, c.n_in_embd,
                       c.original_vocab_size, fallback, sw, sb, out, range_flag);
}

template <typename T>
void table_phase(Runner<T>& R, const int32_t* id_list, int first, int count, const void* src, int src_dtype, int64_t MC, size_t MCS,
                 T* X0, float* Zf, T* Zt, T* BIG, float* PRE, float2* PARTS, bool table_lo, T* tbl16, float* tblst, float* tbl32) {
    zett_hypernet* h = R.h;
    const zett_config& c = h->cfg;
    const int H = c.hidden, EIN = c.n_in_embd;
    hipStream_t st = R.st;
    const float* in_w = c.rescale ? R.Wf("in_scaler.w") : nullptr;
    const float* in_b = c.rescale ? R.Wf("in_scaler.b") : nullptr;
    for (int s0 = first; s0 < first + count && !R.rc; s0 += (int)MC) {
        const int m = (int)std::min<int64_t>(MC, first + count - s0);
        const float* fb = R.Wf("fallback_embeddings.weight");
        if (src_dtype == ZETT_F32) launch_gather<T, 0>(st, id_list, s0, m, src, c, fb, in_w, in_b, X0, h->range_word);
        else if (src_dtype == ZETT_F16) launch_gather<T, 1>(st, id_list, s0, m, src, c, fb, in_w, in_b, X0, h->range_word);
        else launch_gather<T, 2>(st, id_list, s0, m, src, c, fb, in_w, in_b, X0, h->range_word);
        R.check("gather_src");
        GemmEpilogue<T> e0 = R.epi();
        e0.bias = R.Wf("input_projection.0.bias"); e0.out_f32 = Zf; e0.ld_f32 = H; e0.out_lo = Zt; e0.ld_lo = H;
        R.gemm(X0, EIN, R.Wlo("input_projection.0.weight"), EIN, m, H, EIN, e0);
        if (table_lo) R.projector("input_projection.1.", Zt, Zf, m, BIG, PRE, nullptr, tbl16 + (size_t)s0 * H, PARTS, (int)MCS, tblst + 2 * (size_t)s0);
        else R.projector("input_projection.1.", Zt, Zf, m, BIG, PRE, tbl32 + (size_t)s0 * H, nullptr);
    }
}

template <typename T>
bool folded_table_mode(const zett_hypernet* h) {
    const zett_config& c = h->cfg;
    const int H = c.hidden;
    const bool fold = h->ln_fold && !std::is_same<T, float>::value && h->gemm_variant == 0 && H % 128 == 0 && H >= 512 && (int)h->fold_up.size() == c.layers;
    const bool lo_stream = fold && c.layers >= 1 && sizeof(T) == 2 && (h->residual_lo == 2 || (h->residual_lo == 1 && std::is_same<T, f16_t>::value));
    return lo_stream && h->table_lo != 0;
}

template <typename T>
int do_table_rows(zett_hypernet* h, const int32_t* id_list, int first, int count, const void* src, int src_dtype, void* table_out, float* stats_out, hipStream_t st) {
    const zett_config& c = h->cfg;
    if (!folded_table_mode<T>(h))
        return fail(ZETT_E_INVALID, "zett_table_rows needs the folded 16-bit table: f16 arithmetic with the LayerNorm fold, the 16-bit residual stream and table_lo on");
    const WorkspaceSizes ws = workspace_sizes(c, sizeof(T), 1, count, count, h->max_chunk_tokens);
    const int64_t MC = ws.chunk_tokens;
    const size_t MCS = (size_t)MC + 768;
    if (int rc = h->x0.reserve(ws.x0)) return rc;
    if (int rc = h->yf.reserve(ws.f32_rows)) return rc;
    if (int rc = h->yt.reserve(ws.lo_rows)) return rc;
    if (int rc = h->big.reserve(ws.big)) return rc;
    if (int rc = h->pre.reserve(ws.f32_rows)) return rc;
    if (int rc = h->lnparts.reserve((size_t)(c.hidden / 128) * MCS * sizeof(float2))) return rc;
    Runner<T> R{h, st};
    R.a_rows_readable = (long)MCS;
    struct NoTiming { zett_hypernet* h; int saved; ~NoTiming() { h->time_gemm = saved; } } no_timing{h, h->time_gemm};
    h->time_gemm = 0;
    table_phase<T>(R, id_list, first, count, src, src_dtype, MC, MCS, h->x0.as<T>(), h->yf.as<float>(), h->yt.as<T>(), h->big.as<T>(), h->pre.as<float>(),
                   h->lnparts.as<float2>(), true, (T*)table_out, stats_out, nullptr);
    return R.rc;
}

template <typename T>
int do_forward(zett_hypernet* h, const int32_t* sfm, int64_t N, int seq, const void* src, int src_dtype, const zett_dest* dest,
               int64_t v_src, int lang_index, float* out_in, float* out_out, float* out_bias, hipStream_t st) {
    (void)v_src;
    const zett_config& c = h->cfg;
    const int H = c.hidden, I = c.intermediate, E = c.n_embd, EIN = c.n_in_embd;
    const int lam = c.embed_lang ? 1 : 0;
    const int V = c.original_vocab_size + c.n_extra;
    const int64_t max_tok = N * (int64_t)(seq + lam);
    h->stats = zett_stats{};
    h->stats.rows = N;
    h->ev_used = 0;
    h->ev_flops.clear();
    h->ev_shape.clear();
    h->gemm_log.clear();

    zett_hypernet::PlanSlot& ps = h->plan[h->plan_cur ^ 1];
    if (ps.pending && ps.sfm == sfm && ps.n_rows == N && ps.seq == seq && ps.pair_plan == plan_layout(h, ps, N, seq).pair_plan &&
        ps.ext_id_slot == h->ext.id_slot) {
        HIP_TRY(hipStreamWaitEvent(st, ps.done, 0));
    } else {
        if (ps.pending) HIP_TRY(hipEventSynchronize(ps.done));
        if (ps.released) HIP_TRY(hipStreamWaitEvent(st, ps.released, 0));
        if (int rc = enqueue_plan(h, ps, sfm, N, seq, st)) return rc;
    }
    ps.pending = false;
    h->plan_cur ^= 1;
    struct SlotGuard {
        zett_hypernet* h; zett_hypernet::PlanSlot* ps; hipStream_t st; bool lane_forked = false;
        ~SlotGuard() {
            if (lane_forked && h->lane_stream && h->lane_ev[3]) {
                (void)hipEventRecord(h->lane_ev[3], h->lane_stream);
                (void)hipStreamWaitEvent(st, h->lane_ev[3], 0);
            }
            if (ps->released) (void)hipEventRecord(ps->released, st);
        }
    } slot_guard{h, &ps, st};
    const PlanLayout PL = plan_layout(h, ps, N, seq);
    const PlanArrays& p = PL.p;
    const bool pair_plan = PL.pair_plan;
    if (!h->range_accumulate) HIP_TRY(hipMemsetAsync(h->range_word, 0, 4, st));
    for (hipEvent_t& e : h->out_ready)
        if (!e) HIP_TRY(hipEventCreateWithFlags(&e, hipEventDisableTiming));
    const bool dest_check = dest && dest->rows;
    if (dest_check) {
        if (int rc = h->dest_word.reserve(4)) return rc;
        if (!h->dest_host) HIP_TRY(hipHostMalloc((void**)&h->dest_host, 4, hipHostMallocDefault));
        if (!h->dest_checked) HIP_TRY(hipEventCreateWithFlags(&h->dest_checked, hipEventDisableTiming));
        HIP_TRY(hipMemsetAsync(h->dest_word.p, 0, 4, st));
        hipLaunchKernelGGL(dest_rows_check_kernel, dim3((unsigned)((N + 255) / 256)), dim3(256), 0, st, dest->rows, N, dest->n_dest_rows, h->dest_word.as<int32_t>());
        HIP_TRY(hipGetLastError());
        HIP_TRY(hipMemcpyAsync(h->dest_host, h->dest_word.p, 4, hipMemcpyDeviceToHost, st));
        HIP_TRY(hipEventRecord(h->dest_checked, st));
    }
    HIP_TRY(hipEventSynchronize(ps.done));
    int32_t* hoff = ps.host;
    if (hoff[N + 2] != 0)
        return fail(ZETT_E_INDEX, "surface-form row %d holds an id outside [0, %d) (original_vocab_size %d + %d fallback rows)",
                    hoff[N + 2] - 1, V, c.original_vocab_size, c.n_extra);
    if (dest_check) {
        HIP_TRY(hipEventSynchronize(h->dest_checked));
        if (h->dest_host[0] != 0)
            return fail(ZETT_E_INDEX, "destination row map: rows[%d] is outside the destination's %lld rows", h->dest_host[0] - 1, (long long)dest->n_dest_rows);
    }
    const int64_t Ttot = hoff[N];
    const int D = hoff[N + 1];
    h->stats.packed_tokens = Ttot;
    h->stats.distinct_ids = D;
    h->stats.distinct_positions = Ttot;

    const WorkspaceSizes ws = workspace_sizes(c, sizeof(T), seq, Ttot, D, h->max_chunk_tokens);
    const int64_t MC = ws.chunk_tokens;
    const size_t MCS = (size_t)MC + 768;
    if (int rc = h->table.reserve(ws.table)) return rc;
    if (int rc = h->x0.reserve(ws.x0)) return rc;
    if (int rc = h->yf.reserve(ws.f32_rows)) return rc;
    if (int rc = h->yt.reserve(ws.lo_rows)) return rc;
    if (int rc = h->big.reserve(ws.big)) return rc;
    if (int rc = h->pre.reserve(ws.f32_rows)) return rc;
    if (int rc = h->ctx.reserve(ws.lo_rows)) return rc;
    if (int rc = h->cf.reserve(ws.f32_rows)) return rc;
    if (int rc = h->ct.reserve(ws.lo_rows)) return rc;
    if (int rc = h->lnstats.reserve(ws.stats)) return rc;
    const bool fold = h->ln_fold && !std::is_same<T, float>::value && h->gemm_variant == 0 && H % 128 == 0 && H >= 512 &&
                      (int)h->fold_up.size() == c.layers;
    const bool lo_stream = fold && c.layers >= 1 && sizeof(T) == 2 &&
                           (h->residual_lo == 2 || (h->residual_lo == 1 && std::is_same<T, f16_t>::value));
    const size_t ws_parts = fold ? (size_t)(H / 128) * MCS * sizeof(float2) : 0;
    if (int rc = h->lnparts.reserve(ws_parts)) return rc;
    float2* PARTS = h->lnparts.as<float2>();
    float* TBL = h->table.as<float>();
    const bool table_lo = lo_stream && h->table_lo != 0;
    const bool ext_table = h->ext.table != nullptr;
    if (ext_table && !table_lo)
        return fail(ZETT_E_INVALID, "zett_forward_table needs the folded 16-bit table: f16 arithmetic with the LayerNorm fold, the 16-bit residual stream and table_lo on");
    T* TBL16 = ext_table ? (T*)const_cast<void*>(h->ext.table) : (T*)h->table.as<float>();
    float* TBLST = ext_table ? const_cast<float*>(h->ext.stats) : (float*)((char*)h->table.as<float>() + (((size_t)D * H * sizeof(T) + 15) / 16) * 16);
    T* X0 = h->x0.as<T>();
    float* Zf = h->yf.as<float>();
    T* Zt = h->yt.as<T>();
    T* BIG = h->big.as<T>();
    float* PRE = h->pre.as<float>();
    T* CTX = h->ctx.as<T>();
    float* Cf = h->cf.as<float>();
    T* Ct = h->ct.as<T>();
    float* STa = h->lnstats.as<float>();
    float* STb = STa + 2 * MCS;

    Runner<T> R{h, st};
    R.a_rows_readable = (long)MCS;

    if (!ext_table)
        table_phase<T>(R, p.id_list, 0, D, src, src_dtype, MC, MCS, X0, Zf, Zt, BIG, PRE, PARTS, table_lo, TBL16, TBLST, TBL);
    if (R.rc) return R.rc;

    const float* lang_vec = lam ? R.Wf("lang_embeddings.weight") + (size_t)lang_index * H : nullptr;
    const float scaling = 1.0f / std::sqrt((float)(H / c.heads));
    struct Lane { hipStream_t st; size_t off; };
    auto dest_out = [&](void* base, int64_t ld, int64_t r0) {
        const size_t es = dest->dtype == ZETT_F32 ? 4 : 2;
        return typename Runner<T>::DestOut{dest->rows ? base : (void*)((char*)base + (size_t)r0 * (size_t)ld * es), dest->rows ? dest->rows + r0 : nullptr, ld, dest->dtype};
    };
    const size_t ld_parts = MCS;
    auto run_chunk = [&](int64_t r0, int64_t r1, const Lane& lane, int ev_mode) -> int {
        const int rows = (int)(r1 - r0);
        const int tok0 = hoff[r0];
        const int m = hoff[r1] - tok0;
        h->stats.chunks += 1;
        hipStream_t st = lane.st;
        R.st = lane.st;
        R.stage_lane = ev_mode == 2 ? 1 : 0;
        R.a_rows_readable = (long)(MCS - lane.off);
        float* const Zf = h->yf.as<float>() + lane.off * H;
        T* const Zt = h->yt.as<T>() + lane.off * H;
        T* const BIG = h->big.as<T>() + lane.off * (size_t)std::max(I, 3 * H);
        float* const PRE = h->pre.as<float>() + lane.off * H;
        T* const CTX = h->ctx.as<T>() + lane.off * H;
        float* const Cf = h->cf.as<float>() + lane.off * H;
        T* const Ct = h->ct.as<T>() + lane.off * H;
        float* const STa = h->lnstats.as<float>() + 2 * lane.off;
        float* const STb = STa + 2 * MCS;
        float2* const PARTS = h->lnparts.as<float2>() + lane.off;

        LnEmbed emb{TBL, p.tok_slot, p.tok_pos, R.Wf("model.embeddings.token_type_embeddings.weight"),
                    R.Wf("model.embeddings.position_embeddings.weight"), lang_vec, seq, p.tok_row, p.row_offset, r0, rows,
                    table_lo ? (const void*)TBL16 : nullptr, TBLST, R.Wf("input_projection.1.ln.weight"), R.Wf("input_projection.1.ln.bias")};
        float* hs_sum = Zf;
        float* hs_stats = STb;
        const float* hs_gamma = R.Wf("model.embeddings.LayerNorm.weight");
        const float* hs_beta = R.Wf("model.embeddings.LayerNorm.bias");
        auto embed_ln = [&](const LnEmbed& e, int n, int t0, T* lo, float* stats, float* sum) {
            if constexpr (sizeof(T) == 2) {
                const int tpr8 = h->ln_rows8 ? ln_rows8_tpr(H) : 0;
                if (tpr8) {
                    const dim3 grid8((n + 256 / tpr8 - 1) / (256 / tpr8));
                    if (tpr8 == 32)
                        hipLaunchKernelGGL((layernorm_rows8_kernel<T, true, 32, false>), grid8, dim3(256), 0, st, (const float*)nullptr, H, n, H,
                                           hs_gamma, hs_beta, c.ln_eps_encoder, (float*)nullptr, lo, stats, sum, e, t0, LnReadout{});
                    else
                        hipLaunchKernelGGL((layernorm_rows8_kernel<T, true, 64, false>), grid8, dim3(256), 0, st, (const float*)nullptr, H, n, H,
                                           hs_gamma, hs_beta, c.ln_eps_encoder, (float*)nullptr, lo, stats, sum, e, t0, LnReadout{});
                    R.check("embed_layernorm");
                    return;
                }
            }
            if (H <= 2048)
                hipLaunchKernelGGL((layernorm_rows_kernel<T, true, 64>), dim3((n + 3) / 4), dim3(256), 0, st, (const float*)nullptr, H, n, H,
                                   hs_gamma, hs_beta, c.ln_eps_encoder, (float*)nullptr, lo, stats, sum, e, t0, LnReadout{});
            else
                hipLaunchKernelGGL((layernorm_rows_kernel<T, true, 256>), dim3(n), dim3(256), 0, st, (const float*)nullptr, H, n, H,
                                   hs_gamma, hs_beta, c.ln_eps_encoder, (float*)nullptr, lo, stats, sum, e, t0, LnReadout{});
            R.check("embed_layernorm");
        };
        const int P = pair_plan ? hoff[N + 3] : 0;
        const bool pairs = pair_plan && rows == N && P > 0 && (int64_t)P * 100 <= (int64_t)m * 85;
        int32_t* brow_pair = p.tok_pkey;
        if (pairs) {
            LnEmbed pe = emb;
            pe.tok_slot = p.pair_tslot; pe.tok_pos = p.pair_pos; pe.tok_row = nullptr;
            embed_ln(pe, P, 0, Zt, hs_stats, lo_stream ? (float*)nullptr : hs_sum);
            hipLaunchKernelGGL(pair_rows_kernel, dim3((m + 255) / 256), dim3(256), 0, st, m, tok0, r0, rows, p, brow_pair);
            R.check("pair_rows");
            h->stats.distinct_positions = P;
        } else {
            embed_ln(emb, m, tok0, Zt, hs_stats, lo_stream ? (float*)nullptr : hs_sum);
        }

        int zrows = m;
        bool raw = false;
        auto other = [&](float* b) { return b == Zf ? PRE : Zf; };
        auto other_stats = [&](float* b) { return b == STa ? STb : STa; };
        for (int l = 0; l < c.layers && !R.rc; ++l) {
            const std::string lp = "model.encoder.layer." + std::to_string(l) + ".";
            const bool last = l == c.layers - 1;
            const bool cls_only = h->cls_only_last && last;
            const T* wqkv = raw ? (const T*)h->fold_qkv[l].w : (const T*)h->qkv_w[l];
            const float* bqkv = raw ? h->fold_qkv[l].b : h->qkv_b[l];
            const float* cqkv = raw ? h->fold_qkv[l].c : nullptr;
            const int64_t waves = attention_waves(rows, H, h->attention_pack != 0).total;
            const int att_flags = (h->attention_fast ? 2 : 0) | (h->attention_pack ? 4 : 0);
            if (!cls_only) {
                const bool by_pair = pairs && l == 0;
                GemmEpilogue<T> eq = R.epi();
                eq.bias = bqkv; eq.out_lo = BIG; eq.ld_lo = 3 * H;
                if (raw) { eq.fold_stats = hs_stats; eq.fold_c = cqkv; }
                R.gemm(Zt, H, wqkv, H, by_pair ? P : m, 3 * H, H, eq);
                hipLaunchKernelGGL((attention_rows_kernel<T>), dim3((unsigned)((waves + 3) / 4)), dim3(256), 0, st,
                                   (const T*)BIG, (size_t)3 * H, (const T*)BIG + H, (const T*)BIG + 2 * H, (size_t)3 * H,
                                   H, H / c.heads, p.row_offset, p.row_uniform, p.tok_key, r0, rows, tok0, scaling, 0 | att_flags,
                                   by_pair ? (const int32_t*)p.tok_pair : (const int32_t*)nullptr, CTX);
                R.check("attention");
            } else {
                T* KV = BIG;
                T* Q = BIG + (size_t)m * 2 * H;
                GemmEpilogue<T> ekv = R.epi();
                ekv.bias = bqkv + H; ekv.out_lo = KV; ekv.ld_lo = 2 * H;
                if (raw) { ekv.fold_stats = hs_stats; ekv.fold_c = cqkv + H; }
                R.gemm(Zt, H, wqkv + (size_t)H * H, H, m, 2 * H, H, ekv);
                GemmEpilogue<T> eq = R.epi();
                eq.bias = bqkv; eq.out_lo = Q; eq.ld_lo = H;
                if (raw) { eq.fold_stats = hs_stats; eq.fold_c = cqkv; }
                R.gemm(Zt, H, wqkv, H, rows, H, H, eq);
                hipLaunchKernelGGL((attention_rows_kernel<T>), dim3((unsigned)((waves + 3) / 4)), dim3(256), 0, st,
                                   (const T*)Q, (size_t)H, (const T*)KV, (const T*)KV + H, (size_t)2 * H,
                                   H, H / c.heads, p.row_offset, p.row_uniform, p.tok_key, r0, rows, tok0, scaling, 1 | att_flags,
                                   (const int32_t*)nullptr, CTX);
                R.check("attention(position 0)");
                zrows = rows;
            }
            float* s1 = other(hs_sum);
            float* st1 = other_stats(hs_stats);
            GemmEpilogue<T> eo = R.epi();
            eo.bias = R.Wf(lp + "attention.output.dense.bias");
            if (pairs && l == 0) eo.res_index = brow_pair;
            if (lo_stream) {
                eo.residual_lo = Zt; eo.ld_res_lo = H;
                if (raw) { eo.res_stats = hs_stats; eo.res_gamma = hs_gamma; eo.res_beta = hs_beta; }
                eo.out_lo = Ct; eo.ld_lo = H; eo.stats_part = PARTS; eo.ld_part = (int)ld_parts;
            } else {
                eo.residual = hs_sum; eo.ld_res = H;
                eo.res_stats = hs_stats; eo.res_gamma = hs_gamma; eo.res_beta = hs_beta;
                eo.out_f32 = s1; eo.ld_f32 = H;
                if (fold) { eo.out_lo = Zt; eo.ld_lo = H; eo.stats_part = PARTS; eo.ld_part = (int)ld_parts; }
            }
            R.gemm(CTX, H, R.Wlo(lp + "attention.output.dense.weight"), H, zrows, H, H, eo);
            const float* g1 = R.Wf(lp + "attention.output.LayerNorm.weight");
            const float* b1 = R.Wf(lp + "attention.output.LayerNorm.bias");
            const T* mid = lo_stream ? Ct : Zt;
            GemmEpilogue<T> ei = R.epi();
            ei.act = ACT_GELU_ERF; ei.out_lo = BIG; ei.ld_lo = I;
            if (fold) {
                R.ln_stats(PARTS, (int)ld_parts, zrows, c.ln_eps_encoder, st1);
                ei.bias = h->fold_up[l].b; ei.fold_stats = st1; ei.fold_c = h->fold_up[l].c;
                R.gemm(mid, H, (const T*)h->fold_up[l].w, H, zrows, I, H, ei);
            } else {
                R.layernorm(s1, zrows, g1, b1, c.ln_eps_encoder, nullptr, Zt, st1);
                ei.bias = R.Wf(lp + "intermediate.dense.bias");
                R.gemm(Zt, H, R.Wlo(lp + "intermediate.dense.weight"), H, zrows, I, H, ei);
            }
            float* s2 = other(s1);
            float* st2 = other_stats(st1);
            GemmEpilogue<T> ef = R.epi();
            ef.bias = R.Wf(lp + "output.dense.bias");
            if (lo_stream) {
                ef.residual_lo = Ct; ef.ld_res_lo = H; ef.res_stats = st1; ef.res_gamma = g1; ef.res_beta = b1;
                ef.out_lo = Zt; ef.ld_lo = H; ef.stats_part = PARTS; ef.ld_part = (int)ld_parts;
            } else {
                ef.residual = s1; ef.ld_res = H;
                ef.res_stats = st1; ef.res_gamma = g1; ef.res_beta = b1;
                ef.out_f32 = s2; ef.ld_f32 = H;
                if (fold && !last) { ef.out_lo = Zt; ef.ld_lo = H; ef.stats_part = PARTS; ef.ld_part = (int)ld_parts; }
            }
            R.gemm(BIG, I, R.Wlo(lp + "output.dense.weight"), I, zrows, H, I, ef);
            hs_gamma = R.Wf(lp + "output.LayerNorm.weight");
            hs_beta = R.Wf(lp + "output.LayerNorm.bias");
            hs_sum = s2; hs_stats = st2;
            if (!last) {
                if (fold) { R.ln_stats(PARTS, (int)ld_parts, zrows, c.ln_eps_encoder, st2); raw = true; }
                else R.layernorm(s2, zrows, hs_gamma, hs_beta, c.ln_eps_encoder, nullptr, Zt, st2);
            }
        }
        if (R.rc) return R.rc;

        float* bias_out = out_bias ? out_bias + r0 : nullptr;
        const int64_t* bias_rows = nullptr;
        int bias_dtype = -1;
        if (dest && dest->bias) {
            const size_t bes = dest->bias_dtype == ZETT_F32 ? 4 : 2;
            bias_rows = dest->rows ? dest->rows + r0 : nullptr;
            bias_out = (float*)((char*)dest->bias + (dest->rows ? 0 : (size_t)r0 * bes));
            bias_dtype = dest->bias_dtype;
        } else if (dest) {
            if (int rc = h->dest_sink.reserve((size_t)N * sizeof(float))) return rc;
            bias_out = h->dest_sink.as<float>() + r0;
        }
        LnReadout ro{c.predict_bias ? R.Wf("bias_projection.weight") : (const float*)nullptr,
                     c.predict_bias ? R.Wf("bias_projection.bias") : (const float*)nullptr, bias_out};
        ro.bias_rows = bias_rows;
        ro.range_flag = h->range_word;
        R.layernorm(hs_sum, rows, hs_gamma, hs_beta, c.ln_eps_encoder, Cf, Ct, nullptr, ro,
                    lo_stream ? (const T*)Zt : (const T*)nullptr, bias_dtype);
        R.check("readout");
        if (!R.rc) {
            if (ev_mode == 2) HIP_TRY(hipEventRecord(h->lane_ev[1], st));
            if (ev_mode == 3) HIP_TRY(hipStreamWaitEvent(st, h->lane_ev[1], 0));
            if (ev_mode == 1 || ev_mode == 3) HIP_TRY(hipEventRecord(h->out_ready[ZETT_OUT_BIAS], st));
        }

        const bool fold_heads = fold && h->ln_fold == 1 && h->fold_head_in.w != nullptr;
        {
            if (fold_heads) R.projector("output_projection.0.", Ct, Cf, rows, BIG, PRE, nullptr, CTX, PARTS, (int)ld_parts, STa);
            else R.projector("output_projection.0.", Ct, Cf, rows, BIG, PRE, nullptr, CTX);
            GemmEpilogue<T> e = R.epi();
            e.bias = fold_heads ? h->fold_head_in.b : R.Wf("output_projection.1.bias");
            e.scale = c.rescale ? h->head_scale : (fold_heads ? h->head_one : nullptr);
            e.shift = c.rescale ? h->head_shift : (fold_heads ? h->head_zero : nullptr);
            if (fold_heads) { e.fold_stats = STa; e.fold_c = h->fold_head_in.c; }
            e.ld_f32 = E; e.range_final = 1;
            const int width = c.single_head ? EIN : E;
            const bool split = c.single_head && c.separate_out;
            if (!dest) {
                e.out_f32 = out_in + (size_t)r0 * E;
                if (split) { e.split_col = E; e.out_f32_b = out_out + (size_t)r0 * E; }
            } else if (split) {
                e.split_col = E;
            }
            const T* w1 = fold_heads ? (const T*)h->fold_head_in.w : R.Wlo("output_projection.1.weight");
            if (dest) {
                const typename Runner<T>::DestOut din = dest_out(dest->in, dest->ld_in, r0), dout = dest_out(dest->out, dest->ld_out, r0);
                R.head_gemm(CTX, w1, rows, width, H, e, &din, split ? &dout : nullptr, E);
            } else {
                R.gemm(CTX, H, w1, H, rows, width, H, e);
            }
            if (!R.rc) {
                if (ev_mode == 2) HIP_TRY(hipEventRecord(h->lane_ev[2], st));
                if (ev_mode == 3) HIP_TRY(hipStreamWaitEvent(st, h->lane_ev[2], 0));
                if (ev_mode == 1 || ev_mode == 3) HIP_TRY(hipEventRecord(h->out_ready[ZETT_OUT_IN], st));
            }
        }
        if (c.separate_out && !c.single_head) {
            if (fold_heads) R.projector("output_projection_out.0.", Ct, Cf, rows, BIG, PRE, nullptr, CTX, PARTS, (int)ld_parts, STa);
            else R.projector("output_projection_out.0.", Ct, Cf, rows, BIG, PRE, nullptr, CTX);
            GemmEpilogue<T> e = R.epi();
            e.bias = fold_heads ? h->fold_head_out.b : R.Wf("output_projection_out.1.bias");
            e.scale = c.rescale ? R.Wf("out_scaler.w") : (fold_heads ? h->head_one : nullptr);
            e.shift = c.rescale ? R.Wf("out_scaler.b") : (fold_heads ? h->head_zero : nullptr);
            if (fold_heads) { e.fold_stats = STa; e.fold_c = h->fold_head_out.c; }
            e.ld_f32 = E; e.range_final = 1;
            const T* w2 = fold_heads ? (const T*)h->fold_head_out.w : R.Wlo("output_projection_out.1.weight");
            if (dest) {
                const typename Runner<T>::DestOut dout = dest_out(dest->out, dest->ld_out, r0);
                R.head_gemm(CTX, w2, rows, E, H, e, &dout, nullptr, E);
            } else {
                e.out_f32 = out_out + (size_t)r0 * E;
                R.gemm(CTX, H, w2, H, rows, E, H, e);
            }
        }
        return R.rc;
    };
    bool two_lanes = false;
    if (h->concurrent_lanes && Ttot <= MC && N >= 512) {
        const int Pn = pair_plan ? hoff[N + 3] : 0;
        const bool pairs_taken = pair_plan && Pn > 0 && (int64_t)Pn * 100 <= Ttot * 85;
        const double r = (double)((Ttot + 255) / 256) * (double)((H + 255) / 256) / 256.0;
        two_lanes = h->concurrent_lanes == 2 ||
                    (!pairs_taken && !h->time_gemm && H >= 1024 && r < 4.0 && (std::ceil(r) - r) / std::ceil(r) > 0.08);
    }
    if (two_lanes) {
        if (!h->lane_stream) HIP_TRY(hipStreamCreateWithFlags(&h->lane_stream, hipStreamNonBlocking));
        for (hipEvent_t& e : h->lane_ev)
            if (!e) HIP_TRY(hipEventCreateWithFlags(&e, hipEventDisableTiming));
        int64_t ra = ((N / 2 + 128) / 256) * 256;
        ra = std::min<int64_t>(std::max<int64_t>(ra, 256), N - 1);
        const size_t off1 = (size_t)(hoff[ra] - hoff[0]) + 384;
        HIP_TRY(hipEventRecord(h->lane_ev[0], st));
        HIP_TRY(hipStreamWaitEvent(h->lane_stream, h->lane_ev[0], 0));
        slot_guard.lane_forked = true;
        if (int rc = run_chunk(ra, N, Lane{h->lane_stream, off1}, 2)) return rc;
        if (int rc = run_chunk(0, ra, Lane{st, 0}, 3)) return rc;
// ... 46 lines not shown
```

Baseline: 621,800.

## Skip Q/K projections for single-token rows via gathered-row QKV GEMM

Rows whose decomposition has only one token need no attention scores, because softmax over a single key equals the value. The QKV projection is therefore split into a V GEMM over all rows and a Q/K GEMM over only the multi-token rows, gathered through a new a_index row indirection in the 4d GEMM kernel. The attention kernel copies V directly for single-key rows. This adds planning kernels, scans and extra index arrays, and forces the 4d GEMM variant. It also risks lower GEMM efficiency from splitting one wide GEMM into two or three narrower ones.

```diff
diff --git a/zett_amd/csrc/gemm.hip.h b/zett_amd/csrc/gemm.hip.h
--- a/zett_amd/csrc/gemm.hip.h
+++ b/zett_amd/csrc/gemm.hip.h
@@ -252,6 +252,8 @@
     int tile_order = 0;
     int group = 0;
     int row0 = 0;
+    const int32_t* a_index = nullptr;
+    int a_rows = 0;
 };
 
 constexpr int GEMM_BM = 128;
diff --git a/zett_amd/csrc/gemm4d.hip.h b/zett_amd/csrc/gemm4d.hip.h
--- a/zett_amd/csrc/gemm4d.hip.h
+++ b/zett_amd/csrc/gemm4d.hip.h
@@ -105,7 +105,7 @@
     const int wave = __builtin_amdgcn_readfirstlane(tid >> 6);
     const int wm = wave >> 1, wn = wave & 1;
 
-    const unsigned char* a_base = (const unsigned char*)(g.A + (size_t)m0 * g.lda);
+    const unsigned char* a_base = (const unsigned char*)(g.a_index ? g.A : g.A + (size_t)m0 * g.lda);
     const unsigned char* w_base = (const unsigned char*)(g.W + (size_t)n0 * g.ldw);
     uint32_t a_voff[8], w_voff[8];
 #pragma unroll
@@ -120,6 +120,7 @@
         const int row = wave * (GEO::AREQ * 8) + r * 8 + (lane >> 3);
         const int chunk = ((lane & 7) ^ ((row >> 1) & 7)) << 4;
         int ar = row; ar = m0 + ar < g.M ? ar : g.M - 1 - m0;
+        if (g.a_index) ar = g.a_index[m0 + ar];
         a_voff[r] = (uint32_t)ar * (uint32_t)g.lda * (uint32_t)sizeof(T) + chunk;
     }
     const __amdgpu_buffer_rsrc_t a_rsrc = __builtin_amdgcn_make_buffer_rsrc((void*)a_base, (short)0, 0x7fffffff, G4R_RSRC_WORD3);
@@ -431,6 +432,7 @@
 #pragma unroll
             for (int p = 0; p < GEO::NPASS; ++p) {
                 int srow = m0 + wm * GEO::WROWS + p * 64 + lane_e; srow = srow < g.M ? srow : g.M - 1;
+                if (g.a_index) srow = g.a_index[srow];
                 fst[p] = *(const float2*)(e.fold_stats + 2 * (size_t)srow);
             }
         }
@@ -817,6 +819,7 @@
     const bool dst = g.epi.dst != nullptr;
     const int mode = dst ? gemm4d_dst_mode(g) : (force_generic && !g.epi.stats_part && !g.epi.fold_stats) ? G4D_EPI_GENERIC : gemm4d_epi_mode(g);
     if (mode < 0) return hipErrorInvalidValue;
+    if (g.a_index && ((size_t)g.a_rows * (size_t)g.lda * sizeof(T) > (size_t)0x7fffffff || g.a_rows <= 0)) return hipErrorInvalidValue;
     int split = g.row0 == -1 ? gemm4d_row_split(g.M, g.N) : (g.row0 == -2 ? 0 : (g.row0 > 0 ? std::min(g.row0, g.M) : g.M));
     if (split < g.M && (!gemm4d_half_ok(g, mode) || split % G256_BM != 0)) split = g.M;
     GemmArgs<T> full = g;
diff --git a/zett_amd/csrc/gemm_launch.hip b/zett_amd/csrc/gemm_launch.hip
--- a/zett_amd/csrc/gemm_launch.hip
+++ b/zett_amd/csrc/gemm_launch.hip
@@ -4,14 +4,16 @@
 
 hipError_t launch_gemm_variant(int variant, const GemmArgs<f16_t>& g, hipStream_t stream) {
     if (variant == 7 || variant == 8) return launch_gemm_4d(g, stream, variant == 8);
+    if (g.a_index) return hipErrorInvalidValue;
     return launch_gemm_x(variant, g, stream);
 }
 hipError_t launch_gemm_variant(int variant, const GemmArgs<bf16_t>& g, hipStream_t stream) {
     if (variant == 7 || variant == 8) return launch_gemm_4d(g, stream, variant == 8);
+    if (g.a_index) return hipErrorInvalidValue;
     return launch_gemm_x(variant, g, stream);
 }
 hipError_t launch_gemm_variant(int variant, const GemmArgs<float>& g, hipStream_t stream) {
-    if (variant == 7 || variant == 8) return hipErrorInvalidValue;
+    if (variant == 7 || variant == 8 || g.a_index) return hipErrorInvalidValue;
     return launch_gemm_x(variant, g, stream);
 }
 
diff --git a/zett_amd/csrc/rowops.hip.h b/zett_amd/csrc/rowops.hip.h
--- a/zett_amd/csrc/rowops.hip.h
+++ b/zett_amd/csrc/rowops.hip.h
@@ -30,6 +30,15 @@
     int32_t* err;
     int32_t* counters;
     int32_t n_pair_keys;
+    int32_t* row_multi;
+    int32_t* multi_off;
+    int32_t* qk_rows;
+    int32_t* tok_qk;
+    int32_t* pair_qk_flag;
+    int32_t* pair_qk_slot;
+    int32_t* pair_qk_rows;
+    int32_t* tok_qk0;
+    int32_t n_pair_qk;
 };
 
 __global__ void plan_rows_kernel(const int32_t* __restrict__ sfm, int64_t n_rows, int seq, int pad, int lam,
@@ -43,6 +52,7 @@
         if (id < 0 || id >= n_ids) {
             atomicMax(p.err, (int)(n < 0x7ffffffe ? n + 1 : 0x7fffffff));
             p.row_count[n] = 0;
+            if (p.row_multi) p.row_multi[n] = 0;
             p.row_uniform[n] = 2;
             return;
         }
@@ -60,6 +70,7 @@
     }
     p.row_count[n] = count;
     p.row_uniform[n] = uniform ? 1 : 0;
+    if (p.row_multi) p.row_multi[n] = count >= 2 ? 1 : 0;
 }
 
 __global__ __launch_bounds__(1024) void exclusive_scan_kernel(const int32_t* __restrict__ in,
@@ -184,6 +195,31 @@
     brow_pair[chunk_row(t, (int)(n - row0), p.row_offset[n] == tok0 + t, rows)] = p.tok_pair[tok0 + t];
 }
 
+__global__ void plan_pair_qk_mark_kernel(int64_t n_rows, PlanArrays p) {
+    const int64_t t = (int64_t)blockIdx.x * blockDim.x + threadIdx.x;
+    if (t >= p.row_offset[n_rows]) return;
+    if (p.row_multi[p.tok_row[t]]) p.pair_qk_flag[p.tok_pair[t]] = 1;
+}
+__global__ void plan_pair_qk_kernel(int64_t n_rows, PlanArrays p) {
+    const int64_t t = (int64_t)blockIdx.x * blockDim.x + threadIdx.x;
+    if (t >= p.row_offset[n_rows]) return;
+    p.tok_qk0[t] = p.row_multi[p.tok_row[t]] ? p.pair_qk_slot[p.tok_pair[t]] : -1;
+    if (t < p.pair_slot[p.n_pair_keys] && p.pair_qk_flag[t]) p.pair_qk_rows[p.pair_qk_slot[t]] = (int32_t)t;
+}
+
+__global__ void qk_rows_kernel(int m, int tok0, int64_t row0, int rows, int rq, PlanArrays p) {
+    const int t = blockIdx.x * blockDim.x + threadIdx.x;
+    if (t >= m) return;
+    const int n = p.tok_row[tok0 + t];
+    int q = -1;
+    if (p.row_multi[n]) {
+        const bool first = p.row_offset[n] == tok0 + t;
+        q = first ? p.multi_off[n] - p.multi_off[row0] : rq + t - (int)(n - row0) - 1;
+        p.qk_rows[tok0 + q] = chunk_row(t, (int)(n - row0), first, rows);
+    }
+    p.tok_qk[tok0 + t] = q;
+}
+
 __global__ void plan_idlist_kernel(int n_ids, PlanArrays p) {
     const int id = blockIdx.x * blockDim.x + threadIdx.x;
     if (id < n_ids && p.id_flag[id]) p.id_list[p.id_slot[id]] = id;
@@ -191,6 +227,7 @@
         p.counters[0] = p.id_slot[n_ids];
         p.counters[1] = p.err[0];
         p.counters[2] = p.n_pair_keys ? p.pair_slot[p.n_pair_keys] : 0;
+        p.counters[3] = p.n_pair_qk ? p.pair_qk_slot[p.n_pair_qk] : 0;
     }
 }
 
@@ -643,13 +680,14 @@
 
 template <typename T>
 __global__ __launch_bounds__(256) void attention_rows_kernel(const T* __restrict__ qbase, size_t ldq,
-                                                             const T* __restrict__ kbase, const T* __restrict__ vbase,
-                                                             size_t ldkv, int H, int head_dim,
+                                                             const T* __restrict__ kbase, size_t ldk,
+                                                             const T* __restrict__ vbase, size_t ldv, int H, int head_dim,
                                                              const int32_t* __restrict__ row_offset,
                                                              const uint8_t* __restrict__ row_uniform,
                                                              const uint8_t* __restrict__ tok_key, int64_t row0,
                                                              int rows, int tok0, float scaling, int flags ,
-                                                             const int32_t* __restrict__ tok_pair, T* __restrict__ ctx) {
+                                                             const int32_t* __restrict__ tok_pair, const int32_t* __restrict__ tok_qk,
+                                                             T* __restrict__ ctx) {
     const int cls_only = flags & 1;
     const int lane = threadIdx.x & 63;
     const int64_t w = (int64_t)blockIdx.x * 4 + (threadIdx.x >> 6);
@@ -677,13 +715,30 @@
     const int nq = cls_only ? 1 : (t1 - t0);
     const int ccol = active ? col : 0;
     auto brow = [&](int t) -> size_t { return (size_t)chunk_row(t, rl, t == t0, rows); };
-    int pslot = 0;
+    const int nk = t1 - t0;
+    if (nk == 1) {
+        if (active) {
+            const size_t vr = tok_pair ? (size_t)tok_pair[tok0 + t0] : (size_t)rl;
+            float v[8];
+            load8<T>(vbase + vr * ldv + ccol, v);
+#pragma unroll
+            for (int c = 0; c < 8; ++c) v[c] = v[c] + 0.0f;
+            store8<T>(ctx + (size_t)rl * H + col, v);
+        }
+        return;
+    }
+    int pslot = 0, qslot = 0;
     if (tok_pair) { const int t = t0 + li; pslot = t < t1 ? tok_pair[tok0 + t] : 0; }
-    auto qrow = [&](int t) -> size_t {
+    if (tok_qk) { const int t = t0 + li; qslot = t < t1 ? tok_qk[tok0 + t] : 0; }
+    auto vrow = [&](int t) -> size_t {
         if (!tok_pair) return brow(t);
         return t - t0 < lpr ? (size_t)__shfl(pslot, base + (t - t0), 64) : (size_t)tok_pair[tok0 + t];
     };
-    const int nk = t1 - t0;
+    auto qrow = [&](int t) -> size_t {
+        if (!tok_qk) return vrow(t);
+        return t - t0 < lpr ? (size_t)__shfl(qslot, base + (t - t0), 64) : (size_t)tok_qk[tok0 + t];
+    };
+    const size_t q0row = tok_qk ? qrow(t0) : (size_t)rl;
     if constexpr (sizeof(T) == 2) {
         if (nk <= ATT_FAST_KEYS && (flags & 2)) {
             const bool mine = li < nk && (uniform || tok_key[tok0 + t0 + li] != 0);
@@ -693,12 +748,12 @@
             for (int j = 0; j < ATT_FAST_KEYS; ++j) {
                 if (j < nk) {
                     const size_t kr = qrow(t0 + j);
-                    kk[j] = *(const uint4*)(kbase + kr * ldkv + ccol);
-                    vv[j] = *(const uint4*)(vbase + kr * ldkv + ccol);
+                    kk[j] = *(const uint4*)(kbase + kr * ldk + ccol);
+                    vv[j] = *(const uint4*)(vbase + vrow(t0 + j) * ldv + ccol);
                     if (!cls_only) qq[j] = *(const uint4*)(qbase + kr * ldq + ccol);
                 }
             }
-            if (cls_only) qq[0] = *(const uint4*)(qbase + (size_t)rl * ldq + ccol);
+            if (cls_only) qq[0] = *(const uint4*)(qbase + q0row * ldq + ccol);
             const float sc2 = scaling * 1.4426950408889634f;
 #pragma unroll
             for (int qi = 0; qi < ATT_FAST_KEYS; ++qi) {
@@ -743,16 +798,15 @@
     }
     for (int qi = 0; qi < nq; ++qi) {
         float q[8];
-        load8<T>(qbase + (cls_only ? (size_t)rl : qrow(t0 + qi)) * ldq + ccol, q);
+        load8<T>(qbase + (cls_only ? q0row : qrow(t0 + qi)) * ldq + ccol, q);
         float mx = -INFINITY, l = 0.f, acc[8];
 #pragma unroll
         for (int c = 0; c < 8; ++c) acc[c] = 0.f;
         for (int kj = t0; kj < t1; ++kj) {
             if (!uniform && !tok_key[tok0 + kj]) continue;
             float k[8], v[8];
-            const size_t kr = qrow(kj);
-            load8<T>(kbase + kr * ldkv + ccol, k);
-            load8<T>(vbase + kr * ldkv + ccol, v);
+            load8<T>(kbase + qrow(kj) * ldk + ccol, k);
+            load8<T>(vbase + vrow(kj) * ldv + ccol, v);
             float s = 0.f;
 #pragma unroll
             for (int c = 0; c < 8; ++c) s = fmaf(q[c], k[c], s);
diff --git a/zett_amd/csrc/zett_hip.hip b/zett_amd/csrc/zett_hip.hip
--- a/zett_amd/csrc/zett_hip.hip
+++ b/zett_amd/csrc/zett_hip.hip
@@ -57,6 +57,7 @@
     int time_gemm = 0;
     int cls_only_last = 1;
     int pair_dedupe = 1;
+    int single_qk_skip = 1;
     int residual_lo = 1;
     int concurrent_lanes = 0;
     hipStream_t lane_stream = nullptr;
@@ -80,6 +81,7 @@
         int64_t n_rows = 0;
         int seq = 0;
         bool pair_plan = false;
+        bool qk_plan = false;
         const int32_t* ext_id_slot = nullptr;
         bool pending = false;
     } plan[2];
@@ -194,8 +196,8 @@
     const int64_t V = (int64_t)c.original_vocab_size + c.n_extra;
     const int64_t max_tok = N * (int64_t)(seq + (c.embed_lang ? 1 : 0));
     const int64_t K = pair_keys(c, seq);
-    const size_t scan_scratch = 2 * ((size_t)std::max<int64_t>(std::max<int64_t>(N, V), K) / SCAN_CHUNK + 2) + 1;
-    return ((size_t)N + (N + 1) + 3 + V + (V + 1) + V + 7 * (size_t)max_tok + 2 * (size_t)K + 2 + scan_scratch) * 4;
+    const size_t scan_scratch = 2 * ((size_t)std::max<int64_t>(std::max<int64_t>(std::max<int64_t>(N, V), K), max_tok) / SCAN_CHUNK + 2) + 1;
+    return ((size_t)N + (N + 1) + 4 + (N + 1) + N + V + (V + 1) + V + 13 * (size_t)max_tok + 1 + 2 * (size_t)K + 2 + scan_scratch) * 4;
 }
 
 static int64_t chunk_token_cap(const zett_config& c, size_t es) {
@@ -224,6 +226,7 @@
     PlanArrays p{};
     int32_t* scan_tmp = nullptr;
     bool pair_plan = false;
+    bool qk_plan = false;
     int64_t PK = 0;
     size_t n_clear = 0;
 };
@@ -236,14 +239,17 @@
     PlanArrays& p = L.p;
     L.PK = pair_keys(c, seq);
     L.pair_plan = h->pair_dedupe && c.layers >= 2 && L.PK <= std::max<int64_t>(4 * max_tok, (int64_t)1 << 23) && L.PK < (int64_t)0x7fffffff;
+    L.qk_plan = h->single_qk_skip && h->precision != ZETT_PREC_F32 && h->gemm_variant == 0 && c.hidden >= h->gemm4d_min_k;
     int32_t* base = s.i32.as<int32_t>();
     p.id_flag = base; base += V;
     if (L.pair_plan) { p.pair_flag = base; base += L.PK; }
+    if (L.pair_plan && L.qk_plan) { p.pair_qk_flag = base; base += max_tok; }
     p.err = base; base += 1;
     L.n_clear = (size_t)(base - s.i32.as<int32_t>());
     p.row_count = base; base += N;
     p.row_offset = base; base += N + 1;
-    p.counters = base; base += 3;
+    p.counters = base; base += 4;
+    p.multi_off = base; base += N + 1;
     p.id_slot = base; base += V + 1;
     p.id_list = base; base += V;
     p.tok_slot = base; base += max_tok;
@@ -257,6 +263,19 @@
         p.pair_pos = base; base += max_tok;
         p.pair_slot = base; base += L.PK + 1;
     }
+    if (L.qk_plan) {
+        p.row_multi = base; base += N;
+        p.qk_rows = base; base += max_tok;
+        p.tok_qk = base; base += max_tok;
+        if (L.pair_plan) {
+            p.pair_qk_slot = base; base += max_tok + 1;
+            p.pair_qk_rows = base; base += max_tok;
+            p.tok_qk0 = base; base += max_tok;
+            p.n_pair_qk = (int32_t)max_tok;
+        }
+    } else {
+        p.multi_off = nullptr;
+    }
     L.scan_tmp = base;
     p.row_uniform = s.u8.as<uint8_t>();
     p.tok_key = p.row_uniform + N;
@@ -270,7 +289,7 @@
     const int64_t max_tok = N * (int64_t)(seq + lam);
     if (int rc = s.i32.reserve(plan_i32_bytes(c, N, seq))) return rc;
     if (int rc = s.u8.reserve((size_t)N + (size_t)max_tok)) return rc;
-    const size_t need_ints = (size_t)N + 1 + 3;
+    const size_t need_ints = (size_t)N + 1 + 4 + (size_t)N + 1;
     if (s.host_ints < need_ints) {
         if (s.host) (void)hipHostFree(s.host);
         s.host = nullptr;
@@ -285,6 +304,7 @@
     const int rb = (int)((N + 255) / 256);
     hipLaunchKernelGGL(plan_rows_kernel, dim3(rb), dim3(256), 0, st, sfm, N, seq, c.pad_token_id, lam, V, p);
     launch_exclusive_scan(p.row_count, p.row_offset, N, L.scan_tmp, st);
+    if (L.qk_plan) launch_exclusive_scan(p.row_multi, p.multi_off, N, L.scan_tmp, st);
     launch_exclusive_scan(p.id_flag, p.id_slot, (int64_t)V, L.scan_tmp, st);
     {
         PlanArrays pt = p;
@@ -294,12 +314,17 @@
     if (L.pair_plan) {
         launch_exclusive_scan(p.pair_flag, p.pair_slot, L.PK, L.scan_tmp, st);
         hipLaunchKernelGGL(plan_pairs_kernel, dim3((unsigned)((max_tok + 255) / 256)), dim3(256), 0, st, N, p);
+        if (L.qk_plan) {
+            hipLaunchKernelGGL(plan_pair_qk_mark_kernel, dim3((unsigned)((max_tok + 255) / 256)), dim3(256), 0, st, N, p);
+            launch_exclusive_scan(p.pair_qk_flag, p.pair_qk_slot, max_tok, L.scan_tmp, st);
+            hipLaunchKernelGGL(plan_pair_qk_kernel, dim3((unsigned)((max_tok + 255) / 256)), dim3(256), 0, st, N, p);
+        }
     }
     hipLaunchKernelGGL(plan_idlist_kernel, dim3((V + 255) / 256), dim3(256), 0, st, V, p);
     HIP_TRY(hipGetLastError());
-    HIP_TRY(hipMemcpyAsync(s.host, p.row_offset, ((size_t)N + 1 + 3) * 4, hipMemcpyDeviceToHost, st));
+    HIP_TRY(hipMemcpyAsync(s.host, p.row_offset, need_ints * 4, hipMemcpyDeviceToHost, st));
     HIP_TRY(hipEventRecord(s.done, st));
-    s.sfm = sfm; s.n_rows = N; s.seq = seq; s.pair_plan = L.pair_plan; s.ext_id_slot = h->ext.id_slot;
+    s.sfm = sfm; s.n_rows = N; s.seq = seq; s.pair_plan = L.pair_plan; s.qk_plan = L.qk_plan; s.ext_id_slot = h->ext.id_slot;
     return 0;
 }
 
@@ -537,6 +562,8 @@
         h->cls_only_last = value != 0;
     } else if (k == "pair_dedupe") {
         h->pair_dedupe = value != 0;
+    } else if (k == "single_qk_skip") {
+        h->single_qk_skip = value != 0;
     } else if (k == "residual_lo") {
         if (value < 0 || value > 2) return fail(ZETT_E_INVALID, "residual_lo must be 0 (fp32 residual stream), 1 (16-bit stream in f16 mode) or 2 (in bf16 mode too)");
         h->residual_lo = (int)value;
@@ -898,6 +925,7 @@
     long a_rows_readable = 0;
     bool staged_dst = false;
     int stage_lane = 0;
+    bool force_4d = false;
 
     int variant_for(int M, int N, int K, const GemmEpilogue<T>& e) const {
     constexpr bool is_f32 = std::is_same<T, float>::value;
@@ -917,14 +945,16 @@
                          (e.split_col >= N || e.split_col % 8 == 0);
     if (variant != 1 && !wide_ok) variant = 1;
     if (e.residual && (e.scale || e.shift)) variant = 1;
-    if (e.stats_part || e.fold_stats) variant = 7;
+    if (e.stats_part || e.fold_stats || force_4d) variant = 7;
         return variant;
     }
 
 
-    void gemm(const T* A, int lda, const T* Wp, int ldw, int M, int N, int K, const GemmEpilogue<T>& e) {
+    void gemm(const T* A, int lda, const T* Wp, int ldw, int M, int N, int K, const GemmEpilogue<T>& e, const int32_t* a_index = nullptr, int a_rows = 0) {
         if (rc || M <= 0) return;
         GemmArgs<T> g{A, lda, Wp, ldw, M, N, K, e};
+        g.a_index = a_index;
+        g.a_rows = a_rows;
         g.tile_order = h->gemm_tile_order;
         g.group = h->gemm_group;
         g.row0 = h->gemm_tail_split == 1 ? -1 : h->gemm_tail_split == 2 ? ((M / 2 + 255) / 256) * 256 : h->gemm_tail_split == 3 ? -2 : 0;
@@ -1161,7 +1191,7 @@
 
     zett_hypernet::PlanSlot& ps = h->plan[h->plan_cur ^ 1];
     if (ps.pending && ps.sfm == sfm && ps.n_rows == N && ps.seq == seq && ps.pair_plan == plan_layout(h, ps, N, seq).pair_plan &&
-        ps.ext_id_slot == h->ext.id_slot) {
+        ps.qk_plan == plan_layout(h, ps, N, seq).qk_plan && ps.ext_id_slot == h->ext.id_slot) {
         HIP_TRY(hipStreamWaitEvent(st, ps.done, 0));
     } else {
         if (ps.pending) HIP_TRY(hipEventSynchronize(ps.done));
@@ -1183,6 +1213,7 @@
     const PlanLayout PL = plan_layout(h, ps, N, seq);
     const PlanArrays& p = PL.p;
     const bool pair_plan = PL.pair_plan;
+    const bool qk_skip = PL.qk_plan;
     if (!h->range_accumulate) HIP_TRY(hipMemsetAsync(h->range_word, 0, 4, st));
     for (hipEvent_t& e : h->out_ready)
         if (!e) HIP_TRY(hipEventCreateWithFlags(&e, hipEventDisableTiming));
@@ -1319,6 +1350,16 @@
         const int P = pair_plan ? hoff[N + 3] : 0;
         const bool pairs = pair_plan && rows == N && P > 0 && (int64_t)P * 100 <= (int64_t)m * 85;
         int32_t* brow_pair = p.tok_pkey;
+        const int32_t* moff = hoff + N + 5;
+        const int Rq = qk_skip ? moff[r1] - moff[r0] : rows;
+        const int Mq = Rq + (m - rows);
+        const int Pq = qk_skip && pairs ? hoff[N + 4] : P;
+        const bool qk_chunk = qk_skip && Mq < m && (size_t)m * H * sizeof(T) <= (size_t)0x7fffffff;
+        const bool qk_pair = qk_skip && pairs && Pq < P && (size_t)P * H * sizeof(T) <= (size_t)0x7fffffff;
+        if (qk_chunk) {
+            hipLaunchKernelGGL(qk_rows_kernel, dim3((m + 255) / 256), dim3(256), 0, st, m, tok0, r0, rows, Rq, p);
+            R.check("qk_rows");
+        }
         if (pairs) {
             LnEmbed pe = emb;
             pe.tok_slot = p.pair_tslot; pe.tok_pos = p.pair_pos; pe.tok_row = nullptr;
@@ -1345,14 +1386,33 @@
             const int att_flags = (h->attention_fast ? 2 : 0) | (h->attention_pack ? 4 : 0);
             if (!cls_only) {
                 const bool by_pair = pairs && l == 0;
+                const int mv = by_pair ? P : m, mq = by_pair ? Pq : Mq;
                 GemmEpilogue<T> eq = R.epi();
                 eq.bias = bqkv; eq.out_lo = BIG; eq.ld_lo = 3 * H;
                 if (raw) { eq.fold_stats = hs_stats; eq.fold_c = cqkv; }
-                R.gemm(Zt, H, wqkv, H, by_pair ? P : m, 3 * H, H, eq);
-                hipLaunchKernelGGL((attention_rows_kernel<T>), dim3((unsigned)((waves + 3) / 4)), dim3(256), 0, st,
-                                   (const T*)BIG, (size_t)3 * H, (const T*)BIG + H, (const T*)BIG + 2 * H, (size_t)3 * H,
-                                   H, H / c.heads, p.row_offset, p.row_uniform, p.tok_key, r0, rows, tok0, scaling, 0 | att_flags,
-                                   by_pair ? (const int32_t*)p.tok_pair : (const int32_t*)nullptr, CTX);
+                if ((by_pair ? qk_pair : qk_chunk) && R.variant_for(mv, 3 * H, H, eq) == 7) {
+                    T* Vb = BIG;
+                    T* QK = BIG + (size_t)mv * H;
+                    GemmEpilogue<T> ev = eq;
+                    ev.bias = bqkv + 2 * H; ev.out_lo = Vb; ev.ld_lo = H;
+                    if (raw) ev.fold_c = cqkv + 2 * H;
+                    eq.out_lo = QK; eq.ld_lo = 2 * H;
+                    R.force_4d = true;
+                    R.gemm(Zt, H, wqkv + (size_t)2 * H * H, H, mv, H, H, ev);
+                    R.gemm(Zt, H, wqkv, H, mq, 2 * H, H, eq, by_pair ? p.pair_qk_rows : p.qk_rows + tok0, mv);
+                    R.force_4d = false;
+                    hipLaunchKernelGGL((attention_rows_kernel<T>), dim3((unsigned)((waves + 3) / 4)), dim3(256), 0, st,
+                                       (const T*)QK, (size_t)2 * H, (const T*)QK + H, (size_t)2 * H, (const T*)Vb, (size_t)H,
+                                       H, H / c.heads, p.row_offset, p.row_uniform, p.tok_key, r0, rows, tok0, scaling, 0 | att_flags,
+                                       by_pair ? (const int32_t*)p.tok_pair : (const int32_t*)nullptr,
+                                       by_pair ? (const int32_t*)p.tok_qk0 : (const int32_t*)p.tok_qk, CTX);
+                } else {
+                    R.gemm(Zt, H, wqkv, H, mv, 3 * H, H, eq);
+                    hipLaunchKernelGGL((attention_rows_kernel<T>), dim3((unsigned)((waves + 3) / 4)), dim3(256), 0, st,
+                                       (const T*)BIG, (size_t)3 * H, (const T*)BIG + H, (size_t)3 * H, (const T*)BIG + 2 * H, (size_t)3 * H,
+                                       H, H / c.heads, p.row_offset, p.row_uniform, p.tok_key, r0, rows, tok0, scaling, 0 | att_flags,
+                                       by_pair ? (const int32_t*)p.tok_pair : (const int32_t*)nullptr, (const int32_t*)nullptr, CTX);
+                }
                 R.check("attention");
             } else {
                 T* KV = BIG;
@@ -1360,15 +1420,35 @@
                 GemmEpilogue<T> ekv = R.epi();
                 ekv.bias = bqkv + H; ekv.out_lo = KV; ekv.ld_lo = 2 * H;
                 if (raw) { ekv.fold_stats = hs_stats; ekv.fold_c = cqkv + H; }
-                R.gemm(Zt, H, wqkv + (size_t)H * H, H, m, 2 * H, H, ekv);
                 GemmEpilogue<T> eq = R.epi();
                 eq.bias = bqkv; eq.out_lo = Q; eq.ld_lo = H;
                 if (raw) { eq.fold_stats = hs_stats; eq.fold_c = cqkv; }
-                R.gemm(Zt, H, wqkv, H, rows, H, H, eq);
-                hipLaunchKernelGGL((attention_rows_kernel<T>), dim3((unsigned)((waves + 3) / 4)), dim3(256), 0, st,
-                                   (const T*)Q, (size_t)H, (const T*)KV, (const T*)KV + H, (size_t)2 * H,
-                                   H, H / c.heads, p.row_offset, p.row_uniform, p.tok_key, r0, rows, tok0, scaling, 1 | att_flags,
-                                   (const int32_t*)nullptr, CTX);
+                if (qk_chunk && R.variant_for(m, 2 * H, H, ekv) == 7 && R.variant_for(rows, H, H, eq) == 7) {
+                    T* Vb = BIG;
+                    T* Kb = BIG + (size_t)m * H;
+                    T* Qb = Kb + (size_t)Mq * H;
+                    GemmEpilogue<T> ev = ekv;
+                    ev.bias = bqkv + 2 * H; ev.out_lo = Vb; ev.ld_lo = H;
+                    if (raw) ev.fold_c = cqkv + 2 * H;
+                    ekv.out_lo = Kb; ekv.ld_lo = H;
+                    eq.out_lo = Qb;
+                    R.force_4d = true;
+                    R.gemm(Zt, H, wqkv + (size_t)2 * H * H, H, m, H, H, ev);
+                    R.gemm(Zt, H, wqkv + (size_t)H * H, H, Mq, H, H, ekv, p.qk_rows + tok0, m);
+                    R.gemm(Zt, H, wqkv, H, Rq, H, H, eq, p.qk_rows + tok0, m);
+                    R.force_4d = false;
+                    hipLaunchKernelGGL((attention_rows_kernel<T>), dim3((unsigned)((waves + 3) / 4)), dim3(256), 0, st,
+                                       (const T*)Qb, (size_t)H, (const T*)Kb, (size_t)H, (const T*)Vb, (size_t)H,
+                                       H, H / c.heads, p.row_offset, p.row_uniform, p.tok_key, r0, rows, tok0, scaling, 1 | att_flags,
+                                       (const int32_t*)nullptr, (const int32_t*)p.tok_qk, CTX);
+                } else {
+                    R.gemm(Zt, H, wqkv + (size_t)H * H, H, m, 2 * H, H, ekv);
+                    R.gemm(Zt, H, wqkv, H, rows, H, H, eq);
+                    hipLaunchKernelGGL((attention_rows_kernel<T>), dim3((unsigned)((waves + 3) / 4)), dim3(256), 0, st,
+                                       (const T*)Q, (size_t)H, (const T*)KV, (size_t)2 * H, (const T*)KV + H, (size_t)2 * H,
+                                       H, H / c.heads, p.row_offset, p.row_uniform, p.tok_key, r0, rows, tok0, scaling, 1 | att_flags,
+                                       (const int32_t*)nullptr, (const int32_t*)nullptr, CTX);
+                }
                 R.check("attention(position 0)");
                 zrows = rows;
             }
```

Result: no change. 624,200, median of 6 (+0.4%).
